# safe-autonomous-systems/fluidgym

Measured on AMD Instinct MI355X. Metric: env-steps/sec (batched) + pressure-Poisson HBM GB/s vs roofline, 1/2/4/8 GPUs, higher is better.
Workload: dtype f32; 1 GPU; ChannelJet2D-v0 (2D channel stand-in for 'cylinder Re=100 256x128'), 64 envs/GPU, 25 PISO steps/env step, random jets, stirred by a body force N(0,2.0) redrawn every env step; global_batch=64, parallelism=env-sharded x1, 1 bcast + 1 all_gather per step (RCCL), lanes_per_gpu=2, workload_modified=True, capped_solves=0, floor_released_solves=0, advection_solver_form=two-brick, velocity_solver=on-chip Jacobi sweeps (policy advection_jacobi; 11972 solves settled by

## Files before the change

### fluidgym_amd/_lib.py

```python
from __future__ import annotations

import ctypes
import os
from ctypes import POINTER, Structure, c_char_p, c_float, c_int, c_int32, c_int64, c_void_p

_HERE = os.path.dirname(os.path.abspath(__file__))
LIB_PATH = os.environ.get("FLUIDGYM_AMD_LIB") or os.path.join(_HERE, "libfluidgym_hip.so")
LIB_F64_PATH = os.environ.get("FLUIDGYM_AMD_LIB_F64") or os.path.join(_HERE, "libfluidgym_hip_f64.so")

FG_MAX_SCALARS = 4
FG_FIELD_SUMMARY_WORK_BYTES = 128
FG_OK = 0
FG_ERR_NOT_CONVERGED = -5
FG_ERR_NOT_FINITE = -6
FG_ERR_FLUX_BALANCE = -7
FG_PERIODIC, FG_FIXED = 0, 1
FG_DIRICHLET, FG_NEUMANN = 0, 1
FG_VELOCITY, FG_PRESSURE, FG_SCALAR, FG_VELOCITY_SOURCE, FG_VISCOSITY_FIELD = 0, 1, 2, 3, 4
FG_BOUND_VELOCITY, FG_BOUND_SCALAR = 8, 16
FG_SOLVER_CG, FG_SOLVER_JACOBI, FG_SOLVER_RBGS, FG_SOLVER_MGCG, FG_SOLVER_FDCG = 0, 1, 2, 3, 4
(FG_BUF_A, FG_BUF_C_OFF, FG_BUF_ADV_RHS, FG_BUF_VEL_RESULT, FG_BUF_H, FG_BUF_DIV, FG_BUF_P_RESULT,
 FG_BUF_SCALAR_RESULT) = range(8)
FG_ERR_UNSUPPORTED = -4
FG_ERR_INVALID_ARG = -1
# ... 77 lines not shown


class FgMbSimOptions(Structure):
    _fields_ = [
        ("step", FgMbStepOptions),
        ("time_step", c_float),
        ("cfl", c_float),
        ("adaptive", c_int32),
        ("substeps", c_int32),
        ("flux_balance_tol", c_float),
        ("outflow_slot0", c_int32),
        ("outflow_count", c_int32),
        ("outflow_velm", c_float * 3),
        ("outflow_tol", c_float),
        ("max_substeps", c_int32),
        ("outflow_slot0_b", c_int32),
        ("outflow_count_b", c_int32),
    ]


(FG_MB_BUF_A, FG_MB_BUF_C_OFF, FG_MB_BUF_RHS, FG_MB_BUF_H, FG_MB_BUF_DIV, FG_MB_BUF_P_DIAG, FG_MB_BUF_P_OFF,
 FG_MB_BUF_VELOCITY_RESULT) = range(8)
FG_MB_BUF_KRYLOV0 = 8


class FgSimOptions(Structure):
    _fields_ = [
        ("step", FgStepOptions),
        ("time_step", c_float),
        ("cfl", c_float),
        ("adaptive", c_int32),
        ("substeps", c_int32),
        ("flux_balance_tol", c_float),
        ("outflow_mask", c_int32),
        ("outflow_velm", c_float * 3),
        ("outflow_tol", c_float),
        ("max_substeps", c_int32),
    ]


SIGNATURES = {
    "fg_abi_version": (c_int, []),
    "fg_last_error": (c_char_p, []),
    "fg_create": (c_int, [POINTER(FgConfig), POINTER(c_float), POINTER(c_float), POINTER(c_float), POINTER(c_void_p)]),
    "fg_destroy": (c_int, [c_void_p]),
    "fg_bind": (c_int, [c_void_p, c_int, c_void_p]),
    "fg_set_viscosity": (c_int, [c_void_p, c_float]),
    "fg_set_scalar_viscosity": (c_int, [c_void_p, c_int, c_float]),
    "fg_set_viscosity_batch": (c_int, [c_void_p, c_void_p]),
    "fg_set_scalar_viscosity_batch": (c_int, [c_void_p, c_int, c_void_p]),
    "fg_set_fd_preconditioner": (c_int, [c_void_p] + [POINTER(c_float)] * 7),
    "fg_max_velocity": (c_int, [c_void_p, c_void_p, c_void_p]),
    "fg_set_fd_fast_transform": (c_int, [c_void_p, c_int, c_float]),
    "fg_set_return_best": (c_int, [c_void_p, c_int]),
    "fg_set_cg_reset_steps": (c_int, [c_void_p, c_int]),
    "fg_set_advection_start": (c_int, [c_void_p, c_int]),
    "fg_set_wall_stress_forcing": (c_int, [c_void_p, c_int, c_float, c_float]),
    "fg_boundary_flux_balance": (c_int, [c_void_p, c_void_p, c_void_p]),
    "fg_step_diagnostics": (c_int, [c_void_p, POINTER(c_float), c_void_p]),
    "fg_update_advective_boundary": (c_int, [c_void_p, c_int, POINTER(c_float), c_void_p, c_void_p]),
    "fg_balance_boundary_fluxes": (c_int, [c_void_p, c_int, c_float, c_void_p, c_void_p]),
    "fg_setup_advection": (c_int, [c_void_p, c_void_p, c_int, c_int, c_void_p]),
    "fg_solve_advection": (c_int, [c_void_p, c_int, c_int, c_float, c_int, POINTER(FgSolveInfo), c_void_p]),
    "fg_copy_scalar_result_to_blocks": (c_int, [c_void_p, c_int, c_void_p]),
    "fg_setup_pressure_matrix": (c_int, [c_void_p, c_void_p]),
    "fg_setup_pressure_rhs": (c_int, [c_void_p, c_void_p, c_void_p]),
    "fg_solve_pressure": (c_int, [c_void_p, c_int, c_float, c_int, c_int, POINTER(FgSolveInfo), c_void_p]),
    "fg_correct_velocity": (c_int, [c_void_p, c_void_p]),
    "fg_copy_velocity_result_to_blocks": (c_int, [c_void_p, c_void_p]),
    "fg_copy_velocity_result_from_blocks": (c_int, [c_void_p, c_void_p]),
    "fg_piso_step": (c_int, [c_void_p, c_void_p, POINTER(FgStepOptions), POINTER(c_int32), c_void_p]),
    "fg_single_step": (c_int, [c_void_p, POINTER(FgSimOptions), POINTER(c_int32), POINTER(c_float), c_void_p]),
    "fg_multi_step": (c_int, [c_void_p, POINTER(FgSimOptions), c_int32, POINTER(c_void_p), POINTER(c_int32), POINTER(c_float), POINTER(c_int32), c_void_p]),
    "fg_make_divergence_free": (c_int, [c_void_p, c_float, c_int, POINTER(FgSolveInfo), c_void_p]),
    "fg_reset_solver_state": (c_int, [c_void_p, c_void_p]),
    "fg_solver_hints": (c_int, [c_void_p, POINTER(c_int32), c_int32]),
    "fg_env_restore_field": (c_int, [c_void_p, c_int, c_void_p, c_int32, POINTER(FgEnvSel), c_int32, c_int32, c_void_p]),
    "fg_env_reset_solver_state": (c_int, [c_void_p, POINTER(FgEnvSel), c_int32, c_void_p]),
    "fg_mb_env_restore_field": (c_int, [c_void_p, c_int, c_void_p, c_int32, POINTER(FgEnvSel), c_int32, c_int32, c_void_p]),
    "fg_mb_env_reset_solver_state": (c_int, [c_void_p, POINTER(FgEnvSel), c_int32, c_void_p]),
    "fg_set_pressure_refinement": (c_int, [c_void_p, c_int32, c_float, c_float]),
    "fg_get_buffer": (c_int, [c_void_p, c_int, POINTER(c_void_p), POINTER(c_int64)]),
    "fg_read_buffer": (c_int, [c_void_p, c_int, c_void_p, c_void_p]),
    "fg_poisson_apply": (c_int, [c_void_p, c_void_p, c_void_p, c_void_p, c_void_p]),
    "fg_poisson_jacobi": (c_int, [c_void_p, c_void_p, c_void_p, c_void_p, c_int, c_float, c_void_p]),
    "fg_poisson_rbgs": (c_int, [c_void_p, c_void_p, c_void_p, c_void_p, c_int, c_float, c_void_p]),
    "fg_poisson_cg": (c_int, [c_void_p, c_void_p, c_void_p, c_void_p, c_float, c_int, c_int, POINTER(FgSolveInfo),
                              c_void_p]),
    "fg_poisson_fdcg": (c_int, [c_void_p, c_void_p, c_void_p, c_void_p, c_float, c_int, c_int, POINTER(FgSolveInfo),
                                c_void_p]),
    "fg_sparse_apply_ell": (c_int, [c_void_p, c_void_p, c_int32, c_int32, c_void_p, c_int64, c_int32, c_void_p, c_void_p]),
    "fg_sparse_apply_csr": (c_int, [c_void_p, c_void_p, c_void_p, c_int32, c_void_p, c_int64, c_int32, c_void_p, c_void_p]),
    "fg_stream_triad": (c_int, [c_void_p, c_void_p, c_void_p, c_float, c_int64, c_int32, POINTER(c_float), c_void_p]),
    "fg_mb_multilevel_status": (c_int, [c_void_p, POINTER(c_int32)]),
    "fg_mb_multilevel_apply": (c_int, [c_void_p, c_void_p, c_void_p, c_void_p]),
    "fg_mb_debug_ilu_apply": (c_int, [c_void_p, c_void_p, c_void_p, c_void_p]),
    "fg_mb_debug_pressure_cg": (c_int, [c_void_p, c_float, c_int32, c_int32, POINTER(c_int32), POINTER(c_int32), POINTER(ctypes.c_double), c_void_p]),
    "fg_mb_wall_forces": (c_int, [c_void_p, c_void_p, c_void_p, c_void_p, c_int32, c_int32, c_float, c_float, c_void_p, c_void_p]),
    "fg_mb_wall_forces_batch": (c_int, [c_void_p, c_void_p, c_void_p, c_void_p, c_int32, c_int32, c_float, c_float, c_void_p, c_void_p, c_void_p]),
    "fg_mb_debug_bicgstab": (c_int, [c_void_p, c_float, c_int32, c_int32, POINTER(c_int64), POINTER(ctypes.c_double), POINTER(c_float), c_void_p]),
    "fg_dacc_host_sum": (c_int, [POINTER(ctypes.c_double), c_int64, ctypes.c_double, POINTER(ctypes.c_double)]),
    "fg_dacc_device_sum": (c_int, [POINTER(ctypes.c_double), c_int64, ctypes.c_double, c_int32, POINTER(ctypes.c_double), c_void_p]),
    "fg_field_summary": (c_int, [c_void_p, c_int32, c_int32, c_int64, c_int32, c_void_p, c_void_p, c_void_p, ctypes.c_double, ctypes.c_double,
                                 c_int32, c_void_p, c_void_p]),
    "fg_plane_moments": (c_int, [POINTER(c_void_p), POINTER(c_int64), c_int32, c_int32, c_int32, c_int32, c_int32, c_int32, c_void_p, c_void_p,
                                 c_void_p, c_void_p, c_void_p]),
    "fg_plane_budgets": (c_int, [POINTER(c_void_p), POINTER(c_int64), c_int32, c_int32, c_int32, c_int32, c_int32, c_void_p, c_void_p, c_void_p,
                                 c_int32, c_int32, c_void_p, c_void_p, c_void_p, c_void_p, c_void_p]),
    "fg_plane_timecorr": (c_int, [POINTER(c_void_p), POINTER(c_int64), c_int32, c_int32, c_int32, c_int32, c_int32, c_int32, c_int32,
                                  POINTER(c_int32), c_void_p, c_void_p, c_void_p, c_void_p]),
    "fg_mb_cell_moments": (c_int, [c_void_p, c_void_p, c_int32, c_int32, c_int64, POINTER(c_int64), c_int32, c_int64, c_void_p, c_void_p,
                                   c_void_p]),
    "fg_mb_cell_moments_widths": (c_int, [c_void_p, c_void_p, c_int64, POINTER(c_int64), c_int32, c_void_p, c_void_p, POINTER(c_int32)]),
    "fg_plane_spectra": (c_int, [POINTER(c_void_p), POINTER(c_int64), c_int32, c_int32, c_int32, c_int32, c_int32, POINTER(c_int32), c_int32,
                                 c_void_p, c_void_p, c_void_p]),
    "fg_coherence_litmus": (c_int, [c_int32, c_int32, c_int32, c_int32, POINTER(c_int64), POINTER(ctypes.c_double), c_void_p]),
    "fg_profile_enable": (c_int, [c_void_p, c_int]),
    "fg_profile_kinds": (c_int, []),
    "fg_profile_kind_name": (ctypes.c_char_p, [c_int]),
    "fg_profile_read": (c_int, [c_void_p, c_int, POINTER(ctypes.c_double), POINTER(c_int64), POINTER(ctypes.c_double),
                                POINTER(ctypes.c_double), POINTER(ctypes.c_double), POINTER(ctypes.c_double),
                                POINTER(c_int64), POINTER(c_int64), POINTER(ctypes.c_double), POINTER(c_int64)]),
    "fg_coords_to_transforms": (c_int, [c_void_p, c_void_p, c_int, c_int, c_int, c_int, c_void_p]),
    "fg_resampler_create": (c_int, [c_int, POINTER(ctypes.c_int32), POINTER(ctypes.c_int32), POINTER(ctypes.c_int32),
                                    POINTER(ctypes.c_float), c_int, c_int, POINTER(c_void_p)]),
    "fg_resampler_destroy": (c_int, [c_void_p]),
    "fg_resample": (c_int, [c_void_p, c_void_p, c_int, c_int, c_void_p, c_int, c_void_p]),
    "fg_envglue_jet_schedule": (c_int, [c_void_p, c_void_p, c_void_p, c_void_p, c_int32, c_int32, c_int32, c_void_p, c_void_p, c_void_p]),
    "fg_envglue_channel_observe": (c_int, [c_void_p, c_void_p, c_void_p, c_int32, c_int32, c_int32, c_int32, c_float, c_float, c_void_p,
                                           c_void_p, c_void_p, c_void_p, c_void_p, c_void_p]),
    "fg_envglue_channel_observe_batch": (c_int, [c_void_p, c_void_p, c_void_p, c_int32, c_int32, c_int32, c_int32, c_void_p, c_float, c_void_p,
                                                 c_void_p, c_void_p, c_void_p, c_void_p, c_void_p]),
    "fg_mb_create": (c_int, [c_int32, c_int32, c_int32, POINTER(c_void_p)]),
    "fg_mb_destroy": (c_int, [c_void_p]),
    "fg_config_dump": (c_int, [c_void_p, ctypes.c_char_p, c_int]),
    "fg_mb_config_dump": (c_int, [c_void_p, ctypes.c_char_p, c_int]),
    "fg_mb_add_block": (c_int, [c_void_p, POINTER(c_float), c_int32, c_int32, c_int32, POINTER(c_int32)]),
    "fg_mb_connect": (c_int, [c_void_p, c_int32, c_int32, c_int32, c_int32, c_int32, c_int32]),
    "fg_mb_make_periodic": (c_int, [c_void_p, c_int32, c_int32]),
    "fg_mb_set_reference_quirks": (c_int, [c_void_p, c_int32, c_int32]),
    "fg_mb_set_nonortho_flags": (c_int, [c_void_p, c_int32]),
    "fg_mb_finalize": (c_int, [c_void_p]),
    "fg_mb_sizes": (c_int, [c_void_p, POINTER(c_int32), POINTER(c_int32)]),
    "fg_mb_block_info": (c_int, [c_void_p, c_int32, POINTER(c_int32), POINTER(c_int32)]),
    "fg_mb_get_host_table": (c_int, [c_void_p, c_int32, c_void_p, POINTER(c_int64)]),
    "fg_mb_get_neighbors": (c_int, [c_void_p, POINTER(c_int32)]),
    "fg_mb_bind": (c_int, [c_void_p, c_void_p, c_void_p, c_void_p, c_void_p]),
    "fg_mb_set_viscosity": (c_int, [c_void_p, c_float]),
    "fg_mb_set_viscosity_batch": (c_int, [c_void_p, c_void_p]),
    "fg_mb_piso_step": (c_int, [c_void_p, c_void_p, POINTER(FgMbStepOptions), POINTER(c_int32), c_void_p]),
    "fg_mb_max_velocity": (c_int, [c_void_p, POINTER(c_float), c_void_p]),
    "fg_mb_set_residual_projection": (c_int, [c_void_p, POINTER(c_float)]),
    "fg_mb_set_stall_limit": (c_int, [c_void_p, c_int32]),
    "fg_mb_set_advection_start": (c_int, [c_void_p, c_int]),
    "fg_mb_set_advection_jacobi": (c_int, [c_void_p, c_int]),
    "fg_mb_advection_jacobi_counts": (c_int, [c_void_p, POINTER(c_int64)]),
    "fg_mb_set_multilevel": (c_int, [c_void_p, c_int32, c_int32, POINTER(c_int32), POINTER(c_int32), POINTER(c_int32), POINTER(c_float),
                                     POINTER(c_float), c_float, c_int32]),
    "fg_mb_env_status": (c_int, [c_void_p, POINTER(c_int32)]),
    "fg_mb_ladder": (c_int, [c_void_p, POINTER(c_int64), c_int32]),
    "fg_mb_debug_cycles": (c_int, [c_void_p, POINTER(ctypes.c_uint64)]),
    "fg_mb_solver_hints": (c_int, [c_void_p, POINTER(c_int32), c_int32]),
    "fg_mb_solver_unconverged": (c_int, [c_void_p, POINTER(c_int64)]),
    "fg_solver_unconverged": (c_int, [c_void_p, POINTER(c_int64)]),
    "fg_mb_solver_counters": (c_int, [c_void_p, POINTER(c_int64), c_int32]),
    "fg_set_advection_preconditioner": (c_int, [c_void_p, c_int]),
# ... 124 lines not shown
```

### fluidgym_amd/csrc/fg_api.hip

```cpp
#include <stdio.h>
#include <string.h>

#include <cmath>
#include <string>
#include <vector>

#include <stdlib.h>

#include "fg_internal.h"

static thread_local std::string g_last_error;
void fg_set_error(const std::string& msg) { g_last_error = msg; }

extern "C" int fg_abi_version(void) { return FG_ABI_VERSION; }
extern "C" const char* fg_last_error(void) { return g_last_error.c_str(); }

static FgBounds make_bounds(const fg_state* s, int channel) {
    FgBounds b;
    for (int f = 0; f < 6; ++f) {
        b.vel[f] = s->bvel[f];
        b.scal[f] = s->bscal[f];
        b.scalar_bc[f] = s->cfg.scalar_bc[f][channel < 0 ? 0 : channel];
    }
    return b;
// ... 20 lines not shown
    FG_REQUIRE(cfg->n_scalars >= 0 && cfg->n_scalars <= FG_MAX_SCALARS, FG_ERR_INVALID_ARG, "bad n_scalars");
    for (int a = 0; a < cfg->dims; ++a)
        FG_REQUIRE(cfg->face_type[2 * a] == cfg->face_type[2 * a + 1], FG_ERR_INVALID_ARG,
                   "a FIXED face needs a FIXED partner (CloseBoundary closes both, domain_structs.cpp:1981-2002)");
    FG_REQUIRE((long long)cfg->nx * cfg->ny * cfg->nz * cfg->batch * 6 < (1LL << 31), FG_ERR_UNSUPPORTED,
               "index space exceeds int32 (reference index_t is int32 as well)");
    FG_HIP_CHECK(hipSetDevice(cfg->device));

    fg_state* s = new fg_state();
    memset(s, 0, sizeof(*s));
    s->cfg = *cfg;
    FgGrid& g = s->grid;
    g.dims = cfg->dims; g.nx = cfg->nx; g.ny = cfg->ny; g.nz = cfg->nz;
    g.n = cfg->nx * cfg->ny * cfg->nz; g.B = cfg->batch;
    for (int f = 0; f < 6; ++f) g.fixed[f] = (f < 2 * cfg->dims) ? (cfg->face_type[f] == FG_FIXED) : 0;
    s->vec = (!FG_F64 && cfg->nx % 4 == 0) ? 4 : 1;
    s->viscosity = 0.f;

    const fg_real* hsrc[3] = {hx, hy, hz};
    const int hn[3] = {cfg->nx, cfg->ny, cfg->nz};
    for (int a = 0; a < 3; ++a) {
        std::vector<fg_real> h(hn[a], 1.f), rh(hn[a], 1.f);
        if (a < cfg->dims)
            for (int i = 0; i < hn[a]; ++i) {
                if (!(hsrc[a][i] > 0.f)) { delete s; fg_set_error("cell widths must be positive"); return FG_ERR_INVALID_ARG; }
                h[i] = hsrc[a][i]; rh[i] = 1.f / hsrc[a][i];
            }
        FG_HIP_CHECK(hipMalloc(&s->d_h[a], sizeof(fg_real) * hn[a]));
        FG_HIP_CHECK(hipMalloc(&s->d_rh[a], sizeof(fg_real) * hn[a]));
        FG_HIP_CHECK(hipMemcpy(s->d_h[a], h.data(), sizeof(fg_real) * hn[a], hipMemcpyHostToDevice));
        FG_HIP_CHECK(hipMemcpy(s->d_rh[a], rh.data(), sizeof(fg_real) * hn[a], hipMemcpyHostToDevice));
        g.h[a] = s->d_h[a]; g.rh[a] = s->d_rh[a];
    }
    const size_t BN = (size_t)g.B * g.n, d = g.dims;
    auto alloc = [&](fg_real** p, size_t count) -> hipError_t {
        hipError_t e = hipMalloc(p, sizeof(fg_real) * count);
        if (e == hipSuccess) e = hipMemset(*p, 0, sizeof(fg_real) * count);
        return e;
    };
    FG_HIP_CHECK(alloc(&s->A, BN));
    FG_HIP_CHECK(alloc(&s->rA, BN));
    FG_HIP_CHECK(alloc(&s->Coff, BN * 2 * d));
    FG_HIP_CHECK(alloc(&s->adv_rhs, BN * d));
    FG_HIP_CHECK(alloc(&s->vel_result, BN * d));
    FG_HIP_CHECK(alloc(&s->hvec, BN * d));
    FG_HIP_CHECK(alloc(&s->div, BN));
    FG_HIP_CHECK(alloc(&s->p_result, BN));
    FG_HIP_CHECK(alloc(&s->scal_result, BN));
    for (int i = 0; i < 8; ++i) FG_HIP_CHECK(alloc(&s->w[i], BN * d));
    const size_t nsys = (size_t)g.B * d;
    FG_HIP_CHECK(hipMalloc(&s->acc, sizeof(FgDacc) * nsys * FG_ACC_DOUBLES));
    FG_HIP_CHECK(hipMemset(s->acc, 0, sizeof(FgDacc) * nsys * FG_ACC_DOUBLES));
    FG_HIP_CHECK(hipMalloc(&s->flags, sizeof(int32_t) * nsys));
    FG_HIP_CHECK(hipMalloc(&s->info_dev, sizeof(fg_solve_info) * nsys));
    FG_HIP_CHECK(hipHostMalloc(&s->info_pinned, sizeof(fg_solve_info) * nsys));
    FG_HIP_CHECK(hipHostMalloc(&s->flags_pinned, sizeof(int32_t) * nsys));
    FG_HIP_CHECK(alloc(&s->scratch_B, (size_t)g.B * (4 + 2 * d)));
    FG_HIP_CHECK(hipMalloc(&s->d_bvel_ptrs, sizeof(fg_real*) * 6));
    FG_HIP_CHECK(hipMemset(s->d_bvel_ptrs, 0, sizeof(fg_real*) * 6));
    FG_HIP_CHECK(hipHostMalloc(&s->diag_pinned, sizeof(fg_real) * 2 * g.B));
    FG_HIP_CHECK(hipHostMalloc(&s->dt_pinned, sizeof(fg_real) * g.B));
    FG_HIP_CHECK(alloc(&s->dt_dev, g.B));
    FG_HIP_CHECK(hipMalloc(&s->env_sel_dev, sizeof(fg_env_sel) * g.B));
    s->t_rem_dev = nullptr;
#if !FG_F64
    FG_HIP_CHECK(hipMalloc(&s->t_rem_dev, sizeof(double) * g.B));
    FG_HIP_CHECK(hipMemset(s->t_rem_dev, 0, sizeof(double) * g.B));
#endif
    if (int rc = fg_poll_create(&s->poll, (int)(nsys > 2 * (size_t)g.B ? nsys : 2 * (size_t)g.B))) return rc;
    for (int k = 0; k < 4; ++k) { s->pred_bicg[k] = 2; s->pred_cg[k] = 1; }
    s->wall_forcing_axis = -1;
    s->ref64_inner = 1e-4f;
    s->cg_wgs_per_slot = 256;
    { const char* ev = getenv("FG_BICG3"); s->bicg3_force = ev ? atoi(ev) : -1; }
    { const char* ev = getenv("FG_BICG3_BXL"); s->bicg3_bxl = ev ? atoi(ev) : 0; }
    { const char* ev = getenv("FG_BICG_SUB"); s->bicg_sub = ev ? atoi(ev) : -1; }
    { const char* ev = getenv("FG_REDUCE_WGS"); s->reduce_wgs = ev ? atoi(ev) : 0; }
    { const char* ev = getenv("FG_BICG3_MIX"); s->bicg3_mix = ev ? atoi(ev) : 3; }
    { const char* ev = getenv("FG_BICG_FUSED"); s->bicg_fused = ev ? atoi(ev) : 1; }
    s->tridiag_cb = 64;
    s->helm_cb_pref = 32;
    { const char* ev = getenv("FG_HELM_ROWFORM"); s->helm_rowform_off = (ev && atoi(ev) == 0) ? 1 : 0; }
    { const char* ev = getenv("FG_FD_FACFUSE"); s->fd_facfuse = ev ? atoi(ev) : 1; }
    { const char* ev = getenv("FG_DEV_DT"); s->dev_dt = ev ? atoi(ev) : 1; }
    { const char* ev = getenv("FG_ADV_LINESWEEP"); s->adv_linesweep = ev ? atoi(ev) : 0; }
    { const char* ev = getenv("FG_FD_ROWMEAN"); s->fd_rowmean = ev ? atoi(ev) : 1; }
    s->fd_row_epoch = -1; s->rA_epoch = 0; s->fd_row_part_epoch = -1;
    { const char* ev = getenv("FG_CG_FUSED"); s->cg_fused = ev ? atoi(ev) : 1; }
    { const char* ev = getenv("FG_BICG_PFUSED"); s->bicg_pfused = ev ? atoi(ev) : 1; }
    { const char* ev = getenv("FG_ADV_JACOBI"); s->adv_jacobi = ev ? atoi(ev) : 0; s->adv_jacobi_env = ev ? 1 : 0; }
    for (int k = 0; k < 4; ++k) s->jac_hist[k] = FgJacHist{0, 0, 0};
    s->jac_solves = s->jac_fallbacks = 0;
    FG_HIP_CHECK(hipHostMalloc(&s->jac_prev, sizeof(float) * 4 * nsys));
    s->jac_rA_epoch = -1;
    FG_HIP_CHECK(hipMalloc(&s->fcg_alpha, sizeof(double) * 2 * (size_t)g.B));
    FG_HIP_CHECK(hipMemset(s->fcg_alpha, 0, sizeof(double) * 2 * (size_t)g.B));
    FG_HIP_CHECK(hipMalloc(&s->fcg_xsum, sizeof(FgDacc) * 2 * (size_t)g.B));
    FG_HIP_CHECK(hipMemset(s->fcg_xsum, 0, sizeof(FgDacc) * 2 * (size_t)g.B));
    FG_HIP_CHECK(hipMalloc(&s->fcg_lazy, sizeof(int32_t) * (size_t)g.B));
    FG_HIP_CHECK(hipMemset(s->fcg_lazy, 0, sizeof(int32_t) * (size_t)g.B));
    { const char* e = getenv("FG_FCG_FIRST"); s->fcg_first = (e && atoi(e) == 0) ? 0 : 1; }
    { const char* e = getenv("FG_JAC_SPEC"); s->jac_spec = (e && atoi(e) == 0) ? 0 : 1; }
    { const char* e = getenv("FG_FCG_SPEC"); s->fcg_spec = (e && atoi(e) == 0) ? 0 : 1; }
    { const char* e = getenv("FG_JAC_PREFACTOR"); s->jac_prefactor = (e && atoi(e) == 0) ? 0 : 1; }
    { const char* e = getenv("FG_JAC_WARM"); s->jac_warm = e ? (atoi(e) != 0 ? 1 : 0) : -1; }
    s->cg_return_best = 1;
    s->cg_reset_steps = 100;
    s->adv_from_result = 1;
    FG_HIP_CHECK(hipMalloc(&s->cg_acc, sizeof(FgDacc) * (size_t)g.B * 8 * 64));
    FG_HIP_CHECK(hipMemset(s->cg_acc, 0, sizeof(FgDacc) * (size_t)g.B * 8 * 64));
    FG_HIP_CHECK(hipMalloc(&s->cg_best.best_crit, sizeof(fg_real) * g.B));
    FG_HIP_CHECK(hipMalloc(&s->cg_best.saved_crit, sizeof(fg_real) * g.B));
    FG_HIP_CHECK(hipMalloc(&s->cg_best.save_at, sizeof(int32_t) * g.B));
    FG_HIP_CHECK(alloc(&s->cg_best.best_x, BN));
    *out = s;
    return FG_OK;
}

extern "C" int fg_destroy(fg_handle s) {
    if (!s) return FG_OK;
    for (int a = 0; a < 3; ++a) { (void)hipFree(s->d_h[a]); (void)hipFree(s->d_rh[a]); }
    fg_real* owned[] = {s->A, s->rA, s->Coff, s->adv_rhs, s->vel_result, s->hvec, s->div, s->p_result, s->scal_result,
                      s->scratch_B};
    for (fg_real* p : owned) (void)hipFree(p);
    for (int i = 0; i < 8; ++i) (void)hipFree(s->w[i]);
    (void)hipFree(s->acc); (void)hipFree(s->flags); (void)hipFree(s->info_dev);
    (void)hipHostFree(s->info_pinned); (void)hipHostFree(s->flags_pinned);
    fg_prof_destroy(s);
    fg_poll_destroy(&s->poll);
    (void)hipFree(s->d_bvel_ptrs); (void)hipHostFree(s->diag_pinned); (void)hipHostFree(s->dt_pinned); (void)hipFree(s->dt_dev); (void)hipFree(s->t_rem_dev); (void)hipFree(s->env_sel_dev);
    float* fd[] = {s->fd_Qx, s->fd_QxT, s->fd_Qz, s->fd_QzT, s->fd_lower, s->fd_inv, s->fd_cp};
    for (float* p : fd) if (p) (void)hipFree(p);
    if (s->fd_dct_tw) { (void)hipFree(s->fd_dct_tw); (void)hipFree(s->fd_dct_rot); }
    (void)hipFree(s->cg_acc); (void)hipFree(s->fcg_alpha); (void)hipFree(s->fcg_xsum); (void)hipFree(s->fcg_lazy);
    if (s->jac_prev) (void)hipHostFree(s->jac_prev);
    (void)hipFree(s->fd_row_part); (void)hipFree(s->fd_lam_x); (void)hipFree(s->fd_row_inv); (void)hipFree(s->fd_row_cp); (void)hipFree(s->fd_row_lower);
    (void)hipFree(s->line_inv); (void)hipFree(s->line_cp); (void)hipFree(s->ilu_d);
    (void)hipFree(s->r64_buf); (void)hipFree(s->r64_acc); (void)hipFree(s->ref64_x); (void)hipFree(s->force_uniform);
    (void)hipFree(s->fd_lam); (void)hipFree(s->helm_diag); (void)hipFree(s->helm_lower); (void)hipFree(s->helm_upper); (void)hipFree(s->helm_tmp); (void)hipFree(s->helm_lower_row); (void)hipFree(s->helm_lower_row2); (void)hipFree(s->line_inv2); (void)hipFree(s->line_cp2);
    (void)hipFree(s->cg_best.best_crit); (void)hipFree(s->cg_best.saved_crit); (void)hipFree(s->cg_best.save_at); (void)hipFree(s->cg_best.best_x);
    delete s;
    return FG_OK;
}

static int sync_bvel_ptrs(fg_state* s);
extern "C" int fg_bind(fg_handle s, int field, fg_real* ptr) {
    FG_REQUIRE(s, FG_ERR_INVALID_ARG, "null handle");
    if (field == FG_VELOCITY) s->velocity = ptr;
    else if (field == FG_PRESSURE) s->pressure = ptr;
    else if (field == FG_SCALAR) s->scalar = ptr;
    else if (field == FG_VELOCITY_SOURCE) s->velocity_source = ptr;
    else if (field == FG_VISCOSITY_FIELD) s->visc_field = ptr;
    else if (field >= FG_BOUND_VELOCITY && field < FG_BOUND_VELOCITY + 6) {
        s->bvel[field - FG_BOUND_VELOCITY] = ptr;
        return sync_bvel_ptrs(s);
    }
    else if (field >= FG_BOUND_SCALAR && field < FG_BOUND_SCALAR + 6) s->bscal[field - FG_BOUND_SCALAR] = ptr;
    else FG_REQUIRE(false, FG_ERR_INVALID_ARG, "fg_bind: unknown field id");
    return FG_OK;
}

extern "C" int fg_set_viscosity(fg_handle s, fg_real v) {
    FG_REQUIRE(s, FG_ERR_INVALID_ARG, "null handle");
    s->viscosity = v;
    return FG_OK;
}
extern "C" int fg_set_scalar_viscosity(fg_handle s, int ch, fg_real v) {
    FG_REQUIRE(s && ch >= 0 && ch < FG_MAX_SCALARS, FG_ERR_INVALID_ARG, "bad channel");
    s->scalar_viscosity[ch] = v;
    s->scalar_viscosity_set = true;
    return FG_OK;
}
extern "C" int fg_set_viscosity_batch(fg_handle s, const fg_real* nu_B) {
    FG_REQUIRE(s, FG_ERR_INVALID_ARG, "null handle");
    s->viscosity_B = nu_B;
    s->helm_pre_mask = 0;
    return FG_OK;
}
extern "C" int fg_set_scalar_viscosity_batch(fg_handle s, int ch, const fg_real* k_B) {
    FG_REQUIRE(s && ch >= 0 && ch < FG_MAX_SCALARS, FG_ERR_INVALID_ARG, "bad channel");
    s->scalar_viscosity_B[ch] = k_B;
    s->helm_pre_mask = 0;
    return FG_OK;
}

extern "C" int fg_set_fd_preconditioner(fg_handle s, const float* Qx, const float* QxT, const float* Qz, const float* QzT,
                                        const float* lower, const float* inv, const float* cp) {
    FG_REQUIRE(s && Qx && QxT && lower && inv && cp, FG_ERR_INVALID_ARG, "null argument");
    FG_REQUIRE(s->grid.fixed[2] && s->grid.fixed[3], FG_ERR_UNSUPPORTED, "FD preconditioner needs FIXED y faces");
    FG_REQUIRE(s->grid.dims == 2 || (Qz && QzT), FG_ERR_INVALID_ARG, "Qz required in 3-D");
#if !FG_F64
    FG_REQUIRE(s->grid.ny <= 640, FG_ERR_UNSUPPORTED, "FD preconditioner: at most 640 cells along y (LDS of the tridiagonal solve)");
#endif
    const size_t nx = s->grid.nx, ny = s->grid.ny, nz = s->grid.nz;
    auto up = [&](float** dst, const float* src, size_t count) -> hipError_t {
        if (*dst) (void)hipFree(*dst);
        hipError_t e = hipMalloc(dst, sizeof(float) * count);
        if (e == hipSuccess) e = hipMemcpy(*dst, src, sizeof(float) * count, hipMemcpyHostToDevice);
        return e;
    };
    FG_HIP_CHECK(up(&s->fd_Qx, Qx, nx * nx));
    FG_HIP_CHECK(up(&s->fd_QxT, QxT, nx * nx));
    if (s->grid.dims == 3) {
        FG_HIP_CHECK(up(&s->fd_Qz, Qz, nz * nz));
        FG_HIP_CHECK(up(&s->fd_QzT, QzT, nz * nz));
    }
    FG_HIP_CHECK(up(&s->fd_lower, lower, ny));
    FG_HIP_CHECK(up(&s->fd_inv, inv, nx * ny * nz));
    FG_HIP_CHECK(up(&s->fd_cp, cp, nx * ny * nz));
    s->fd_dct_x = 0;
    return FG_OK;
}

extern "C" int fg_set_return_best(fg_handle s, int on) {
    FG_REQUIRE(s, FG_ERR_INVALID_ARG, "null handle");
    s->cg_return_best = on ? 1 : 0;
    return FG_OK;
// ... 221 lines not shown
    return setup_advection(s, dt_B, for_scalar, channel, stream, -1, 0);
}
static int setup_advection(fg_handle s, const fg_real* dt_B, int for_scalar, int channel, void* stream, int buoy_axis, fg_real buoy_factor) {
    FG_REQUIRE(s && dt_B, FG_ERR_INVALID_ARG, "null argument");
    if (int rc = check_bound(s, for_scalar != 0)) return rc;
    FG_REQUIRE(!for_scalar || (channel >= 0 && channel < s->cfg.n_scalars), FG_ERR_INVALID_ARG, "bad scalar channel");
    s->cur_dt = dt_B;
    FgAdvArgs a;
    memset(&a, 0, sizeof(a));
    a.vel = s->velocity;
    a.dt = dt_B;
    a.for_scalar = for_scalar;
    a.channel = channel;
    a.n_scalars = s->cfg.n_scalars;
    a.A = s->A; a.Coff = s->Coff; a.rhs = s->adv_rhs;
    if (for_scalar) {
        a.scal = s->scalar + (size_t)channel * s->grid.n;
        a.scal_env_stride = (long)s->cfg.n_scalars * s->grid.n;
        a.nu = fg_nu(s, 1, channel);
    } else {
        a.source = s->velocity_source;
        if (s->wall_forcing_axis >= 0)
            if (int rc = fg_launch_wall_forcing(s, (hipStream_t)stream)) return rc;
        a.force = s->wall_forcing_axis >= 0 ? s->force_uniform : nullptr;
        a.visc = s->visc_field;
        a.nu = fg_nu(s);
        a.rA = s->rA;
        s->adv_last_dt = dt_B;
        s->rA_epoch++;
        s->jac_rA_epoch = s->rA_epoch;
#if !FG_F64
        if (fg_fd_rowmean_ok(s) && s->vec == 4 && (s->grid.nx & 63) == 0) {
            if (!s->fd_row_part) FG_HIP_CHECK(hipMalloc(&s->fd_row_part, sizeof(float) * (size_t)s->grid.B * s->grid.ny * (s->grid.nx / 64)));
            a.row_part = s->fd_row_part;
            s->fd_row_part_epoch = s->rA_epoch;
        }
#endif
        if (buoy_axis >= 0) {
            a.buoy_T = s->scalar; a.buoy_stride = (long)s->cfg.n_scalars * s->grid.n; a.buoy_axis = buoy_axis; a.buoy_factor = buoy_factor;
            a.source_w = s->velocity_source;
        }
    }
    return fg_launch_adv_build(s, make_bounds(s, channel), a, (hipStream_t)stream);
}

static int advection_solve(fg_state* s, FgBicgArgs a, fg_solve_info* info, hipStream_t st, int for_scalar = 0, int channel = 0, bool* spec_ran = nullptr);

extern "C" int fg_solve_advection(fg_handle s, int for_scalar, int channel, fg_real tol, int max_iterations,
                                  fg_solve_info* info_host, void* stream) {
    FG_REQUIRE(s, FG_ERR_INVALID_ARG, "null handle");
    FgBicgArgs a;
    a.diag = s->A; a.off = s->Coff; a.rhs = s->adv_rhs;
    a.dt = s->cur_dt;
    a.tol = tol; a.max_iterations = max_iterations;
    if (for_scalar) { a.x = s->scal_result; a.nc = 1; a.use_x0 = 0; a.kind = 0; }
    else { a.x = s->vel_result; a.nc = s->grid.dims; a.use_x0 = s->adv_from_result; }
    return advection_solve(s, a, info_host, (hipStream_t)stream, for_scalar, channel);
}

extern "C" int fg_copy_scalar_result_to_blocks(fg_handle s, int channel, void* stream) {
    FG_REQUIRE(s && s->scalar, FG_ERR_NOT_BOUND, "scalar not bound");
    const int n = s->grid.n;
    if (s->cfg.n_scalars == 1) return fg_launch_copy_active(s, s->cur_dt, s->scal_result, s->scalar, 1, (hipStream_t)stream);
    FG_HIP_CHECK(hipMemcpy2DAsync(s->scalar + (size_t)channel * n, sizeof(fg_real) * n * s->cfg.n_scalars, s->scal_result,
                                  sizeof(fg_real) * n, sizeof(fg_real) * n, s->grid.B, hipMemcpyDeviceToDevice,
                                  (hipStream_t)stream));
    return FG_OK;
}

extern "C" int fg_setup_pressure_matrix(fg_handle s, void* stream) {
    FG_REQUIRE(s, FG_ERR_INVALID_ARG, "null handle");
    s->rA_epoch++;
    return fg_launch_pressure_setup(s, s->cur_dt, (hipStream_t)stream);
}

extern "C" int fg_setup_pressure_rhs(fg_handle s, const fg_real* dt_B, void* stream) {
    FG_REQUIRE(s && dt_B, FG_ERR_INVALID_ARG, "null argument");
    if (int rc = check_bound(s, false)) return rc;
    hipStream_t st = (hipStream_t)stream;
    if (int rc = fg_launch_h(s, dt_B, s->vel_result, st)) return rc;
    return fg_launch_div(s, make_bounds(s, 0), dt_B, s->hvec, s->div, st);
}

struct SpecH { fg_state* s; const fg_real* dt; const fg_step_options* opt; hipStream_t st; };
static int spec_h(void* p) {
    const SpecH* c = static_cast<const SpecH*>(p);
    fg_state* s = c->s;
    if (int rc = fg_launch_h(s, c->dt, s->vel_result, c->st)) return rc;
    return fg_launch_div(s, make_bounds(s, 0), c->dt, s->hvec, s->div, c->st, !c->opt->pressure_warm_start,
                         c->opt->pressure_method == FG_SOLVER_FDCG && s->fd_Qx != nullptr);
}

static int launch_corrector(fg_state* s, const fg_real* dt, const FgCgOutcome& o, bool last, hipStream_t st) {
    const bool mean_folded = last && o.mean_ready;
    FG_REQUIRE(!o.lazy_z || !last || mean_folded, FG_ERR_UNSUPPORTED, "fg_piso_step: an unmaterialised pressure without its folded mean");
    if (last && !mean_folded)
        if (int rc = fg_launch_mean_sub(s, dt, s->p_result, s->pressure, st)) return rc;
    const FgMeanRef mean = {s->fcg_xsum, s->info_dev, s->pressure, o.marks_valid ? s->fcg_lazy : nullptr, s->fcg_alpha};
    const FgLazyRef lazy = {s->fcg_lazy, s->fcg_alpha, last ? s->p_result : nullptr};
    const fg_real* p = o.lazy_z ? o.lazy_z : ((last && !mean_folded) ? s->pressure : s->p_result);
    return fg_launch_correct(s, dt, s->rA, s->hvec, p, s->vel_result, st, last ? s->velocity : nullptr, mean_folded ? &mean : nullptr, o.lazy_z ? &lazy : nullptr);
}

struct SpecCorrect { fg_state* s; const fg_real* dt; bool last; hipStream_t st; };
static int spec_correct(void* p, const FgCgOutcome& o) {
    const SpecCorrect* c = static_cast<const SpecCorrect*>(p);
    return launch_corrector(c->s, c->dt, o, c->last, c->st);
}

static int solve_pressure(fg_state* s, const fg_real* dt, int method, fg_real tol, int max_iterations, int use_previous,
                          fg_solve_info* info_host, hipStream_t st, bool finalize = true, int kind = 2, FgCgOutcome* out = nullptr,
                          FgCgSpec spec = FgCgSpec{}) {
    int rc = FG_OK;
    FgCgOutcome own;
    if (!out) out = &own;
    if (method == FG_SOLVER_CG || method == FG_SOLVER_FDCG) {
        FgCgArgs a;
        a.rA = s->rA; a.b = s->div; a.x = s->p_result;
        a.r = s->w[0]; a.p = s->w[1]; a.Ap = s->w[2];
        a.dt = dt; a.tol = tol; a.max_iterations = max_iterations; a.use_x0 = use_previous;
        a.reset_steps = s->cg_reset_steps;
        a.precond = (method == FG_SOLVER_FDCG);
        a.kind = kind;
        a.check_every = a.precond ? 2 : 16;
        a.lazy_ok = finalize ? 0 : 1;
        a.spec = spec;
#if !FG_F64
        if (s->ref64_outer > 0) a.lazy_ok = 0;
#endif
        rc = fg_cg_solve(s, a, info_host, st, out);
#if !FG_F64
        if (s->ref64_outer > 0 && (rc == FG_OK || rc == FG_ERR_NOT_CONVERGED)) rc = fg_refine64_pressure(s, a, info_host, st, out);
        if (s->double_fallback && (rc == FG_ERR_NOT_FINITE || (s->ladder_force & 2))) {
            std::vector<fg_solve_info> tmp;
            fg_solve_info* info = info_host;
            if (!info) { tmp.assign(s->info_pinned, s->info_pinned + s->grid.B); info = tmp.data(); }
            s->rung_count[2] += 1;
            rc = fg_rung64_cg(s, a, info, (s->ladder_force & 2) != 0, st, out);
        }
#endif
    } else {
        fg_set_error("fg_solve_pressure: only FG_SOLVER_CG drives the PISO step (Jacobi/RBGS are smoothers)");
        return FG_ERR_UNSUPPORTED;
    }
    if (rc != FG_OK && rc != FG_ERR_NOT_CONVERGED) return rc;
    if (finalize)
        if (int rc2 = fg_launch_mean_sub(s, dt, s->p_result, s->pressure, st)) return rc2;
    return rc;
}

extern "C" int fg_solve_pressure(fg_handle s, int method, fg_real tol, int max_iterations, int use_previous,
                                 fg_solve_info* info_host, void* stream) {
    FG_REQUIRE(s, FG_ERR_INVALID_ARG, "null handle");
    if (int rc = check_bound(s, false)) return rc;
    return solve_pressure(s, s->cur_dt, method, tol, max_iterations, use_previous, info_host, (hipStream_t)stream);
}

extern "C" int fg_set_pressure_refinement(fg_handle s, int32_t max_corrections, fg_real target_tol, fg_real inner_relative_tol) {
    FG_REQUIRE(s, FG_ERR_INVALID_ARG, "null handle");
    FG_REQUIRE(!FG_F64 || max_corrections <= 0, FG_ERR_UNSUPPORTED, "fg_set_pressure_refinement: the fp64 build solves in fp64 already");
    FG_REQUIRE(max_corrections <= 0 || (target_tol > 0 && inner_relative_tol > 0 && inner_relative_tol < 1), FG_ERR_INVALID_ARG,
               "fg_set_pressure_refinement: tolerances must be positive, the relative one below 1");
    s->ref64_outer = max_corrections > 0 ? max_corrections : 0;
    s->ref64_tol = (float)target_tol; s->ref64_inner = (float)inner_relative_tol;
    return FG_OK;
}

extern "C" int fg_correct_velocity(fg_handle s, void* stream) {
    FG_REQUIRE(s, FG_ERR_INVALID_ARG, "null handle");
    if (int rc = check_bound(s, false)) return rc;
    return fg_launch_correct(s, s->cur_dt, s->rA, s->hvec, s->pressure, s->vel_result, (hipStream_t)stream);
}

// ... 29 lines not shown
    if (failed && s->double_fallback && rc != FG_ERR_HIP) {
        s->rung_count[0] += 1;
        rc = fg_rung64_bicgstab(s, a, info, (s->ladder_force & 1) != 0, st);
        if (rc != FG_OK && rc != FG_ERR_NOT_CONVERGED && rc != FG_ERR_NOT_FINITE) return rc;
        failed = (rc != FG_OK) || (s->ladder_force & 4);
    }
#endif
    if (failed && (s->adv_precond == 2 || s->adv_precond == 5)) {
        s->line_retries += 1;
        s->rung_count[1] += 1;
        a.precond = s->adv_precond == 5 ? 3 : 1; a.use_x0 = 0;
        rc = fg_bicgstab_solve(s, a, info, st);
    }
    (void)nsys;
    return rc;
}

extern "C" int fg_piso_step(fg_handle s, const fg_real* dt_B, const fg_step_options* opt, int32_t* stats_host,
                            void* stream) {
    FG_REQUIRE(s && dt_B && opt, FG_ERR_INVALID_ARG, "null argument");
    const bool scalar = opt->advect_scalar && s->cfg.n_scalars > 0;
    if (int rc = check_bound(s, scalar)) return rc;
    FG_REQUIRE(opt->buoyancy_axis < s->grid.dims, FG_ERR_INVALID_ARG, "bad buoyancy axis");
    FG_REQUIRE(opt->buoyancy_axis < 0 || (s->velocity_source && s->scalar), FG_ERR_NOT_BOUND,
               "buoyancy needs velocity source and scalar bound");
    hipStream_t st = (hipStream_t)stream;
    const int B = s->grid.B, d = s->grid.dims;
    std::vector<fg_solve_info> info((size_t)B * d);
    int32_t stats[4] = {-1, -1, -1, -1};
    struct DropHelmRecord { fg_state* s; ~DropHelmRecord() { s->helm_pre_mask = 0; } } drop_helm_record{s};
    int status = FG_OK;
    auto soft = [&](int rc) {
        if (rc == FG_ERR_NOT_CONVERGED) { status = rc; return FG_OK; }
        return rc;
    };
#if !FG_F64
    const bool sweeps_first = s->adv_linesweep && s->grid.dims == 2 && s->jac_hist[0].skip == 0 && s->jac_hist[1].skip == 0;
    if (scalar && s->cfg.n_scalars == 1 && s->adv_precond == 3 && s->fd_lam && !s->visc_field && !sweeps_first) {
        const FgNu nu2[2] = {fg_nu(s, 1, 0), fg_nu(s)};
        const int wlo[2] = {s->cfg.scalar_bc[2][0] == FG_DIRICHLET, 1}, whi[2] = {s->cfg.scalar_bc[3][0] == FG_DIRICHLET, 1};
        if (int rc = fg_helm_factor_pair(s, dt_B, nu2, wlo, whi, st)) return rc;
    }
#endif
    if (scalar) {
        FgRange range_scalar("scalar_advection");
        for (int ch = 0; ch < s->cfg.n_scalars; ++ch) {
            if (int rc = fg_setup_advection(s, dt_B, 1, ch, stream)) return rc;
            FgBicgArgs a;
            a.diag = s->A; a.off = s->Coff; a.rhs = s->adv_rhs; a.x = s->scal_result; a.nc = 1;
            a.dt = dt_B; a.tol = opt->advection_tol; a.max_iterations = opt->max_iterations; a.use_x0 = 0; a.kind = 0;
            if (int rc = soft(advection_solve(s, a, info.data(), st, 1, ch))) return rc;
            const int m = max_iters(info.data(), B);
            stats[0] = m > stats[0] ? m : stats[0];
            s->ctr.add(0, info.data(), B);
            const int n = s->grid.n;
            if (s->cfg.n_scalars == 1) {
                if (int rc = fg_launch_copy_active(s, dt_B, s->scal_result, s->scalar, 1, st)) return rc;
            } else {
                (void)n;
                fg_set_error("multi-channel scalar copy with inactive envs not implemented");
                return FG_ERR_UNSUPPORTED;
            }
        }
    }
    fg_range_push("velocity_assembly_and_solve");
    struct PopOnce { bool armed = true; void fire() { if (armed) { fg_range_pop(); armed = false; } } ~PopOnce() { fire(); } } range_velocity;
    if (int rc = setup_advection(s, dt_B, 0, 0, stream, opt->buoyancy_axis, opt->buoyancy_factor)) return rc;
    bool h_div_ran = false;
    {
        FgBicgArgs a;
        a.diag = s->A; a.off = s->Coff; a.rhs = s->adv_rhs; a.x = s->vel_result; a.nc = d;
        a.dt = dt_B; a.tol = opt->advection_tol; a.max_iterations = opt->max_iterations; a.use_x0 = s->adv_from_result;
        SpecH spec_h_ctx = {s, dt_B, opt, st};
        if (opt->corrector_steps > 0) a.spec = FgSpecHook{spec_h, &spec_h_ctx};
        if (int rc = soft(advection_solve(s, a, info.data(), st, 0, 0, &h_div_ran))) return rc;
        stats[1] = max_iters(info.data(), B * d);
        s->ctr.add(1, info.data(), B * d);
    }
    range_velocity.fire();
    for (int c = 0; c < opt->corrector_steps; ++c) {
        FgRange range_corr(c == 0 ? "pressure_corrector_0" : "pressure_corrector_1+");
        const bool last = (c + 1 == opt->corrector_steps);
        if (!(c == 0 && h_div_ran)) {
            if (int rc = fg_launch_h(s, dt_B, s->vel_result, st)) return rc;
            if (int rc = fg_launch_div(s, make_bounds(s, 0), dt_B, s->hvec, s->div, st, !opt->pressure_warm_start,
                                       opt->pressure_method == FG_SOLVER_FDCG && s->fd_Qx != nullptr))
                return rc;
        }
        SpecCorrect spec_ctx = {s, dt_B, last, st};
        FgCgOutcome outcome;
        if (int rc = soft(solve_pressure(s, dt_B, opt->pressure_method, opt->pressure_tol, opt->max_iterations, opt->pressure_warm_start ? 1 : 0,
                                         info.data(), st, false, c == 0 ? 0 : 1, &outcome, FgCgSpec{spec_correct, &spec_ctx})))
            return rc;
        if (c < 2) { stats[2 + c] = max_iters(info.data(), B); s->ctr.add(2 + c, info.data(), B); }
        if (!outcome.spec_done)
            if (int rc = launch_corrector(s, dt_B, outcome, last, st)) return rc;
    }
    if (opt->corrector_steps <= 0)
        if (int rc = fg_launch_copy_active(s, dt_B, s->vel_result, s->velocity, d, st)) return rc;
    if (stats_host) memcpy(stats_host, stats, sizeof(stats));
    s->ctr.piso_steps += 1;
    return status;
}

extern "C" int fg_config_dump(fg_handle s, char* buf, int n) {
    FG_REQUIRE(s && buf && n > 0, FG_ERR_INVALID_ARG, "fg_config_dump: bad argument");
    char tmp[3072];
    const int len = snprintf(tmp, sizeof(tmp),
        "{\"build\": \"%s\", \"FG_CG_FUSED\": %d, \"FG_BICG_PFUSED\": %d, \"FG_BICG_FUSED\": %d, \"FG_BICG_SUB\": %d, \"FG_BICG3\": %d, "
        "\"FG_BICG3_BXL\": %d, \"FG_BICG3_MIX\": %d, \"FG_REDUCE_WGS\": %d, \"FG_CG_WGS_PER_SLOT\": %d, \"FG_TRIDIAG_CB\": %d, \"FG_HELM_CB\": %d, "
        "\"FG_HELM_ROWFORM\": %d, \"FG_FD_ROWMEAN\": %d, \"FG_POLL_SPIN\": %d, \"FG_PROF_PERIOD\": %d, \"fast_transform_x\": %d, \"fd_preconditioner\": %d, "
        "\"helmholtz\": %d, \"advection_preconditioner\": %d, \"advection_from_result\": %d, \"return_best\": %d, \"cg_reset_steps\": %d, "
        "\"double_fallback\": %d, \"wall_forcing_axis\": %d, \"FG_ADV_JACOBI\": %d, \"FG_FCG_FIRST\": %d, \"FG_JAC_WARM\": %d, \"first_iterate_polls\": %ld, \"unstored_pressure_solves\": %ld, \"FG_JAC_SPEC\": %d, \"FG_FCG_SPEC\": %d, \"jacobi_speculation_misses\": %ld, \"jacobi_floor_released\": %ld, \"pressure_refinement_corrections\": %ld}",
        FG_F64 ? "f64" : "f32", s->cg_fused, s->bicg_pfused, s->bicg_fused, s->bicg_sub, s->bicg3_force, s->bicg3_bxl, s->bicg3_mix, s->reduce_wgs,
        s->cg_wgs_per_slot, s->tridiag_cb, s->helm_cb_pref, s->helm_rowform_off ? 0 : 1, s->fd_rowmean, s->poll.spin, s->prof.period, s->fd_dct_x, s->fd_Qx ? 1 : 0,
        s->fd_lam ? 1 : 0, s->adv_precond, s->adv_from_result, s->cg_return_best, s->cg_reset_steps, s->double_fallback, s->wall_forcing_axis, s->adv_jacobi, s->fcg_first, s->jac_warm,
        s->fcg_first_polls, s->fcg_unstored, s->jac_spec, s->fcg_spec, s->jac_spec_missed, s->jac_floor_released, s->ref64_corrections);
    if (len >= n) return len + 1;
    memcpy(buf, tmp, (size_t)len + 1);
    return FG_OK;
}

extern "C" int fg_solver_unconverged(fg_handle s, int64_t* out4) {
    FG_REQUIRE(s != nullptr && out4 != nullptr, FG_ERR_INVALID_ARG, "fg_solver_unconverged: bad argument");
    for (int k = 0; k < 4; ++k) out4[k] = s->ctr.unconv[k];
    return FG_OK;
}

extern "C" int fg_solver_counters(fg_handle s, int64_t* out13, int32_t reset) {
    FG_REQUIRE(s != nullptr, FG_ERR_INVALID_ARG, "fg_solver_counters: null handle");
    if (out13) s->ctr.write(out13);
    if (reset) s->ctr.reset();
    return FG_OK;
}

extern "C" int fg_single_step(fg_handle s, const fg_sim_options* o, int32_t* out, fg_real* flux_host, void* stream);
extern "C" int fg_multi_step(fg_handle s, const fg_sim_options* o, int32_t n, const fg_real* const* bvel_schedule, int32_t* out_6n,
                             fg_real* flux_host, int32_t* steps_done, void* stream) {
    FG_REQUIRE(s && o && out_6n && n >= 0, FG_ERR_INVALID_ARG, "fg_multi_step: bad argument");
    if (steps_done) *steps_done = 0;
    for (int k = 0; k < n; ++k) {
        if (bvel_schedule)
            for (int f = 0; f < 2 * s->grid.dims; ++f)
                if (const fg_real* p = bvel_schedule[(size_t)k * 6 + f])
                    if (int rc = fg_bind(s, FG_BOUND_VELOCITY + f, const_cast<fg_real*>(p))) return rc;
        if (int rc = fg_single_step(s, o, out_6n + 6 * (size_t)k, flux_host, stream)) return rc;
        if (steps_done) *steps_done = k + 1;
        if (out_6n[6 * (size_t)k + 5] == 0 && !s->cg_return_best) break;
    }
    return FG_OK;
}

static inline bool is_close_zero(double a) { return std::fabs(a) <= 1e-8; }

extern "C" int fg_single_step(fg_handle s, const fg_sim_options* o, int32_t* out, fg_real* flux_host, void* stream) {
    fg_htrace("single_step_in");
    FgRange range_sim("fg_single_step");
    FG_REQUIRE(s && o && out, FG_ERR_INVALID_ARG, "null argument");
    if (int rc = check_bound(s, o->step.advect_scalar && s->cfg.n_scalars > 0)) return rc;
    hipStream_t st = (hipStream_t)stream;
    const int B = s->grid.B;
    const FgBounds bnd = make_bounds(s, 0);
    std::vector<double> t_rem(B, (double)o->time_step);
    int32_t stats[4] = {-1, -1, -1, -1};
    int substeps = 0, all_ok = 1;
    bool first = true;
    int fixed_left = o->adaptive ? 0 : (o->substeps > 0 ? o->substeps : 1);
    for (;;) {
        bool any = false;
        if (o->adaptive) {
            for (int b = 0; b < B; ++b) any = any || (t_rem[b] > 0 && !is_close_zero(t_rem[b]));
        } else {
            any = fixed_left > 0;
        }
        if (!any) break;
        auto advance = [&](int b, fg_real max_vel) -> fg_real {
            fg_real ts = 0.f;
            if (!o->adaptive) {
                ts = o->time_step;
            } else if (t_rem[b] > 0 && !is_close_zero(t_rem[b])) {
                const double mv = (double)max_vel;
                const double max_ts = is_close_zero(mv) ? t_rem[b] : (double)o->cfl / mv;
                double tsd;
                if (max_ts >= t_rem[b]) tsd = t_rem[b];
                else tsd = t_rem[b] / (double)(long long)std::ceil(t_rem[b] / max_ts);
                t_rem[b] -= tsd;
                ts = (fg_real)tsd;
            }
            return ts;
        };
        auto flux_guard = [&]() -> int {
            fg_real worst = 0.f;
            for (int b = 0; b < B; ++b) {
                if (flux_host) flux_host[b] = s->diag_pinned[b];
                const fg_real a = std::fabs(s->diag_pinned[b]);
                worst = (a > worst || a != a) ? a : worst;
            }
            if (!(worst <= o->flux_balance_tol)) {
                fg_set_error("Domain boundary fluxes not balanced, cannot proceed with simulation step.");
                return FG_ERR_FLUX_BALANCE;
// ... 53 lines not shown
                s->diag_pinned[B + b] = fg_poll_word_float(&s->poll, 12 * B + b);
                if (first) s->diag_pinned[b] = fg_poll_word_float(&s->poll, 13 * B + b);
            }
            if (first) if (int rc2 = flux_guard()) return rc2;
            for (int b = 0; b < B; ++b) s->dt_pinned[b] = advance(b, s->diag_pinned[B + b]);
        }
        ++substeps;
        first = false;
        if (!o->adaptive) --fixed_left;
        if (substeps >= (o->max_substeps > 0 ? o->max_substeps : 100000)) break;
    }
    fg_htrace("single_step_out");
    for (int i = 0; i < 4; ++i) out[i] = stats[i];
    out[4] = substeps;
    out[5] = all_ok;
    return FG_OK;
}

extern "C" int fg_make_divergence_free(fg_handle s, fg_real tol, int max_iterations, fg_solve_info* info_host,
                                       void* stream) {
    FG_REQUIRE(s, FG_ERR_INVALID_ARG, "null handle");
    if (int rc = check_bound(s, false)) return rc;
    s->cur_dt = nullptr;
    hipStream_t st = (hipStream_t)stream;
    const size_t BN = (size_t)s->grid.B * s->grid.n;
    std::vector<fg_real> ones(BN, 1.f);
    FG_HIP_CHECK(hipMemcpyAsync(s->rA, ones.data(), sizeof(fg_real) * BN, hipMemcpyHostToDevice, st));
    s->rA_epoch++;
    FG_HIP_CHECK(hipStreamSynchronize(st));
    if (int rc = fg_launch_copy_active(s, nullptr, s->velocity, s->hvec, s->grid.dims, st)) return rc;
    if (int rc = fg_launch_div(s, make_bounds(s, 0), nullptr, s->hvec, s->div, st)) return rc;
    int rc = solve_pressure(s, nullptr, FG_SOLVER_CG, tol, max_iterations, 0, info_host, st);
    if (rc != FG_OK && rc != FG_ERR_NOT_CONVERGED) return rc;
    if (int rc2 = fg_launch_correct(s, nullptr, s->rA, s->hvec, s->pressure, s->vel_result, st)) return rc2;
    if (int rc2 = fg_launch_copy_active(s, nullptr, s->vel_result, s->velocity, s->grid.dims, st)) return rc2;
    return rc;
}

extern "C" int fg_reset_solver_state(fg_handle s, void* stream) {
    FG_REQUIRE(s && s->velocity, FG_ERR_NOT_BOUND, "velocity not bound");
    for (int k = 0; k < 4; ++k) s->jac_hist[k] = FgJacHist{0, 0, 0};
    FG_HIP_CHECK(hipMemsetAsync(s->p_result, 0, sizeof(fg_real) * (size_t)s->grid.B * s->grid.n, (hipStream_t)stream));
    return fg_launch_copy_active(s, nullptr, s->velocity, s->vel_result, s->grid.dims, (hipStream_t)stream);
}

extern "C" int fg_solver_hints(fg_handle s, int32_t* hints12, int32_t set) {
    FG_REQUIRE(s != nullptr && hints12 != nullptr, FG_ERR_INVALID_ARG, "fg_solver_hints: bad argument");
    for (int k = 0; k < 4; ++k) {
        FgJacHist& H = s->jac_hist[k];
        if (set) { H.sweeps = hints12[3 * k]; H.skip = hints12[3 * k + 1]; H.fails = hints12[3 * k + 2]; }
        else { hints12[3 * k] = H.sweeps; hints12[3 * k + 1] = H.skip; hints12[3 * k + 2] = H.fails; }
    }
    return FG_OK;
}

extern "C" int fg_get_buffer(fg_handle s, int which, fg_real** out_ptr, int64_t* out_count) {
    FG_REQUIRE(s && out_ptr && out_count, FG_ERR_INVALID_ARG, "null argument");
    const int64_t BN = (int64_t)s->grid.B * s->grid.n, d = s->grid.dims;
    switch (which) {
        case FG_BUF_A: *out_ptr = s->A; *out_count = BN; break;
        case FG_BUF_C_OFF: *out_ptr = s->Coff; *out_count = BN * 2 * d; break;
        case FG_BUF_ADV_RHS: *out_ptr = s->adv_rhs; *out_count = BN * d; break;
        case FG_BUF_VEL_RESULT: *out_ptr = s->vel_result; *out_count = BN * d; break;
        case FG_BUF_H: *out_ptr = s->hvec; *out_count = BN * d; break;
        case FG_BUF_DIV: *out_ptr = s->div; *out_count = BN; break;
        case FG_BUF_P_RESULT: *out_ptr = s->p_result; *out_count = BN; break;
        case FG_BUF_SCALAR_RESULT: *out_ptr = s->scal_result; *out_count = BN; break;
        default:
            if (which >= 100 && which < 108) { *out_ptr = s->w[which - 100]; *out_count = BN * d; break; }
            FG_REQUIRE(false, FG_ERR_INVALID_ARG, "unknown buffer id");
    }
    return FG_OK;
}

extern "C" int fg_read_buffer(fg_handle s, int which, fg_real* dst, void* stream) {
    fg_real* src = nullptr;
    int64_t count = 0;
    if (int rc = fg_get_buffer(s, which, &src, &count)) return rc;
    FG_REQUIRE(dst, FG_ERR_INVALID_ARG, "null destination");
    FG_HIP_CHECK(hipMemcpyAsync(dst, src, sizeof(fg_real) * count, hipMemcpyDeviceToDevice, (hipStream_t)stream));
    return FG_OK;
}

extern "C" int fg_poisson_apply(fg_handle s, const fg_real* rA, const fg_real* x, fg_real* y, void* stream) {
    FG_REQUIRE(s && rA && x && y, FG_ERR_INVALID_ARG, "null argument");
    return fg_poisson_apply_launch(s, rA, x, y, (hipStream_t)stream);
}

extern "C" int fg_poisson_jacobi(fg_handle s, const fg_real* rA, const fg_real* b, fg_real* x, int n_sweeps, fg_real omega,
                                 void* stream) {
    FG_REQUIRE(s && rA && b && x && n_sweeps >= 0, FG_ERR_INVALID_ARG, "bad argument");
    hipStream_t st = (hipStream_t)stream;
    fg_real* buf[2] = {x, s->w[5]};
    for (int i = 0; i < n_sweeps; ++i)
        if (int rc = fg_poisson_jacobi_launch(s, rA, b, buf[i & 1], buf[(i + 1) & 1], omega, st)) return rc;
    if (n_sweeps & 1)
        FG_HIP_CHECK(hipMemcpyAsync(x, s->w[5], sizeof(fg_real) * (size_t)s->grid.B * s->grid.n, hipMemcpyDeviceToDevice, st));
    return FG_OK;
}

extern "C" int fg_poisson_rbgs(fg_handle s, const fg_real* rA, const fg_real* b, fg_real* x, int n_sweeps, fg_real omega,
                               void* stream) {
    FG_REQUIRE(s && rA && b && x && n_sweeps >= 0, FG_ERR_INVALID_ARG, "bad argument");
    hipStream_t st = (hipStream_t)stream;
    for (int i = 0; i < n_sweeps; ++i) {
        if (int rc = fg_poisson_rbgs_launch(s, rA, b, x, omega, 0, st)) return rc;
        if (int rc = fg_poisson_rbgs_launch(s, rA, b, x, omega, 1, st)) return rc;
    }
    return FG_OK;
}

extern "C" int fg_poisson_cg(fg_handle s, const fg_real* rA, const fg_real* b, fg_real* x, fg_real tol, int max_iterations,
                             int use_x0, fg_solve_info* info_host, void* stream) {
    FG_REQUIRE(s && rA && b && x, FG_ERR_INVALID_ARG, "null argument");
    FgCgArgs a;
    a.rA = rA; a.b = b; a.x = x;
    a.r = s->w[0]; a.p = s->w[1]; a.Ap = s->w[2];
    a.dt = nullptr; a.tol = tol; a.max_iterations = max_iterations; a.use_x0 = use_x0;
    a.reset_steps = 100;
    a.precond = 0;
    a.check_every = (tol > 0.f) ? 16 : (1 << 30);
    return fg_cg_solve(s, a, info_host, (hipStream_t)stream);
}

extern "C" int fg_poisson_fdcg(fg_handle s, const fg_real* rA, const fg_real* b, fg_real* x, fg_real tol, int max_iterations,
                               int use_x0, fg_solve_info* info_host, void* stream) {
    FG_REQUIRE(s && rA && b && x, FG_ERR_INVALID_ARG, "null argument");
    FgCgArgs a;
    a.rA = rA; a.b = b; a.x = x;
    a.r = s->w[0]; a.p = s->w[1]; a.Ap = s->w[2];
    a.dt = nullptr; a.tol = tol; a.max_iterations = max_iterations; a.use_x0 = use_x0;
    a.reset_steps = 0;
    a.precond = 1;
    a.check_every = (tol > 0.f) ? 2 : (1 << 30);
    return fg_cg_solve(s, a, info_host, (hipStream_t)stream);
}

extern "C" int fg_coords_to_transforms(const float* coords, float* transforms, int dims, int nx, int ny, int nz,
                                       void* stream) {
    FG_REQUIRE(coords && transforms && (dims == 2 || dims == 3), FG_ERR_INVALID_ARG, "bad argument");
#if FG_F64
    fg_set_error("fg_coords_to_transforms is an fp32 entry point: use libfluidgym_hip.so");
    return FG_ERR_UNSUPPORTED;
#else
    return fg_metrics_launch(coords, transforms, dims, nx, ny, nz, (hipStream_t)stream);
#endif
}
```

### fluidgym_amd/csrc/fg_cg.h

```cpp
#pragma once
#include "fg_internal.h"

#define FG_CG_SLOTS 64
#define FG_CG_NAMES 8

#ifdef __HIPCC__
__device__ __forceinline__ FgDacc* fg_acc_ptr(FgDacc* acc, int b, int name) {
    return acc + ((size_t)b * FG_CG_NAMES + name) * FG_CG_SLOTS;
}
__device__ __forceinline__ double fg_acc_total(const FgDacc* a, int ns) {
    if (ns == 1) return acc_ld(a + (0));
    const int lane = threadIdx.x & 63;
    double v = (lane < ns) ? acc_ld(a + (lane)) : 0.0;
#pragma unroll
    for (int o = 32; o > 0; o >>= 1) v += __shfl_xor(v, o, 64);
    return v;
}
__device__ __forceinline__ void fg_acc_zero(FgDacc* a, int ns) {
    const int lane = threadIdx.x & 63;
    if (lane < ns) acc_st(a + (lane), 0.0);
}
__device__ __forceinline__ void fg_acc_add(FgDacc* a, int ns, unsigned tile, double v) {
    acc_add(a + (tile & (unsigned)(ns - 1)), v);
}
#endif

struct FgCgBegin { FgDacc* acc; int32_t* flags; fg_solve_info* info; FgDacc* mean_sums; FgBest best; int track_best, ns;
                   FgDacc* xsum; };
int fg_cg_slots(const fg_state* s);
#ifdef __HIPCC__
__device__ __forceinline__ void fg_cg_begin_env(const FgCgBegin& q, const fg_real* __restrict__ dt, int b) {
    for (int k = threadIdx.x; k < FG_CG_NAMES * q.ns; k += blockDim.x)
        acc_st(fg_acc_ptr(q.acc, b, k / q.ns) + k % q.ns, 0.0);
    if (threadIdx.x != 0) return;
    acc_st(q.mean_sums + b, 0.0);
    if (q.xsum) { acc_st(q.xsum + 2 * b, 0.0); acc_st(q.xsum + 2 * b + 1, 0.0); }
    q.best.best_crit[b] = q.track_best ? INFINITY : 0.f;
    q.best.saved_crit[b] = INFINITY;
    q.best.save_at[b] = -1;
    const bool active = (dt == nullptr) || (dt[b] > 0.f);
    flag_st(q.flags + (b), active ? 0 : 3);
    q.info[b].final_residual = 0.f;
    q.info[b].used_iterations = -1;
    q.info[b].converged = active ? 0 : 1;
    q.info[b].is_finite = 1;
}
#endif

struct FgCgStart { FgDacc* acc; fg_real* r; fg_real* x; int ns; };

struct FgCgJudge {
    FgDacc* acc;
    int32_t* flags; fg_solve_info* info;
    fg_real tol; int it, n, ns;
};
#ifdef __HIPCC__
__device__ __forceinline__ bool fg_cg_judge(const FgCgJudge& j, int b, bool leader) {
    const double rr = fg_acc_total(fg_acc_ptr(j.acc, b, (j.it + 1) % 3), j.ns);
    const fg_real crit = (fg_real)sqrt(rr / (double)j.n);
    if (crit >= j.tol) return false;
    if (leader) {
        const bool finite = isfinite(crit);
        j.info[b].final_residual = crit;
        j.info[b].used_iterations = j.it;
        j.info[b].converged = finite ? 1 : 0;
        j.info[b].is_finite = finite ? 1 : 0;
        flag_st(j.flags + (b), finite ? 1 : 2);
    }
    return true;
}
#endif

struct FgCgLead { FgCgJudge judge; FgBest best; };
#ifdef __HIPCC__
__device__ __forceinline__ bool fg_cg_lead(const FgCgLead& q, int b, bool lead_block) {
    const FgCgJudge& j = q.judge;
    const double rr = fg_acc_total(fg_acc_ptr(j.acc, b, (j.it + 1) % 3), j.ns);
    const fg_real crit = (fg_real)sqrt(rr / (double)j.n);
    const bool done = !(crit >= j.tol);
    if (lead_block && threadIdx.x < 64) {
        if (!done) fg_acc_zero(fg_acc_ptr(j.acc, b, (j.it + 2) % 3), j.ns);
        if (threadIdx.x == 0) {
            j.info[b].final_residual = crit;
            j.info[b].used_iterations = j.it;
            if (done) {
                const bool finite = isfinite(crit);
                j.info[b].converged = finite ? 1 : 0;
                j.info[b].is_finite = finite ? 1 : 0;
                flag_st(j.flags + (b), finite ? 1 : 2);
            } else {
                fg_best_decide(q.best, b, crit, j.it + 1);
            }
        }
    }
    return done;
}
#endif
```

### fluidgym_amd/csrc/fg_fftcg.h

```cpp
#pragma once
#include "fg_internal.h"
#include "fg_cg.h"

constexpr int FCG_DELTA = 3, FCG_GAMMA = 5;

struct FcgVectors {
    fg_real* z; fg_real* w;
    fg_real* p; fg_real* s;
    fg_real* x; fg_real* r; fg_real* t1;
};

struct FcgUpdArgs {
    const float* z; const float* w; float* p; float* s; float* x; float* r; float* t1;
    const float2* tw; const float2* rot; float fs0, fs;
    const int32_t* flags; FgDacc* acc; double* alpha; FgDacc* xsum; FgBest best;
    int ns, rows, it, first; long env_stride;
    const float* r0; int x_zero;
    const int32_t* lazy;
};
struct FcgInvArgs {
    const float* u; const float* r; const float* rA; float* z; float* w;
    const float2* tw; const float2* rot; float is0, is;
    const int32_t* flags; FgDacc* acc; int ns, rows, it; long env_stride;
    const float* hy; const float* rhy; const float* hx; const float* rhx; int fixed_x;
    FgDacc* xsum; int extras;
};

struct FcgDivArgs {
    const float* h; float* div; float* r; float* x; float* t1;
    const float* bvel[4];
    const float2* tw; const float2* rot; float fs0, fs;
    const float* dt; FgDacc* acc; int ns, rows; long n;
    const float* hx; const float* hy; int fixed_x;
};

#if !FG_F64
int fg_fcg_div_fwd(fg_state* s, const FgBounds& bnd, const fg_real* dt, const fg_real* hvec, fg_real* div, int ns, hipStream_t st);
bool fg_fcg_ok(const fg_state* s);
int fg_fcg_update_fwd(fg_state* s, const FcgVectors& v, int it, int first, int ns, hipStream_t st, bool marks_valid, const fg_real* r0 = nullptr);
int fg_fcg_inv_apply(fg_state* s, const FcgVectors& v, const fg_real* rA, int it, int ns, hipStream_t st, int extras = 0);
int fg_fcg_check0(fg_state* s, fg_real tol, int ns, hipStream_t st, FgPollOut poll, bool* marks_valid);
#endif
```

### fluidgym_amd/csrc/fg_fftcg.hip

```cpp
#include "fg_internal.h"
#include "fg_cg.h"
#include "fg_fftrow.h"
#include "fg_fftcg.h"

#if !FG_F64
namespace {

using fgfft::Map;

template <int N, bool PERIODIC>
__global__ __launch_bounds__(256) void k_fcg_update_fwd(FcgUpdArgs a) {
    constexpr int EPL = N / 64;
    __shared__ __attribute__((aligned(16))) float2 buf[2][4][N];
    __shared__ __attribute__((aligned(16))) float2 twl[N];
    __shared__ float red[8];
    const int b = blockIdx.y;
    const int lane = threadIdx.x & 63, wave = threadIdx.x >> 6;
    if (a.flags[b] != 0) {
        if (a.lazy && a.lazy[b] == 1) {
            const float alpha = (float)a.alpha[b * 2];
            const int row0 = 2 * (blockIdx.x * 4 + wave);
#pragma unroll
            for (int half = 0; half < 2; ++half) {
                const int row = row0 + half;
                if (row >= a.rows) continue;
                const size_t o = (size_t)b * a.env_stride + (size_t)row * N;
                float zv[EPL], xv[EPL];
                fgfft::load_row<N>(a.z + o, lane, zv);
                if (a.x_zero) {
#pragma unroll
                    for (int e = 0; e < EPL; ++e) xv[e] = 0.f;
                } else {
                    fgfft::load_row<N>(a.x + o, lane, xv);
                }
#pragma unroll
                for (int e = 0; e < EPL; ++e) xv[e] += alpha * zv[e];
                fgfft::store_row<N>(a.x + o, lane, xv);
            }
        } else if (a.x_zero && (a.flags[b] == 1 || a.flags[b] == 2)) {
            float z0[EPL];
#pragma unroll
            for (int e = 0; e < EPL; ++e) z0[e] = 0.f;
            const int r0 = 2 * (blockIdx.x * 4 + wave);
            if (r0 < a.rows) fgfft::store_row<N>(a.x + (size_t)b * a.env_stride + (size_t)r0 * N, lane, z0);
            if (r0 + 1 < a.rows) fgfft::store_row<N>(a.x + (size_t)b * a.env_stride + (size_t)(r0 + 1) * N, lane, z0);
        }
        return;
    }
    for (int k = threadIdx.x; k < N; k += 256) twl[k] = a.tw[k];
    const int it = a.it;
    const double g_new = fg_acc_total(fg_acc_ptr(a.acc, b, FCG_GAMMA + it % 3), a.ns);
    const double d_new = fg_acc_total(fg_acc_ptr(a.acc, b, FCG_DELTA + (it & 1)), a.ns);
    double beta = 0.0, denom = d_new;
    if (!a.first) {
        const double g_old = fg_acc_total(fg_acc_ptr(a.acc, b, FCG_GAMMA + (it + 2) % 3), a.ns);
        const double al_old = a.alpha[b * 2 + ((it + 1) & 1)];
        beta = g_new / g_old;
        denom = d_new - beta * g_new / al_old;
    }
    const double alpha_d = g_new / denom;
    const float alpha = (float)alpha_d, betaf = (float)beta;
    const bool save = a.best.save_at[b] == it;
    if (blockIdx.x == 0 && threadIdx.x < 64) {
        fg_acc_zero(fg_acc_ptr(a.acc, b, FCG_GAMMA + (it + 1) % 3), a.ns);
        fg_acc_zero(fg_acc_ptr(a.acc, b, FCG_DELTA + ((it + 1) & 1)), a.ns);
        if (threadIdx.x == 0) {
            a.alpha[b * 2 + (it & 1)] = alpha_d;
            acc_st(a.xsum + (b * 2 + ((it + 1) & 1)), 0.0);
        }
    }
    const int row0 = 2 * (blockIdx.x * 4 + wave), row1 = row0 + 1;
    const bool live0 = row0 < a.rows, live1 = row1 < a.rows;
    const size_t o0 = (size_t)b * a.env_stride + (size_t)(live0 ? row0 : 0) * N;
    const size_t o1 = (size_t)b * a.env_stride + (size_t)(live1 ? row1 : 0) * N;
    float pa[EPL], pb[EPL], sa[EPL], sb[EPL], xa[EPL], xb[EPL], ra[EPL], rb[EPL];
    {
        float za[EPL], zb[EPL], wa[EPL], wb[EPL];
        fgfft::load_row<N>(a.z + o0, lane, za); fgfft::load_row<N>(a.z + o1, lane, zb);
        fgfft::load_row<N>(a.w + o0, lane, wa); fgfft::load_row<N>(a.w + o1, lane, wb);
        if (!a.first) {
            fgfft::load_row<N>(a.p + o0, lane, pa); fgfft::load_row<N>(a.p + o1, lane, pb);
            fgfft::load_row<N>(a.s + o0, lane, sa); fgfft::load_row<N>(a.s + o1, lane, sb);
        }
        if (a.x_zero) {
#pragma unroll
            for (int e = 0; e < EPL; ++e) { xa[e] = 0.f; xb[e] = 0.f; }
// ... 189 lines not shown
        const double g = fg_acc_total(fg_acc_ptr(acc, b, FCG_GAMMA), ns), d = fg_acc_total(fg_acc_ptr(acc, b, FCG_DELTA), ns);
        const double dd = fg_acc_total(fg_acc_ptr(acc, b, 2), ns);
        const double dw = fg_acc_total(fg_acc_ptr(acc, b, FCG_GAMMA + 2), ns), ww = fg_acc_total(fg_acc_ptr(acc, b, FCG_DELTA + 1), ns);
        const double alpha_d = g / d;
        const double e1 = 1.0 - (double)(float)alpha_d;
        double rr1 = dd + 2.0 * e1 * dw + e1 * e1 * ww;
        if (rr1 < 0.0) rr1 = 0.0;
        const float crit = (float)sqrt(rr1 / (double)n);
        if (lane == 0) {
            info[b].final_residual = crit;
            info[b].used_iterations = 0;
            if (!(crit >= tol)) {
                const bool finite = isfinite(crit);
                flag_st(flags + (b), finite ? 1 : 2);
                info[b].converged = finite ? 1 : 0;
                info[b].is_finite = finite ? 1 : 0;
                if (finite) { alpha[b * 2] = alpha_d; lz = 1; }
            }
        }
    }
    if (valid && lane == 0) lazy[b] = lz;
    if (!mirror) return;
    if (poll.gran) {
        uint32_t w[2] = {0u, 0u};
        const bool writer = valid && lane == 0;
        if (writer) { const fg_solve_info v = info[b]; w[0] = __float_as_uint(v.final_residual); w[1] = fg_info_word(v); }
        fg_poll_publish_records<2>(poll, b0, min(CHECK_WAVES, B - b0), wave, w, writer, stage);
    } else if (valid && lane == 0) { mirror[b] = info[b]; fg_poll_publish(poll, b); }
}

template <int N, bool PERIODIC>
__global__ __launch_bounds__(256) void k_fcg_div_fwd(FcgDivArgs a) {
    constexpr int EPL = N / 64;
    using M = Map<N>;
    constexpr int VW = M::VW;
    __shared__ __attribute__((aligned(16))) float2 buf[2][4][N];
    __shared__ __attribute__((aligned(16))) float2 twl[N];
    __shared__ float red[4];
    const int b = blockIdx.y;
    if (a.dt && !(a.dt[b] > 0.f)) return;
    const int lane = threadIdx.x & 63, wave = threadIdx.x >> 6;
    for (int k = threadIdx.x; k < N; k += 256) twl[k] = a.tw[k];
    const int row0 = 2 * (blockIdx.x * 4 + wave);
    const size_t hb0 = ((size_t)b * 2 + 0) * a.n, hb1 = ((size_t)b * 2 + 1) * a.n;
    float* sx = reinterpret_cast<float*>(buf[1][wave]);
    float da[EPL], db[EPL];
    float part[1] = {0.f};
#pragma unroll
    for (int half = 0; half < 2; ++half) {
        const int j = row0 + half;
        const bool live = j < a.rows;
        const int jc = live ? j : 0;
        float h0[EPL];
        fgfft::load_row<N>(a.h + hb0 + (size_t)jc * N, lane, h0);
#pragma unroll
        for (int q = 0; q < M::NG; ++q) fgfft::stv<VW>(sx + half * N + q * 64 * VW + lane * VW, &h0[q * VW]);
    }
    fgfft::wave_sync();
#pragma unroll
    for (int half = 0; half < 2; ++half) {
        const int j = row0 + half;
        const bool live = j < a.rows;
        const int jc = live ? j : 0;
        const float hy = a.hy[jc];
        const bool at_lo = jc == 0, at_hi = jc == a.rows - 1;
        const float* sr = sx + half * N;
        float* out = half ? db : da;
#pragma unroll
        for (int q = 0; q < M::NG; ++q) {
            const int i0 = q * 64 * VW + lane * VW;
            float hc[VW], v1[VW], vu[VW], vd[VW], hx[VW], bl[VW], bh[VW];
            fgfft::ldv<VW>(sr + i0, hc);
            fgfft::ldv<VW>(a.h + hb1 + (size_t)jc * N + i0, v1);
            fgfft::ldv<VW>(a.h + hb1 + (size_t)(at_lo ? jc : jc - 1) * N + i0, vu);
            fgfft::ldv<VW>(a.h + hb1 + (size_t)(at_hi ? jc : jc + 1) * N + i0, vd);
            fgfft::ldv<VW>(a.hx + i0, hx);
            if (at_lo) fgfft::ldv<VW>(a.bvel[2] + ((size_t)b * 2 + 1) * N + i0, bl);
            if (at_hi) fgfft::ldv<VW>(a.bvel[3] + ((size_t)b * 2 + 1) * N + i0, bh);
            const float hl = sr[(i0 == 0) ? N - 1 : i0 - 1], hr = sr[(i0 + VW == N) ? 0 : i0 + VW];
            const bool xlo = (i0 == 0) && a.fixed_x, xhi = (i0 + VW == N) && a.fixed_x;
#pragma unroll
            for (int e = 0; e < VW; ++e) {
                const float h_l = (e == 0) ? hl : hc[e > 0 ? e - 1 : 0], h_r = (e == VW - 1) ? hr : hc[e < VW - 1 ? e + 1 : VW - 1];
                float acc = 0.f;
                {
                    const float area = hy;
                    const float F_hi = (e == VW - 1 && xhi) ? a.bvel[1][((size_t)b * 2 + 0) * a.rows + jc] * area : 0.5f * (hc[e] + h_r) * area;
                    const float F_lo = (e == 0 && xlo) ? a.bvel[0][((size_t)b * 2 + 0) * a.rows + jc] * area : 0.5f * (hc[e] + h_l) * area;
                    acc += F_hi - F_lo;
                }
                {
                    const float area = hx[e];
                    const float F_hi = at_hi ? bh[e] * area : 0.5f * (v1[e] + vd[e]) * area;
                    const float F_lo = at_lo ? bl[e] * area : 0.5f * (v1[e] + vu[e]) * area;
                    acc += F_hi - F_lo;
                }
                out[q * VW + e] = live ? acc : 0.f;
            }
        }
        if (live) {
#pragma unroll
            for (int e = 0; e < EPL; ++e) part[0] += out[e] * out[e];
            const size_t o = (size_t)b * a.n + (size_t)j * N;
            fgfft::store_row<N>(a.div + o, lane, half ? db : da);
        }
    }
    __syncthreads();
    float oa[EPL], ob[EPL];
    fgfft::forward_rows<N, PERIODIC>(da, db, oa, ob, buf[0][wave], buf[1][wave], twl, a.rot, fgfft::Scales{a.fs0, a.fs}, lane);
    if (row0 < a.rows) fgfft::store_row<N>(a.t1 + (size_t)b * a.n + (size_t)row0 * N, lane, oa);
    if (row0 + 1 < a.rows) fgfft::store_row<N>(a.t1 + (size_t)b * a.n + (size_t)(row0 + 1) * N, lane, ob);
    fg_block_sum<1>(part, red);
    if (threadIdx.x == 0) fg_acc_add(fg_acc_ptr(a.acc, b, 0), a.ns, blockIdx.x, (double)part[0]);
}

template <bool PERIODIC>
int launch_upd(const fg_state* s, int slot, int n, const FcgUpdArgs& a, dim3 grid, hipStream_t st) {
    switch (n) {
        case 64: FG_LAUNCH_P(s, slot, (k_fcg_update_fwd<64, PERIODIC>), grid, dim3(256), 0, st, a); break;
        case 128: FG_LAUNCH_P(s, slot, (k_fcg_update_fwd<128, PERIODIC>), grid, dim3(256), 0, st, a); break;
        case 256: FG_LAUNCH_P(s, slot, (k_fcg_update_fwd<256, PERIODIC>), grid, dim3(256), 0, st, a); break;
        case 512: FG_LAUNCH_P(s, slot, (k_fcg_update_fwd<512, PERIODIC>), grid, dim3(256), 0, st, a); break;
        default: fg_set_error("fused CG: unsupported row length"); return FG_ERR_UNSUPPORTED;
    }
    return FG_OK;
}
template <bool PERIODIC>
int launch_inv(const fg_state* s, int slot, int n, const FcgInvArgs& a, dim3 grid, hipStream_t st) {
    switch (n) {
        case 64: FG_LAUNCH_P(s, slot, (k_fcg_inv_apply<64, PERIODIC>), grid, dim3(320), 0, st, a); break;
        case 128: FG_LAUNCH_P(s, slot, (k_fcg_inv_apply<128, PERIODIC>), grid, dim3(320), 0, st, a); break;
        case 256: FG_LAUNCH_P(s, slot, (k_fcg_inv_apply<256, PERIODIC>), grid, dim3(320), 0, st, a); break;
        case 512: FG_LAUNCH_P(s, slot, (k_fcg_inv_apply<512, PERIODIC>), grid, dim3(320), 0, st, a); break;
        default: fg_set_error("fused CG: unsupported row length"); return FG_ERR_UNSUPPORTED;
    }
    return FG_OK;
}

template <bool PERIODIC>
int launch_div(const fg_state* s, int n, const FcgDivArgs& a, dim3 grid, hipStream_t st) {
    const int slot = fg_prof_slot(s, FG_PK_DIV, nullptr, s->grid.B, 28.0 * (double)s->grid.n, (8.0 + 5.0 * log2((double)n)) * (double)s->grid.n, st);
    switch (n) {
        case 64: FG_LAUNCH_P(s, slot, (k_fcg_div_fwd<64, PERIODIC>), grid, dim3(256), 0, st, a); break;
        case 128: FG_LAUNCH_P(s, slot, (k_fcg_div_fwd<128, PERIODIC>), grid, dim3(256), 0, st, a); break;
        case 256: FG_LAUNCH_P(s, slot, (k_fcg_div_fwd<256, PERIODIC>), grid, dim3(256), 0, st, a); break;
        case 512: FG_LAUNCH_P(s, slot, (k_fcg_div_fwd<512, PERIODIC>), grid, dim3(256), 0, st, a); break;
        default: fg_set_error("fused CG: unsupported row length"); return FG_ERR_UNSUPPORTED;
    }
    return FG_OK;
}

}

bool fg_fcg_ok(const fg_state* s) {
    const FgGrid& G = s->grid;
    return s->cg_fused && s->fd_dct_x != 0 && G.dims == 2 && fg_fd_dct_supported(G.nx) && G.fixed[2] && G.fixed[3] && G.ny >= 3 &&
           s->fcg_alpha != nullptr;
}

int fg_fcg_update_fwd(fg_state* s, const FcgVectors& v, int it, int first, int ns, hipStream_t st, bool marks_valid, const fg_real* r0) {
    const FgGrid& G = s->grid;
    FcgUpdArgs a = {};
    a.r0 = r0; a.x_zero = r0 ? 1 : 0;
    a.lazy = (it == 0 && marks_valid) ? s->fcg_lazy : nullptr;
    a.z = v.z; a.w = v.w; a.p = v.p; a.s = v.s; a.x = v.x; a.r = v.r; a.t1 = v.t1;
    a.tw = s->fd_dct_tw; a.rot = s->fd_dct_rot; a.fs0 = s->fd_dct_fwd[0]; a.fs = s->fd_dct_fwd[1];
    a.flags = s->flags; a.acc = s->cg_acc; a.alpha = s->fcg_alpha; a.xsum = s->fcg_xsum; a.best = s->cg_best;
    a.ns = ns; a.rows = G.ny; a.it = it; a.first = first; a.env_stride = G.n;
    const dim3 grid((G.ny + 7) / 8, G.B);
    const int slot = fg_prof_slot(s, FG_PK_FCG_UPD, s->flags, G.B, (first ? (r0 ? 24.0 : 28.0) : 44.0) * G.n, (10.0 + 5.0 * log2((double)G.nx)) * G.n, st);
    if (int rc = (s->fd_dct_x == 2 ? launch_upd<true>(s, slot, G.nx, a, grid, st) : launch_upd<false>(s, slot, G.nx, a, grid, st))) return rc;
    FG_HIP_CHECK(hipGetLastError());
    return FG_OK;
}

int fg_fcg_inv_apply(fg_state* s, const FcgVectors& v, const fg_real* rA, int it, int ns, hipStream_t st, int extras) {
    const FgGrid& G = s->grid;
    FcgInvArgs a = {};
    a.u = v.t1; a.r = v.r; a.rA = rA; a.z = v.z; a.w = v.w;
    a.tw = s->fd_dct_tw; a.rot = s->fd_dct_rot; a.is0 = s->fd_dct_inv[0]; a.is = s->fd_dct_inv[1];
    a.flags = s->flags; a.acc = s->cg_acc; a.ns = ns; a.rows = G.ny; a.it = it; a.env_stride = G.n;
    a.xsum = s->fcg_xsum; a.extras = (extras && it == 0) ? 1 : 0;
    a.hy = G.h[1]; a.rhy = G.rh[1]; a.hx = G.h[0]; a.rhx = G.rh[0]; a.fixed_x = G.fixed[0];
    const dim3 grid((G.ny + 7) / 8, G.B);
    const int slot = fg_prof_slot(s, FG_PK_FCG_INV, s->flags, G.B, 20.0 * G.n, (14.0 + 5.0 * log2((double)G.nx)) * G.n, st);
    if (int rc = (s->fd_dct_x == 2 ? launch_inv<true>(s, slot, G.nx, a, grid, st) : launch_inv<false>(s, slot, G.nx, a, grid, st))) return rc;
    FG_HIP_CHECK(hipGetLastError());
    return FG_OK;
}
int fg_fcg_check0(fg_state* s, fg_real tol, int ns, hipStream_t st, FgPollOut poll, bool* marks_valid) {
    const FgGrid& G = s->grid;
    hipLaunchKernelGGL(k_fcg_check0, dim3((G.B + CHECK_WAVES - 1) / CHECK_WAVES), dim3(64 * CHECK_WAVES), 0, st, s->cg_acc, s->flags, s->info_dev, s->info_pinned, s->fcg_alpha, s->fcg_lazy,
                       tol, G.n, G.B, ns, poll);
    FG_HIP_CHECK(hipGetLastError());
    *marks_valid = true;
    return FG_OK;
}
int fg_fcg_div_fwd(fg_state* s, const FgBounds& bnd, const fg_real* dt, const fg_real* hvec, fg_real* div, int ns, hipStream_t st) {
    const FgGrid& G = s->grid;
    FcgDivArgs a = {};
    a.h = hvec; a.div = div; a.r = s->w[0]; a.x = s->p_result; a.t1 = s->w[3];
    for (int f = 0; f < 4; ++f) a.bvel[f] = bnd.vel[f];
    a.tw = s->fd_dct_tw; a.rot = s->fd_dct_rot; a.fs0 = s->fd_dct_fwd[0]; a.fs = s->fd_dct_fwd[1];
    a.dt = dt; a.acc = s->cg_acc; a.ns = ns; a.rows = G.ny; a.n = G.n;
    a.hx = G.h[0]; a.hy = G.h[1]; a.fixed_x = G.fixed[0];
    const dim3 grid((G.ny + 7) / 8, G.B);
    if (int rc = (s->fd_dct_x == 2 ? launch_div<true>(s, G.nx, a, grid, st) : launch_div<false>(s, G.nx, a, grid, st))) return rc;
    FG_HIP_CHECK(hipGetLastError());
    return FG_OK;
}
#endif
```

### fluidgym_amd/csrc/fg_internal.h

```cpp
#pragma once
#include <hip/hip_runtime.h>
#include <hip/hip_ext.h>
#include <math.h>
#include <stdint.h>
#include <cstring>
#include <string>
#include <type_traits>

#include "../../include/fluidgym_hip.h"

#ifdef FG_REAL_DOUBLE
struct alignas(16) fg_real4 { double x, y, z, w; };
__host__ __device__ __forceinline__ fg_real4 make_fg_real4(double x, double y, double z, double w) { fg_real4 r; r.x = x; r.y = y; r.z = z; r.w = w; return r; }
#define FG_F64 1
#define FG_FMAX fmax
#define FG_FABS fabs
#define FG_SQRT sqrt
#else
typedef float4 fg_real4;
#define make_fg_real4 make_float4
#define FG_F64 0
#define FG_FMAX fmaxf
#define FG_FABS fabsf
#define FG_SQRT sqrtf
// ... 550 lines not shown
    bool cg_for(const fg_real* dt) const { return cg_ns > 0 && cg_dt == dt; }
    void set_cg_start(int form) { cg_start = form; }
    bool take_bicg(int nc, const fg_real* dt) { const bool ready = bicg_nc == nc && bicg_dt == dt; clear(); return ready; }
    int take_cg(int ns, int best, const fg_real* dt) {
        const int got = (cg_ns == ns && cg_best == best && cg_dt == dt) ? cg_start : -1; clear(); return got;
    }
};

struct FgNu {
    fg_real v = 0; const fg_real* per_env = nullptr;
#ifdef __HIPCC__
    __device__ __forceinline__ fg_real at(int b) const { return per_env ? per_env[b] : v; }
#endif
    bool same(const FgNu& o) const { return v == o.v && per_env == o.per_env; }
};

struct fg_state {
    fg_config cfg;
    FgGrid grid;
    int vec;
    fg_real viscosity;
    fg_real scalar_viscosity[FG_MAX_SCALARS];
    bool scalar_viscosity_set;
    const fg_real* viscosity_B;
    const fg_real* scalar_viscosity_B[FG_MAX_SCALARS];
    fg_real* d_h[3];
    fg_real* d_rh[3];
    fg_real* velocity;
    fg_real* pressure;
    fg_real* scalar;
    fg_real* velocity_source;
    fg_real* visc_field;
    fg_real* bvel[6];
    fg_real* bscal[6];
    fg_real* A;
    fg_real* rA;
    fg_real* Coff;
    fg_real* adv_rhs;
    fg_real* vel_result;
    fg_real* hvec;
    fg_real* div;
    fg_real* p_result;
    fg_real* scal_result;
    fg_real* w[8];
    FgDacc* acc;
    int32_t* flags;
    fg_solve_info* info_dev;
    fg_solve_info* info_pinned;
    int32_t* flags_pinned;
    fg_real* scratch_B;
    FgProf prof;
    FgDacc* cg_acc;
    FgBest cg_best;
    int cg_return_best;
    int cg_reset_steps;
    int adv_from_result;
    int adv_precond; long long line_retries;
    int cg_wgs_per_slot;
    int wall_forcing_axis; fg_real wall_forcing_coef[2]; fg_real* force_uniform;
    int reduce_wgs;
    int bicg_sub;
    int bicg3_force, bicg3_bxl, bicg3_mix;
    int bicg_fused;
    int cg_fused, bicg_pfused; double* fcg_alpha; FgDacc* fcg_xsum;
    int32_t* fcg_lazy; int fcg_first;
    int fcg_spec;
    int jac_spec; long jac_spec_missed;
    long jac_floor_released = 0;
    int jac_prefactor;
    int jac_warm;
    long fcg_unstored, fcg_first_polls;
    fg_real* line_inv; fg_real* line_cp;
    fg_real* ilu_d;
    int double_fallback; int ladder_force; long long rung_count[4];
    double* r64_buf; FgDacc* r64_acc;
    int ref64_outer; float ref64_tol, ref64_inner; double* ref64_x; long ref64_corrections;
    float* fd_Qx; float* fd_QxT; float* fd_Qz; float* fd_QzT; float* fd_lower; float* fd_inv; float* fd_cp;
    float* fd_lam; float* helm_diag; float* helm_lower; float* helm_upper; float* helm_tmp;
    float* helm_lower_row; float helm_rs; int helm_cb, helm_rowform_off, helm_cb_pref;
    float* line_inv2; float* line_cp2; float* helm_lower_row2; int helm_pre_mask; const fg_real* helm_pre_dt; FgNu helm_pre_nu[2]; int helm_pre_walls[2][2]; int helm_set;
    int tridiag_cb;
    int fd_dct_x; float2* fd_dct_tw; float2* fd_dct_rot; float fd_dct_fwd[2]; float fd_dct_inv[2];
    float* fd_lam_x; float* fd_row_inv; float* fd_row_cp; float* fd_row_lower; int fd_rowmean; long fd_row_epoch; mutable long rA_epoch;
    int fd_facfuse;
    float* fd_row_part; long fd_row_part_epoch;
    int32_t* forms_rec;
    const fg_real* adv_last_dt;
    fg_real** d_bvel_ptrs;
    fg_real* diag_pinned;
    fg_real* dt_pinned;
    fg_real* dt_dev;
    double* t_rem_dev;
    int dev_dt;
    int pred_bicg[4], pred_cg[4];
    int adv_jacobi, adv_jacobi_env; FgJacHist jac_hist[4]; float* jac_prev;
    int adv_linesweep;
    long long jac_solves, jac_fallbacks;
    long jac_rA_epoch;
    FgCounters ctr;
    const fg_real* cur_dt;
    FgPoll poll;
    mutable int maxvel_clean;
    FgPrepared prepared;
    fg_env_sel* env_sel_dev;
    size_t n_cells() const { return (size_t)grid.n; }
};
inline FgNu fg_nu(const fg_state* s, int for_scalar = 0, int channel = 0) {
    FgNu n;
    if (for_scalar && s->scalar_viscosity_B[channel]) { n.v = s->scalar_viscosity[channel]; n.per_env = s->scalar_viscosity_B[channel]; }
    else if (for_scalar && s->scalar_viscosity_set) n.v = s->scalar_viscosity[channel];
    else { n.v = s->viscosity; n.per_env = s->viscosity_B; }
    return n;
}

void fg_set_error(const std::string& msg);
#define FG_REQUIRE(cond, code, msg)  \
    do {                             \
        if (!(cond)) {               \
            fg_set_error(msg);       \
            return code;             \
        }                            \
    } while (0)
#define FG_HIP_CHECK(expr)                                                                        \
    do {                                                                                          \
        hipError_t _e = (expr);                                                                   \
        if (_e != hipSuccess) {                                                                   \
            fg_set_error(std::string(#expr) + ": " + hipGetErrorString(_e));                      \
            return FG_ERR_HIP;                                                                    \
        }                                                                                         \
    } while (0)

#if FG_F64
#define FG_DISPATCH(s, ...)                                                       \
    do {                                                                          \
        if ((s)->grid.dims == 2) { constexpr int DIMS = 2, VEC = 1; __VA_ARGS__; } \
        else { constexpr int DIMS = 3, VEC = 1; __VA_ARGS__; }                    \
    } while (0)
#else
#define FG_DISPATCH(s, ...)                                                       \
    do {                                                                          \
        if ((s)->grid.dims == 2) {                                                \
            if ((s)->vec == 4) { constexpr int DIMS = 2, VEC = 4; __VA_ARGS__; }  \
            else { constexpr int DIMS = 2, VEC = 1; __VA_ARGS__; }                \
        } else {                                                                  \
            if ((s)->vec == 4) { constexpr int DIMS = 3, VEC = 4; __VA_ARGS__; }  \
            else { constexpr int DIMS = 3, VEC = 1; __VA_ARGS__; }                \
        }                                                                         \
    } while (0)
#endif

struct FgBicgBegin { FgDacc* acc; fg_real* sc; int32_t* flags; fg_solve_info* info; int nc; };
#ifdef __HIPCC__
__device__ __forceinline__ void fg_bicg_begin_sys(const FgBicgBegin& q, const fg_real* __restrict__ dt, int sys) {
    for (int k = 0; k < FG_ACC_DOUBLES; ++k) acc_st(q.acc + ((size_t)sys * FG_ACC_DOUBLES + k), 0.0);
    sc_st(q.sc + (sys * 2), 1.f); sc_st(q.sc + (sys * 2 + 1), 1.f);
    const bool active = (dt == nullptr) || (dt[sys / q.nc] > 0.f);
    flag_st(q.flags + (sys), active ? 0 : 3);
    q.info[sys].final_residual = 0.f;
    q.info[sys].used_iterations = -1;
    q.info[sys].converged = active ? 0 : 1;
    q.info[sys].is_finite = 1;
}
#endif
struct FgAdvArgs {
    const fg_real* vel;
    const fg_real* scal;
    long scal_env_stride;
    const fg_real* source;
    const fg_real* force;
    const fg_real* dt;
    FgNu nu;
    const fg_real* visc;
    int for_scalar;
    int channel, n_scalars;
    fg_real* A; fg_real* Coff; fg_real* rhs;
    fg_real* rA;
    FgBicgBegin begin;
    const fg_real* buoy_T; long buoy_stride; int buoy_axis; fg_real buoy_factor; fg_real* source_w;
    fg_real* row_part;
};
int fg_launch_adv_build(fg_state* s, const FgBounds& bnd, const FgAdvArgs& a, hipStream_t st);
int fg_launch_wall_forcing(const fg_state* s, hipStream_t st);
int fg_launch_sgs(const fg_state* s, const FgBounds& bnd, fg_real coefficient, fg_real* out, hipStream_t st);
int fg_launch_pressure_setup(const fg_state* s, const fg_real* dt, hipStream_t st);
int fg_launch_h(fg_state* s, const fg_real* dt, const fg_real* vel_result, hipStream_t st);
int fg_launch_div(fg_state* s, const FgBounds& bnd, const fg_real* dt, const fg_real* hvec, fg_real* div, hipStream_t st,
                  bool cg_from_zero = false,
                  bool fused_fwd = false);
struct FgMeanRef { const FgDacc* sums; const fg_solve_info* info; fg_real* p_copy; const int32_t* lazy; const double* alpha; };
struct FgLazyRef { const int32_t* lazy; const double* alpha; fg_real* p_res; };
int fg_launch_correct(const fg_state* s, const fg_real* dt, const fg_real* rA, const fg_real* hvec, const fg_real* p,
                      fg_real* vel_out, hipStream_t st, fg_real* vel_copy = nullptr, const FgMeanRef* mean = nullptr, const FgLazyRef* lazy = nullptr);
struct FgDtRule { double* t_rem; fg_real* dt_out; float cfl; double time_step; int reset; };
int fg_launch_max_velocity(const fg_state* s, const FgBounds& bnd, fg_real* out_B, hipStream_t st, fg_real* mirror_B = nullptr,
                           FgPollOut poll = FgPollOut{nullptr, 0}, fg_real* flux_B = nullptr, fg_real* flux_mirror = nullptr,
                           FgDtRule rule = FgDtRule{nullptr, nullptr, 0.f, 0.0, 0});
int fg_launch_flux_balance(const fg_state* s, const FgBounds& bnd, fg_real* out_B, hipStream_t st, FgPollOut poll = FgPollOut{nullptr, 0});
int fg_launch_copy_active(const fg_state* s, const fg_real* dt, const fg_real* src, fg_real* dst, int comps, hipStream_t st);
int fg_launch_buoyancy(const fg_state* s, const fg_real* dt, const fg_real* T, long t_env_stride, fg_real* source, int axis,
                       fg_real factor, hipStream_t st);
int fg_launch_outflow(const fg_state* s, int face, fg_real velm_axis, const fg_real* dt, hipStream_t st);
int fg_launch_balance(const fg_state* s, const FgBounds& bnd, int free_mask, fg_real atol, const fg_real* dt, hipStream_t st,
                      int outflow_mask = 0, const fg_real* outflow_velm = nullptr,
                      const fg_real* dt_host_values = nullptr);
bool fg_outflow_folds(const fg_state* s, int outflow_mask);
int fg_launch_mean_sub(const fg_state* s, const fg_real* active_dt, fg_real* p, fg_real* p_copy, hipStream_t st);

int fg_poisson_apply_launch(const fg_state* s, const fg_real* rA, const fg_real* x, fg_real* y, hipStream_t st);
int fg_poisson_jacobi_launch(const fg_state* s, const fg_real* rA, const fg_real* b, const fg_real* x, fg_real* xnew,
                             fg_real omega, hipStream_t st);
int fg_poisson_rbgs_launch(const fg_state* s, const fg_real* rA, const fg_real* b, fg_real* x, fg_real omega, int color,
                           hipStream_t st);
struct FgCgOutcome {
    const fg_real* lazy_z = nullptr;
    bool mean_ready = false;
    bool marks_valid = false;
    bool spec_done = false;
};
struct FgCgSpec { int (*fn)(void* ctx, const FgCgOutcome& o) = nullptr; void* ctx = nullptr; };
struct FgCgArgs {
    const fg_real* rA; const fg_real* b; fg_real* x;
    fg_real* r; fg_real* p; fg_real* Ap;
    const fg_real* dt;
    fg_real tol; int max_iterations; int use_x0; int reset_steps;
    int check_every;
    int precond;
    int kind = 2;
    int lazy_ok = 0;
    FgCgSpec spec;
};
int fg_cg_solve(fg_state* s, const FgCgArgs& a, fg_solve_info* info_host, hipStream_t st, FgCgOutcome* out = nullptr);

struct FgSpecHook { int (*fn)(void* ctx) = nullptr; void* ctx = nullptr; };
struct FgBicgArgs {
    const fg_real* diag; const fg_real* off;
    const fg_real* rhs; fg_real* x;
    int nc;
    const fg_real* dt;
    fg_real tol; int max_iterations; int use_x0;
    int precond = 0;
    FgNu nu; int wall_lo = 1, wall_hi = 1;
    int kind = 1;
    FgSpecHook spec;
};
int fg_bicgstab_solve(fg_state* s, const FgBicgArgs& a, fg_solve_info* info_host, hipStream_t st, bool* spec_ran = nullptr);
#if !FG_F64
enum FgSweepOutcome {
    FG_SWEEP_NOT_TRIED,
    FG_SWEEP_SOLVED,
    FG_SWEEP_SOLVED_SPEC,
    FG_SWEEP_GAVE_UP,
    FG_SWEEP_SPEC_MISSED,
};
bool fg_jacobi_ok(const fg_state* s, const FgBicgArgs& a);
bool fg_linesweep_ok(const fg_state* s, const FgBicgArgs& a);
int fg_linesweep_solve(fg_state* s, const FgBicgArgs& a, fg_solve_info* info_host, hipStream_t st, FgSweepOutcome* outcome);
int fg_jacobi_solve(fg_state* s, const FgBicgArgs& a, fg_solve_info* info_host, hipStream_t st, FgSweepOutcome* outcome);
#endif
int fg_rung64_bicgstab(fg_state* s, const FgBicgArgs& a, fg_solve_info* info_host, bool all_systems, hipStream_t st);
int fg_rung64_cg(fg_state* s, const FgCgArgs& a, fg_solve_info* info_host, bool all_envs, hipStream_t st, FgCgOutcome* out);

bool fg_zmarch_ok(const fg_state* s, int* zc_out);
int fg_zmarch_apply(const fg_state* s, const fg_real* rA, const fg_real* x, fg_real* y, int zc, hipStream_t st);
int fg_zmarch_relax(const fg_state* s, const fg_real* rA, const fg_real* b, const fg_real* x, fg_real* xnew, fg_real omega,
                    int color, int zc, hipStream_t st);
int fg_zmarch_cg_ap(const fg_state* s, const fg_real* rA, const fg_real* z, const fg_real* p_in, fg_real* p_out, fg_real* Ap,
                    FgDacc* acc, int32_t* flags, fg_solve_info* info, int prof_slot, fg_real tol, int it, int first,
                    int ns, int num_base, int zc, hipStream_t st);
// ... 42 lines not shown
```

### fluidgym_amd/csrc/fg_piso.hip

```cpp
#include "fg_internal.h"
#include "fg_cg.h"
#include "fg_fftcg.h"

namespace {

template <int VEC>
__device__ __forceinline__ fg_real fg_elem_mask(int e, fg_real lo_mask_or_hi, bool is_edge_elem) {
    return is_edge_elem ? lo_mask_or_hi : 1.f;
}

template <int DIMS, int VEC>
__device__ __forceinline__ int fg_slab_index(const FgGrid& g, const FgCtx<DIMS, VEC>& c, int a) {
    if (a == 0) return c.k * g.ny + c.j;
    if (a == 1) return c.k * g.nx + c.i0;
    return c.j * g.nx + c.i0;
}
__device__ __forceinline__ int fg_slab_size(const FgGrid& g, int a) {
    return (a == 0) ? g.ny * g.nz : (a == 1) ? g.nx * g.nz : g.nx * g.ny;
}

template <int DIMS, int VEC, bool SCALAR, bool VISC = false>
__global__ __launch_bounds__(FG_BLOCK) void k_adv_build(FgGrid g, FgBounds bnd, FgAdvArgs a, int tiles_x,
                                                         int tiles_y, int tiles) {
    const FgCtx<DIMS, VEC> c = fg_make_ctx<DIMS, VEC>(g, tiles_x, tiles_y, tiles);
    if (a.begin.acc) {
        if (fg_xcd_remap(blockIdx.x, gridDim.x) % (unsigned)tiles == 0 && (int)threadIdx.x < a.begin.nc)
            fg_bicg_begin_sys(a.begin, a.dt, c.b * a.begin.nc + threadIdx.x);
    }
    const fg_real dt = a.dt[c.b];
    if (!(dt > 0.f) || !c.valid) return;
    const size_t N = g.n;
    const fg_real* __restrict__ vel = a.vel + (size_t)c.b * DIMS * N;
    const FgMetric<DIMS, VEC> m = fg_metrics<DIMS, VEC>(g, c);
    const fg_real nu = a.nu.at(c.b);
    const fg_real rdt = 1.f / dt;

    fg_real J[VEC], diag[VEC], off[2 * DIMS][VEC];
    fg_real bsum[SCALAR ? 1 : DIMS][VEC];
#pragma unroll
    for (int e = 0; e < VEC; ++e) {
        J[e] = m.hx[e] * m.hy * m.hz;
        diag[e] = J[e] * rdt;
#pragma unroll
        for (int q = 0; q < (SCALAR ? 1 : DIMS); ++q) bsum[q][e] = 0.f;
    }
    FgVec<VEC> u[DIMS];

#pragma unroll
    for (int ax = 0; ax < DIMS; ++ax) {
        FgVec<VEC> lo, hi;
        fg_gather_axis<DIMS, VEC>(vel + ax * N, c, ax, u[ax], lo, hi);
        FgVec<VEC> nu_c, nu_lo, nu_hi;
        if constexpr (VISC) fg_gather_axis<DIMS, VEC>(a.visc + (size_t)c.b * N, c, ax, nu_c, nu_lo, nu_hi);
        const int f_lo = 2 * ax, f_hi = 2 * ax + 1;
        const int slab = fg_slab_index<DIMS, VEC>(g, c, ax);
        const int slab_n = fg_slab_size(g, ax);
#pragma unroll
        for (int e = 0; e < VEC; ++e) {
            fg_real area, rh_p, rh_lo, rh_hi, mask_lo, mask_hi;
            if (ax == 0) {
                area = m.hy * m.hz;
                rh_p = m.rhx[e];
                rh_lo = (e == 0) ? m.rhx_m : m.rhx[e > 0 ? e - 1 : 0];
                rh_hi = (e == VEC - 1) ? m.rhx_p : m.rhx[e < VEC - 1 ? e + 1 : VEC - 1];
                mask_lo = (e == 0) ? c.mxm : 1.f;
                mask_hi = (e == VEC - 1) ? c.mxp : 1.f;
            } else if (ax == 1) {
                area = m.hx[e] * m.hz;
                rh_p = m.rhy; rh_lo = m.rhy_m; rh_hi = m.rhy_p;
                mask_lo = c.mym; mask_hi = c.myp;
            } else {
                area = m.hx[e] * m.hy;
                rh_p = m.rhz; rh_lo = m.rhz_m; rh_hi = m.rhz_p;
                mask_lo = c.mzm; mask_hi = c.mzp;
            }
            const fg_real Uc = u[ax].v[e] * area;
            const fg_real al_p = area * rh_p;
            const fg_real nu_p = VISC ? nu_c.v[e] : nu;
            if (mask_lo != 0.f) {
                const fg_real ff = -0.25f * (Uc + lo.v[e] * area);
                fg_real visc;
                if constexpr (VISC) visc = 0.5f * (nu_p * al_p + nu_lo.v[e] * (area * rh_lo));
                else visc = 0.5f * nu * (al_p + area * rh_lo);
                diag[e] += ff + visc;
                off[f_lo][e] = ff - visc;
// ... 61 lines not shown
#define FG_DPP16(x, ctrl) __int_as_float(__builtin_amdgcn_update_dpp(__float_as_int(x), __float_as_int(x), ctrl, 0xf, 0xf, false))
                v += FG_DPP16(v, 0xb1);
                v += FG_DPP16(v, 0x4e);
                v += FG_DPP16(v, 0x124);
                v += FG_DPP16(v, 0x128);
#undef FG_DPP16
                if ((threadIdx.x & 15) == 0) a.row_part[((size_t)c.b * g.ny + c.j) * tiles_x + c.i0 / 64] = v;
            }
        }
#endif
    }
#pragma unroll
    for (int f = 0; f < 2 * DIMS; ++f) {
#pragma unroll
        for (int e = 0; e < VEC; ++e) out.v[e] = off[f][e] * rJ[e];
        fg_store<VEC>(a.Coff + ((size_t)c.b * 2 * DIMS + f) * N + c.idx, out);
    }
    if constexpr (SCALAR) {
        const FgVec<VEC> T = fg_load<VEC>(a.scal + (size_t)c.b * a.scal_env_stride + c.idx);
#pragma unroll
        for (int e = 0; e < VEC; ++e) out.v[e] = (J[e] * T.v[e] * rdt + bsum[0][e]) * rJ[e];
        fg_store<VEC>(a.rhs + (size_t)c.b * N + c.idx, out);
    } else {
#pragma unroll
        for (int q = 0; q < DIMS; ++q) {
            FgVec<VEC> S;
            const bool have_s = a.source != nullptr || a.buoy_T != nullptr;
            if (a.buoy_T) {
                if (q == a.buoy_axis) {
                    S = fg_load<VEC>(a.buoy_T + (size_t)c.b * a.buoy_stride + c.idx);
#pragma unroll
                    for (int e = 0; e < VEC; ++e) S.v[e] = a.buoy_factor * S.v[e];
                } else {
#pragma unroll
                    for (int e = 0; e < VEC; ++e) S.v[e] = 0.f;
                }
                fg_store<VEC>(a.source_w + ((size_t)c.b * DIMS + q) * N + c.idx, S);
            } else if (a.source) S = fg_load<VEC>(a.source + ((size_t)c.b * DIMS + q) * N + c.idx);
            const fg_real F = a.force ? a.force[c.b * DIMS + q] : 0.f;
#pragma unroll
            for (int e = 0; e < VEC; ++e)
                out.v[e] = (J[e] * u[q].v[e] * rdt + bsum[q][e]) * rJ[e] + ((have_s ? S.v[e] : 0.f) + F);
            fg_store<VEC>(a.rhs + ((size_t)c.b * DIMS + q) * N + c.idx, out);
        }
    }
}

__global__ __launch_bounds__(FG_BLOCK) void k_reciprocal(const fg_real* __restrict__ A, fg_real* __restrict__ rA,
                                                          const fg_real* __restrict__ dt, int n, int n4) {
    const int b = blockIdx.y;
    if (dt && !(dt[b] > 0.f)) return;
    const fg_real4* src = reinterpret_cast<const fg_real4*>(A + (size_t)b * n);
    fg_real4* dst = reinterpret_cast<fg_real4*>(rA + (size_t)b * n);
    for (int i = blockIdx.x * blockDim.x + threadIdx.x; i < n4; i += gridDim.x * blockDim.x) {
        const fg_real4 v = src[i];
        dst[i] = make_fg_real4(1.f / v.x, 1.f / v.y, 1.f / v.z, 1.f / v.w);
    }
    if (blockIdx.x == 0) {
        for (int i = n4 * 4 + threadIdx.x; i < n; i += blockDim.x) rA[(size_t)b * n + i] = 1.f / A[(size_t)b * n + i];
    }
}

template <int DIMS, int VEC>
__global__ __launch_bounds__(FG_BLOCK) void k_h(FgGrid g, const fg_real* __restrict__ dt,
                                                 const fg_real* __restrict__ rA_, const fg_real* __restrict__ Coff,
                                                 const fg_real* __restrict__ rhs, const fg_real* __restrict__ velr,
                                                 fg_real* __restrict__ hvec, FgCgBegin begin, int tiles_x, int tiles_y, int tiles) {
    const FgCtx<DIMS, VEC> c = fg_make_ctx<DIMS, VEC>(g, tiles_x, tiles_y, tiles);
    if (begin.acc && fg_xcd_remap(blockIdx.x, gridDim.x) % (unsigned)tiles == 0) fg_cg_begin_env(begin, dt, c.b);
    if (!(dt[c.b] > 0.f) || !c.valid) return;
    const size_t N = g.n;
    const FgVec<VEC> rA = fg_load<VEC>(rA_ + (size_t)c.b * N + c.idx);
    FgVec<VEC> off[2 * DIMS];
#pragma unroll
    for (int f = 0; f < 2 * DIMS; ++f) off[f] = fg_load<VEC>(Coff + ((size_t)c.b * 2 * DIMS + f) * N + c.idx);
#pragma unroll
    for (int q = 0; q < DIMS; ++q) {
        const size_t base = ((size_t)c.b * DIMS + q) * N;
        const FgNbr<DIMS, VEC> u = fg_gather<DIMS, VEC>(velr + base, c);
        const FgVec<VEC> r = fg_load<VEC>(rhs + base + c.idx);
        FgVec<VEC> out;
#pragma unroll
        for (int e = 0; e < VEC; ++e) {
            fg_real H = off[0].v[e] * u.xm.v[e] + off[1].v[e] * u.xp.v[e] + off[2].v[e] * u.ym.v[e] +
                      off[3].v[e] * u.yp.v[e];
            if constexpr (DIMS == 3) H += off[4].v[e] * u.zm.v[e] + off[5].v[e] * u.zp.v[e];
            out.v[e] = rA.v[e] * (r.v[e] - H);
        }
        fg_store<VEC>(hvec + base + c.idx, out);
    }
}

template <int DIMS, int VEC>
__global__ __launch_bounds__(FG_BLOCK) void k_div(FgGrid g, FgBounds bnd, const fg_real* __restrict__ dt,
                                                   const fg_real* __restrict__ hvec, fg_real* __restrict__ div, FgCgStart start,
                                                   int tiles_x, int tiles_y, int tiles) {
    const FgCtx<DIMS, VEC> c = fg_make_ctx<DIMS, VEC>(g, tiles_x, tiles_y, tiles);
    if (dt && !(dt[c.b] > 0.f)) return;
    if (!c.valid && !start.acc) return;
    const size_t N = g.n;
    const FgMetric<DIMS, VEC> m = fg_metrics<DIMS, VEC>(g, c);
    fg_real acc[VEC];
#pragma unroll
    for (int e = 0; e < VEC; ++e) acc[e] = 0.f;
#pragma unroll
    for (int ax = 0; ax < DIMS; ++ax) {
        FgVec<VEC> ctr, lo, hi;
        fg_gather_axis<DIMS, VEC>(hvec + ((size_t)c.b * DIMS + ax) * N, c, ax, ctr, lo, hi);
        const int slab = fg_slab_index<DIMS, VEC>(g, c, ax);
        const int slab_n = fg_slab_size(g, ax);
#pragma unroll
        for (int e = 0; e < VEC; ++e) {
            fg_real area, mask_lo, mask_hi;
            if (ax == 0) { area = m.hy * m.hz; mask_lo = (e == 0) ? c.mxm : 1.f; mask_hi = (e == VEC - 1) ? c.mxp : 1.f; }
            else if (ax == 1) { area = m.hx[e] * m.hz; mask_lo = c.mym; mask_hi = c.myp; }
            else { area = m.hx[e] * m.hy; mask_lo = c.mzm; mask_hi = c.mzp; }
            const int bi = slab + ((ax == 0) ? 0 : e);
            fg_real F_hi, F_lo;
            if (mask_hi != 0.f) F_hi = 0.5f * (ctr.v[e] + hi.v[e]) * area;
            else F_hi = bnd.vel[2 * ax + 1][((size_t)c.b * DIMS + ax) * slab_n + bi] * area;
            if (mask_lo != 0.f) F_lo = 0.5f * (ctr.v[e] + lo.v[e]) * area;
            else F_lo = bnd.vel[2 * ax][((size_t)c.b * DIMS + ax) * slab_n + bi] * area;
            acc[e] += F_hi - F_lo;
        }
    }
    FgVec<VEC> out;
#pragma unroll
    for (int e = 0; e < VEC; ++e) out.v[e] = acc[e];
    if (c.valid) fg_store<VEC>(div + (size_t)c.b * N + c.idx, out);
    if (start.acc) {
        __shared__ fg_real lds[4];
        fg_real part[1] = {0.f};
        if (c.valid) {
            FgVec<VEC> z;
#pragma unroll
            for (int e = 0; e < VEC; ++e) { z.v[e] = 0.f; part[0] += out.v[e] * out.v[e]; }
            fg_store<VEC>(start.x + (size_t)c.b * N + c.idx, z);
            fg_store<VEC>(start.r + (size_t)c.b * N + c.idx, out);
        }
        fg_block_sum<1>(part, lds);
        if (threadIdx.x == 0) {
            const unsigned tile = fg_xcd_remap(blockIdx.x, gridDim.x) % tiles;
            fg_acc_add(fg_acc_ptr(start.acc, c.b, 0), start.ns, tile, (double)part[0]);
        }
    }
}

template <int DIMS, int VEC>
__global__ __launch_bounds__(FG_BLOCK) void k_correct(FgGrid g, const fg_real* __restrict__ dt,
                                                       const fg_real* __restrict__ rA_, const fg_real* __restrict__ hvec,
                                                       const fg_real* __restrict__ p, fg_real* __restrict__ vel_out,
                                                       fg_real* __restrict__ vel_copy, FgMeanRef mean, FgLazyRef lazy, int tiles_x, int tiles_y, int tiles) {
    const FgCtx<DIMS, VEC> c = fg_make_ctx<DIMS, VEC>(g, tiles_x, tiles_y, tiles);
    if ((dt && !(dt[c.b] > 0.f)) || !c.valid) return;
    const size_t N = g.n;
    const FgMetric<DIMS, VEC> m = fg_metrics<DIMS, VEC>(g, c);
    const FgVec<VEC> rA = fg_load<VEC>(rA_ + (size_t)c.b * N + c.idx);
    FgNbr<DIMS, VEC> P = fg_gather<DIMS, VEC>(p + (size_t)c.b * N, c);
    if (lazy.lazy) {
        const bool on = lazy.lazy[c.b] == 1;
        const fg_real sc = on ? (fg_real)lazy.alpha[2 * c.b] : (fg_real)0;
        auto scale = [&](FgVec<VEC>& v) {
#pragma unroll
            for (int e = 0; e < VEC; ++e) v.v[e] = on ? sc * v.v[e] : (fg_real)0;
        };
        scale(P.c); scale(P.xm); scale(P.xp); scale(P.ym); scale(P.yp);
        if constexpr (DIMS == 3) { scale(P.zm); scale(P.zp); }
        if (lazy.p_res) fg_store<VEC>(lazy.p_res + (size_t)c.b * N + c.idx, P.c);
    }
    if (mean.sums) {
// ... 523 lines not shown
                for (int q = 0; q < DIMS; ++q) diff[q] += (up ? 1.f : -1.f) * u[(size_t)q * g.n + n];
            }
        }
#pragma unroll
        for (int q = 0; q < DIMS; ++q) grad[q][a] = diff[q] / dist * g.rh[a][pos[a]];
    }
    fg_real d = 0.f;
#pragma unroll
    for (int i = 0; i < DIMS; ++i)
#pragma unroll
        for (int j = i; j < DIMS; ++j) {
            fg_real sij = 0.5f * (grad[i][j] + grad[j][i]);
            sij *= sij;
            d += (i != j) ? 2.f * sij : sij;
        }
    out[(size_t)b * g.n + c] = coefficient * delta * FG_SQRT(2.f * d);
}

__global__ __launch_bounds__(1024) void k_wall_forcing(FgGrid g, const fg_real* __restrict__ vel, int axis, fg_real coef_lo, fg_real coef_hi,
                                                        fg_real* __restrict__ force, int dims) {
    const int b = blockIdx.x;
    const size_t N = g.n;
    const fg_real* __restrict__ u = vel + ((size_t)b * dims + axis) * N;
    double lo = 0.0, hi = 0.0;
    const int rows = g.nz;
    for (int idx = threadIdx.x; idx < rows * g.nx; idx += blockDim.x) {
        const int k = idx / g.nx, i = idx - k * g.nx;
        lo += (double)u[((size_t)k * g.ny + 0) * g.nx + i];
        hi += (double)u[((size_t)k * g.ny + (g.ny - 1)) * g.nx + i];
    }
    __shared__ double lds[2][16];
#pragma unroll
    for (int o = 32; o > 0; o >>= 1) { lo += __shfl_down(lo, o, 64); hi += __shfl_down(hi, o, 64); }
    if ((threadIdx.x & 63) == 0) { lds[0][threadIdx.x >> 6] = lo; lds[1][threadIdx.x >> 6] = hi; }
    __syncthreads();
    if (threadIdx.x == 0) {
        double sl = 0.0, sh = 0.0;
        for (int w = 0; w < (int)(blockDim.x >> 6); ++w) { sl += lds[0][w]; sh += lds[1][w]; }
        const double n = (double)rows * g.nx;
        const fg_real tau_lo = coef_lo * (fg_real)(sl / n), tau_hi = coef_hi * (fg_real)(sh / n);
        for (int q = 0; q < dims; ++q) force[b * dims + q] = (q == axis) ? (fg_real)0.5 * (tau_lo + tau_hi) : (fg_real)0;
    }
}

int fg_launch_wall_forcing(const fg_state* s, hipStream_t st) {
    hipLaunchKernelGGL(k_wall_forcing, dim3(s->grid.B), dim3(1024), 0, st, s->grid, (const fg_real*)s->velocity, s->wall_forcing_axis,
                       s->wall_forcing_coef[0], s->wall_forcing_coef[1], s->force_uniform, s->grid.dims);
    FG_HIP_CHECK(hipGetLastError());
    return FG_OK;
}

int fg_launch_sgs(const fg_state* s, const FgBounds& bnd, fg_real coefficient, fg_real* out, hipStream_t st) {
    const dim3 grid((s->grid.n + FG_BLOCK - 1) / FG_BLOCK, s->grid.B);
    if (s->grid.dims == 2) hipLaunchKernelGGL(k_sgs_smagorinsky<2>, grid, dim3(FG_BLOCK), 0, st, s->grid, bnd, (const fg_real*)s->velocity, coefficient, out);
    else hipLaunchKernelGGL(k_sgs_smagorinsky<3>, grid, dim3(FG_BLOCK), 0, st, s->grid, bnd, (const fg_real*)s->velocity, coefficient, out);
    FG_HIP_CHECK(hipGetLastError());
    return FG_OK;
}

int fg_launch_pressure_setup(const fg_state* s, const fg_real* dt, hipStream_t st) {
    const int n = s->grid.n;
    hipLaunchKernelGGL(k_reciprocal, stride_grid(s, n), dim3(FG_BLOCK), 0, st, s->A, s->rA, dt, n, (n % 4 == 0) ? n / 4 : 0);
    FG_HIP_CHECK(hipGetLastError());
    return FG_OK;
}

int fg_launch_h(fg_state* s, const fg_real* dt, const fg_real* vel_result, hipStream_t st) {
    fg_htrace("h_launch_in");
    FgCgBegin begin;
    begin.acc = s->cg_acc; begin.flags = s->flags; begin.info = s->info_dev; begin.mean_sums = s->acc; begin.best = s->cg_best;
    begin.track_best = s->cg_return_best; begin.ns = fg_cg_slots(s); begin.xsum = s->fcg_xsum;
    s->prepared.set_cg(begin.ns, begin.track_best, dt);
    const int slot_h = fg_prof_slot(s, FG_PK_H, nullptr, s->grid.B, (s->grid.dims == 3 ? 68.0 : 52.0) * (double)s->grid.n, 6.0 * s->grid.dims * s->grid.dims * (double)s->grid.n, st);
    FG_DISPATCH(s, {
        const FgLaunch L = fg_launch_geometry<DIMS, VEC>(s->grid);
        FG_LAUNCH_P(s, slot_h, (k_h<DIMS, VEC>), L.grid, dim3(FG_BLOCK), 0, st, s->grid, dt, s->rA, s->Coff, s->adv_rhs,
                    vel_result, s->hvec, begin, L.tiles_x, L.tiles_y, L.tiles);
    });
    FG_HIP_CHECK(hipGetLastError());
    fg_htrace("h_launch_out");
    return FG_OK;
}

int fg_launch_div(fg_state* s, const FgBounds& bnd, const fg_real* dt, const fg_real* hvec, fg_real* div,
                  hipStream_t st, bool cg_from_zero, bool fused_fwd) {
    FgCgStart start = {nullptr, nullptr, nullptr, 1};
    s->prepared.set_cg_start(0);
    if (cg_from_zero && dt != nullptr && s->prepared.cg_for(dt) && div == s->div) {
#if !FG_F64
        if (fused_fwd && fg_fcg_ok(s)) {
            s->prepared.set_cg_start(2);
            return fg_fcg_div_fwd(s, bnd, dt, hvec, div, s->prepared.cg_ns, st);
        }
#endif
        start.acc = s->cg_acc; start.r = s->w[0]; start.x = s->p_result; start.ns = s->prepared.cg_ns;
        s->prepared.set_cg_start(1);
    }
    const int slot_d = fg_prof_slot(s, FG_PK_DIV, nullptr, s->grid.B, 28.0 * (double)s->grid.n, 4.0 * s->grid.dims * (double)s->grid.n, st);
    FG_DISPATCH(s, {
        const FgLaunch L = fg_launch_geometry<DIMS, VEC>(s->grid);
        FG_LAUNCH_P(s, slot_d, (k_div<DIMS, VEC>), L.grid, dim3(FG_BLOCK), 0, st, s->grid, bnd, dt, hvec, div, start, L.tiles_x,
                    L.tiles_y, L.tiles);
    });
    FG_HIP_CHECK(hipGetLastError());
    return FG_OK;
}

int fg_launch_correct(const fg_state* s, const fg_real* dt, const fg_real* rA, const fg_real* hvec, const fg_real* p,
                      fg_real* vel_out, hipStream_t st, fg_real* vel_copy, const FgMeanRef* mean, const FgLazyRef* lazy) {
    fg_htrace("correct_in");
    const FgMeanRef mr = mean ? *mean : FgMeanRef{nullptr, nullptr, nullptr, nullptr, nullptr};
    const FgLazyRef lz = lazy ? *lazy : FgLazyRef{nullptr, nullptr, nullptr};
    const double cb = (s->grid.dims == 3 ? 36.0 : 28.0) + (vel_copy ? 4.0 * s->grid.dims : 0.0) + ((mean && mean->sums) || (lazy && lazy->p_res) ? 4.0 : 0.0);
    const int slot_c = fg_prof_slot(s, FG_PK_CORRECT, nullptr, s->grid.B, cb * (double)s->grid.n, 5.0 * s->grid.dims * (double)s->grid.n, st);
    FG_DISPATCH(s, {
        const FgLaunch L = fg_launch_geometry<DIMS, VEC>(s->grid);
        FG_LAUNCH_P(s, slot_c, (k_correct<DIMS, VEC>), L.grid, dim3(FG_BLOCK), 0, st, s->grid, dt, rA, hvec, p, vel_out, vel_copy, mr, lz,
                    L.tiles_x, L.tiles_y, L.tiles);
    });
    FG_HIP_CHECK(hipGetLastError());
    fg_htrace("correct_out");
    return FG_OK;
}

int fg_launch_max_velocity(const fg_state* s, const FgBounds& bnd, fg_real* out_B, hipStream_t st, fg_real* mirror_B, FgPollOut poll,
                           fg_real* flux_B, fg_real* flux_mirror, FgDtRule rule) {
    FG_REQUIRE(!rule.t_rem || (poll.gran && mirror_B && !FG_F64), FG_ERR_INVALID_ARG, "the device-side sub-step rule needs the result-word form");
    FG_REQUIRE(!flux_B || (mirror_B && flux_mirror), FG_ERR_INVALID_ARG, "the flux balance rides in the mirrored form only");
    int32_t* done_B = reinterpret_cast<int32_t*>(out_B + s->grid.B);
    FG_REQUIRE(!mirror_B || out_B == s->scratch_B + s->grid.B, FG_ERR_INVALID_ARG, "mirror needs the scratch row as out_B");
    if (!mirror_B || !s->maxvel_clean)
        FG_HIP_CHECK(hipMemsetAsync(out_B, 0, mirror_B ? sizeof(fg_real) * s->grid.B + sizeof(int32_t) * (s->grid.B + 1) : sizeof(fg_real) * s->grid.B, st));
    s->maxvel_clean = mirror_B ? 1 : 0;
    if ((s->grid.nx & 3) == 0) {
        const int rows = s->grid.ny * s->grid.nz;
        int rpb = 4;
        while ((long)((rows + 2 * rpb - 1) / (2 * rpb)) * s->grid.B >= 2048) rpb *= 2;
        while ((rows + rpb - 1) / rpb > (int)fg_reduce_wgs(s)) rpb *= 2;
        dim3 grid((rows + rpb - 1) / rpb, s->grid.B);
        const int slot_m = fg_prof_slot(s, FG_PK_MAXVEL, nullptr, s->grid.B, 4.0 * s->grid.dims * (double)s->grid.n, 2.0 * s->grid.dims * (double)s->grid.n, st);
        if (s->grid.dims == 2)
            FG_LAUNCH_P(s, slot_m, k_max_velocity_rows<2>, grid, dim3(FG_BLOCK), 0, st, s->grid, bnd, s->velocity, out_B, done_B,
                        mirror_B, rpb, poll, flux_B, flux_mirror, rule);
        else
            FG_LAUNCH_P(s, slot_m, k_max_velocity_rows<3>, grid, dim3(FG_BLOCK), 0, st, s->grid, bnd, s->velocity, out_B, done_B,
                        mirror_B, rpb, poll, flux_B, flux_mirror, rule);
        FG_HIP_CHECK(hipGetLastError());
        return FG_OK;
    }
    dim3 grid = stride_grid(s, (long)s->grid.n * 4);
    if (s->grid.dims == 2)
        hipLaunchKernelGGL(k_max_velocity<2>, grid, dim3(FG_BLOCK), 0, st, s->grid, bnd, s->velocity, out_B, done_B, mirror_B, poll, flux_B, flux_mirror, rule);
    else
        hipLaunchKernelGGL(k_max_velocity<3>, grid, dim3(FG_BLOCK), 0, st, s->grid, bnd, s->velocity, out_B, done_B, mirror_B, poll, flux_B, flux_mirror, rule);
    FG_HIP_CHECK(hipGetLastError());
    return FG_OK;
}

int fg_launch_flux_balance(const fg_state* s, const FgBounds& bnd, fg_real* out_B, hipStream_t st, FgPollOut poll) {
    if (s->grid.dims == 2)
        hipLaunchKernelGGL(k_flux_balance<2>, dim3(s->grid.B), dim3(FG_BLOCK), 0, st, s->grid, bnd, out_B, poll);
    else
        hipLaunchKernelGGL(k_flux_balance<3>, dim3(s->grid.B), dim3(FG_BLOCK), 0, st, s->grid, bnd, out_B, poll);
    FG_HIP_CHECK(hipGetLastError());
    return FG_OK;
}
// ... 74 lines not shown
```

### fluidgym_amd/native.py

```python
from __future__ import annotations

import ctypes
import os
from typing import Dict, List, Optional, Sequence

import numpy as np
import torch

from . import _lib as L


def _ptr(t: Optional[torch.Tensor]):
    return None if t is None else ctypes.c_void_p(t.data_ptr())


def _stream(device) -> ctypes.c_void_p:
    return ctypes.c_void_p(torch.cuda.current_stream(device).cuda_stream)


class LinsolveError(RuntimeError):
    """A linear solve failed (reference: ``PISOtorch_diff.LinsolveError``, PISOtorch_diff.py:262)."""


class NativeSolver:
# ... 105 lines not shown
        for f in range(2 * self.dims):
            if self.fixed[f]:
                self.set_boundary_velocity(f, z(self.B, self.dims, *self.slab(f)))
                if self.n_scalars:
                    self.set_boundary_scalar(f, z(self.B, self.n_scalars, *self.slab(f)))

    def set_velocity(self, t):
        self.velocity = t
        self.bind(L.FG_VELOCITY, t)

    def set_pressure(self, t):
        self.pressure = t
        self.bind(L.FG_PRESSURE, t)

    def set_scalar(self, t):
        self.scalar = t
        self.bind(L.FG_SCALAR, t)

    def set_velocity_source(self, t):
        self.velocity_source = t
        self.bind(L.FG_VELOCITY_SOURCE, t)

    def set_viscosity_field(self, t: Optional[torch.Tensor]):
        self.viscosity_field = t
        self.bind(L.FG_VISCOSITY_FIELD, t)

    def sgs_smagorinsky(self, coefficient: float, out: Optional[torch.Tensor] = None) -> torch.Tensor:
        if out is None:
            out = torch.empty((self.B,) + tuple(self.spatial), dtype=self.dtype, device=self.device)
        L.check(self.lib.fg_sgs_smagorinsky(self.handle, float(coefficient), _ptr(out), _stream(self.device)), lib=self.lib)
        return out

    def set_boundary_velocity(self, face, t):
        self.bvel[face] = t
        self.bind(L.FG_BOUND_VELOCITY + face, t)

    def set_boundary_scalar(self, face, t):
        self.bscal[face] = t
        self.bind(L.FG_BOUND_SCALAR + face, t)

    def _per_env(self, v, what: str) -> Optional[torch.Tensor]:
        if isinstance(v, (int, float)):
            return None
        t = (v.detach() if isinstance(v, torch.Tensor) else torch.as_tensor(np.asarray(v, dtype=np.float64))).reshape(-1)
        if t.numel() == 1:
            return None
        if t.numel() != self.B:
            raise ValueError(f"{what}: expected one value or one per env ({self.B}), got {t.numel()}")
        return t.to(device=self.device, dtype=self.dtype).contiguous()

    def set_viscosity(self, nu):
        per_env = self._per_env(nu, "set_viscosity")
        if per_env is None:
            self.viscosity = float(torch.as_tensor(nu).reshape(-1)[0]) if not isinstance(nu, (int, float)) else float(nu)
            L.check(self.lib.fg_set_viscosity(self.handle, self.viscosity), lib=self.lib)
        else:
            self.viscosity = None
        self.viscosity_B = per_env
        L.check(self.lib.fg_set_viscosity_batch(self.handle, _ptr(per_env)), lib=self.lib)

    def set_scalar_viscosity(self, ch: int, k):
        per_env = self._per_env(k, "set_scalar_viscosity")
        if per_env is None:
            kf = float(torch.as_tensor(k).reshape(-1)[0]) if not isinstance(k, (int, float)) else float(k)
            self.scalar_viscosities[int(ch)] = kf
            L.check(self.lib.fg_set_scalar_viscosity(self.handle, ch, kf), lib=self.lib)
        self.scalar_viscosities_B[int(ch)] = per_env
        L.check(self.lib.fg_set_scalar_viscosity_batch(self.handle, ch, _ptr(per_env)), lib=self.lib)

    def dt_tensor(self, dt) -> torch.Tensor:
        if isinstance(dt, torch.Tensor) and dt.is_cuda:
            return dt
        self._dt_host.copy_(torch.as_tensor(np.broadcast_to(np.asarray(dt, dtype=self._np_real), (self.B,)).copy()))
        self._dt.copy_(self._dt_host, non_blocking=True)
        return self._dt

    def buffer(self, which: int, shape) -> torch.Tensor:
        p, n = ctypes.c_void_p(), ctypes.c_int64()
        L.check(self.lib.fg_get_buffer(self.handle, which, ctypes.byref(p), ctypes.byref(n)), lib=self.lib)
        out = torch.empty(int(n.value), dtype=self.dtype, device=self.device)
        L.check(self.lib.fg_read_buffer(self.handle, which, _ptr(out), _stream(self.device)), lib=self.lib)
        return out.view(*shape)

    def _infos(self, n):
        return (L.FgSolveInfo * n)()

    def max_velocity(self) -> torch.Tensor:
        L.check(self.lib.fg_max_velocity(self.handle, _ptr(self._out_B), _stream(self.device)), lib=self.lib)
        return self._out_B.clone()

    def boundary_flux_balance(self) -> torch.Tensor:
        L.check(self.lib.fg_boundary_flux_balance(self.handle, _ptr(self._out_B), _stream(self.device)), lib=self.lib)
        return self._out_B.clone()

    def step_diagnostics(self):
        buf = np.empty(2 * self.B, dtype=self._np_real)
        L.check(self.lib.fg_step_diagnostics(self.handle, buf.ctypes.data_as(ctypes.POINTER(self._c_real)),
                                             _stream(self.device)))
        return buf[: self.B], buf[self.B:]

    def update_advective_boundary(self, face: int, velm, dt):
        v = np.ascontiguousarray(velm, dtype=self._np_real).reshape(-1)
        L.check(self.lib.fg_update_advective_boundary(self.handle, face, v.ctypes.data_as(ctypes.POINTER(self._c_real)),
                                                      _ptr(self.dt_tensor(dt)), _stream(self.device)))

    def balance_boundary_fluxes(self, free_faces, atol: float, dt):
        mask = 0
        for f in free_faces:
            mask |= 1 << int(f)
        L.check(self.lib.fg_balance_boundary_fluxes(self.handle, mask, float(atol), _ptr(self.dt_tensor(dt)),
                                                    _stream(self.device)))

    def setup_advection(self, dt, for_scalar=False, channel=0):
        L.check(self.lib.fg_setup_advection(self.handle, _ptr(self.dt_tensor(dt)), int(for_scalar), channel,
                                            _stream(self.device)))

    def solve_advection(self, for_scalar=False, channel=0, tol=1e-5, max_iterations=5000) -> List[L.FgSolveInfo]:
        n = self.B * (1 if for_scalar else self.dims)
        info = self._infos(n)
        rc = self.lib.fg_solve_advection(self.handle, int(for_scalar), channel, tol, max_iterations, info,
                                         _stream(self.device))
        L.check(rc, allow=(L.FG_ERR_NOT_CONVERGED, L.FG_ERR_NOT_FINITE))
        return list(info)

    def copy_scalar_result_to_blocks(self, channel=0):
        L.check(self.lib.fg_copy_scalar_result_to_blocks(self.handle, channel, _stream(self.device)), lib=self.lib)

    def setup_pressure_matrix(self):
        L.check(self.lib.fg_setup_pressure_matrix(self.handle, _stream(self.device)), lib=self.lib)

    def setup_pressure_rhs(self, dt):
        L.check(self.lib.fg_setup_pressure_rhs(self.handle, _ptr(self.dt_tensor(dt)), _stream(self.device)), lib=self.lib)

    def solve_pressure(self, tol=1e-5, max_iterations=5000, method=None, use_previous=False):
        method = self.default_method if method is None else method
        info = self._infos(self.B)
        rc = self.lib.fg_solve_pressure(self.handle, method, tol, max_iterations, int(use_previous), info,
                                        _stream(self.device))
        L.check(rc, allow=(L.FG_ERR_NOT_CONVERGED, L.FG_ERR_NOT_FINITE))
        return list(info)

    def correct_velocity(self):
        L.check(self.lib.fg_correct_velocity(self.handle, _stream(self.device)), lib=self.lib)

    def copy_velocity_result_to_blocks(self):
        L.check(self.lib.fg_copy_velocity_result_to_blocks(self.handle, _stream(self.device)), lib=self.lib)

    def copy_velocity_result_from_blocks(self):
        L.check(self.lib.fg_copy_velocity_result_from_blocks(self.handle, _stream(self.device)), lib=self.lib)

    def piso_step(self, dt, corrector_steps=2, advect_scalar=True, advection_tol=1e-5, pressure_tol=1e-5,
                  max_iterations=5000, buoyancy_axis=-1, buoyancy_factor=0.0, method=None,
                  pressure_warm_start=False):
        method = self.default_method if method is None else method
        opt = self._StepOptions(corrector_steps, int(advect_scalar), method, max_iterations, advection_tol,
                              pressure_tol, buoyancy_axis, buoyancy_factor, int(pressure_warm_start))
        stats = (ctypes.c_int32 * 4)()
        rc = self.lib.fg_piso_step(self.handle, _ptr(self.dt_tensor(dt)), ctypes.byref(opt), stats,
                                   _stream(self.device))
        if rc == L.FG_ERR_NOT_FINITE:
            raise LinsolveError("linear solve produced a non-finite residual")
        L.check(rc, allow=(L.FG_ERR_NOT_CONVERGED,))
        return rc == L.FG_OK, list(stats)

    def _sim_options(self, time_step, cfl, adaptive=True, substeps=1, flux_balance_tol=1e-5, outflow_faces=(),
                     outflow_velm=(0.0, 0.0, 0.0), outflow_tol=1e-5, corrector_steps=2, advect_scalar=True,
                     advection_tol=1e-5, pressure_tol=1e-5, max_iterations=5000, buoyancy_axis=-1, buoyancy_factor=0.0,
                     method=None, pressure_warm_start=False, max_substeps=1000):
        method = self.default_method if method is None else method
        o = self._SimOptions()
        o.step = self._StepOptions(corrector_steps, int(advect_scalar), method, max_iterations, advection_tol, pressure_tol,
                                 buoyancy_axis, buoyancy_factor, int(pressure_warm_start))
        o.time_step, o.cfl, o.adaptive, o.substeps = float(time_step), float(cfl), int(adaptive), int(substeps)
        o.flux_balance_tol = float(flux_balance_tol)
        mask = 0
        for f in outflow_faces:
            mask |= 1 << int(f)
        o.outflow_mask = mask
        for i in range(3):
            o.outflow_velm[i] = float(outflow_velm[i]) if i < len(outflow_velm) else 0.0
        o.outflow_tol = float(outflow_tol)
        o.max_substeps = int(max_substeps)
        return o

    def single_step(self, time_step, cfl, adaptive=True, substeps=1, flux_balance_tol=1e-5, outflow_faces=(),
                    outflow_velm=(0.0, 0.0, 0.0), outflow_tol=1e-5, corrector_steps=2, advect_scalar=True,
                    advection_tol=1e-5, pressure_tol=1e-5, max_iterations=5000, buoyancy_axis=-1, buoyancy_factor=0.0,
                    method=None, pressure_warm_start=False, max_substeps=1000):
        o = self._sim_options(time_step, cfl, adaptive, substeps, flux_balance_tol, outflow_faces, outflow_velm, outflow_tol, corrector_steps,
                              advect_scalar, advection_tol, pressure_tol, max_iterations, buoyancy_axis, buoyancy_factor, method,
                              pressure_warm_start, max_substeps)
        out = (ctypes.c_int32 * 6)()
        flux = (self._c_real * self.B)()
        rc = self.lib.fg_single_step(self.handle, ctypes.byref(o), out, flux, _stream(self.device))
        if rc == L.FG_ERR_FLUX_BALANCE:
            raise RuntimeError(
                "Domain boundary fluxes not balanced, cannot proceed with simulation step. "
                f"Flux balance: {list(flux)}, flux_balance_tol: {flux_balance_tol}")
        if rc == L.FG_ERR_NOT_FINITE:
            raise LinsolveError("linear solve produced a non-finite residual")
        L.check(rc)
        return bool(out[5]), [int(out[i]) for i in range(4)], int(out[4])

    def multi_step(self, n, time_step, cfl, boundary_schedule=None, **kw):
        o = self._sim_options(time_step, cfl, **kw)
        sched = None
        if boundary_schedule:
            sched = (ctypes.c_void_p * (6 * n))()
            for face, t in boundary_schedule.items():
                assert t.shape[0] == n and t[0].is_contiguous() and t.dtype == self.dtype and t.device == self.device
                base, step_bytes = t.data_ptr(), t.stride(0) * t.element_size()
                for k in range(n):
                    sched[6 * k + int(face)] = base + k * step_bytes
        out = (ctypes.c_int32 * (6 * n))()
        flux = (self._c_real * self.B)()
# ... 193 lines not shown
```

### include/fluidgym_hip.h

```cpp
#ifndef FLUIDGYM_HIP_H
#define FLUIDGYM_HIP_H

#include <stdint.h>

#ifdef __cplusplus
extern "C" {
#endif

#define FG_ABI_VERSION 1

#ifdef FG_REAL_DOUBLE
typedef double fg_real;
#else
typedef float fg_real;
#endif
#define FG_MAX_SCALARS 4

#define FG_OK 0
#define FG_ERR_INVALID_ARG (-1)
#define FG_ERR_NOT_BOUND (-2)
#define FG_ERR_HIP (-3)
#define FG_ERR_UNSUPPORTED (-4)
#define FG_ERR_NOT_CONVERGED (-5)
#define FG_ERR_NOT_FINITE (-6)
// ... 98 lines not shown
#define FG_FORM_TRI_F64 6
#define FG_FORM_FAC_GRID 1
#define FG_FORM_FAC_ROWMEAN 2
#define FG_FORM_FAC_MADE 3
#define FG_FORM_HELM_ARRAY 1
#define FG_FORM_HELM_ROW32 2
#define FG_FORM_HELM_ROW64 3
#define FG_FORM_LINE_LDS 1
#define FG_FORM_LINE_STREAM 2
int fg_set_fd_helmholtz(fg_handle h, const float* lam_host);
int fg_advection_retries(fg_handle h, int64_t* out, int32_t reset);
int fg_set_double_fallback(fg_handle h, int on);
int fg_set_advection_jacobi(fg_handle h, int on);
int fg_advection_jacobi_counts(fg_handle h, int64_t* out2);
int fg_ladder(fg_handle h, int64_t* out4, int32_t force_mask);
int fg_advection_solver_form(fg_handle h, int nc, int32_t* out);
int fg_copy_scalar_result_to_blocks(fg_handle h, int channel, void* stream);
int fg_setup_pressure_matrix(fg_handle h, void* stream);
int fg_setup_pressure_rhs(fg_handle h, const fg_real* dt_B, void* stream);
int fg_solve_pressure(fg_handle h, int method, fg_real tol, int max_iterations, int use_previous,
                      fg_solve_info* info_host, void* stream);
int fg_set_pressure_refinement(fg_handle h, int32_t max_corrections, fg_real target_tol, fg_real inner_relative_tol);
int fg_correct_velocity(fg_handle h, void* stream);
int fg_copy_velocity_result_to_blocks(fg_handle h, void* stream);
int fg_copy_velocity_result_from_blocks(fg_handle h, void* stream);

typedef struct fg_step_options {
    int32_t corrector_steps;
    int32_t advect_scalar;
    int32_t pressure_method;
    int32_t max_iterations;
    fg_real advection_tol;
    fg_real pressure_tol;
    int32_t buoyancy_axis;
    fg_real buoyancy_factor;
    int32_t pressure_warm_start;
} fg_step_options;
int fg_piso_step(fg_handle h, const fg_real* dt_B, const fg_step_options* opt, int32_t* stats_host,
                 void* stream);
int fg_solver_counters(fg_handle h, int64_t* out13_host, int32_t reset);
int fg_solver_unconverged(fg_handle h, int64_t* out4_host);
typedef struct fg_sim_options {
    fg_step_options step;
    fg_real time_step;
    fg_real cfl;
    int32_t adaptive;
    int32_t substeps;
    fg_real flux_balance_tol;
    int32_t outflow_mask;
    fg_real outflow_velm[3];
    fg_real outflow_tol;
    int32_t max_substeps;
} fg_sim_options;
int fg_single_step(fg_handle h, const fg_sim_options* opt, int32_t* out_host_6, fg_real* flux_balance_host,
                   void* stream);
int fg_multi_step(fg_handle h, const fg_sim_options* opt, int32_t n, const fg_real* const* bvel_schedule, int32_t* out_host_6n,
                  fg_real* flux_balance_host, int32_t* steps_done, void* stream);
int fg_make_divergence_free(fg_handle h, fg_real tol, int max_iterations, fg_solve_info* info_host,
                            void* stream);

enum fg_buffer {
    FG_BUF_A = 0,
    FG_BUF_C_OFF = 1,
    FG_BUF_ADV_RHS = 2,
    FG_BUF_VEL_RESULT = 3,
    FG_BUF_H = 4,
    FG_BUF_DIV = 5,
    FG_BUF_P_RESULT = 6,
    FG_BUF_SCALAR_RESULT = 7
};
int fg_reset_solver_state(fg_handle h, void* stream);
int fg_solver_hints(fg_handle h, int32_t* hints12, int32_t set);

typedef struct fg_env_sel {
    int32_t env, src;
    int32_t flip_x, flip_z;
    int32_t shift_x, shift_z;
} fg_env_sel;
int fg_env_restore_field(fg_handle h, int which_field, const fg_real* bank, int32_t S, const fg_env_sel* sel, int32_t n_sel,
                         int32_t signed_components, void* stream);
int fg_env_reset_solver_state(fg_handle h, const fg_env_sel* sel, int32_t n_sel, void* stream);
int fg_get_buffer(fg_handle h, int which, fg_real** out_ptr, int64_t* out_count);
int fg_read_buffer(fg_handle h, int which, fg_real* dst, void* stream);

int fg_poisson_apply(fg_handle h, const fg_real* rA, const fg_real* x, fg_real* y, void* stream);
int fg_poisson_jacobi(fg_handle h, const fg_real* rA, const fg_real* b, fg_real* x, int n_sweeps, fg_real omega,
                      void* stream);
int fg_poisson_rbgs(fg_handle h, const fg_real* rA, const fg_real* b, fg_real* x, int n_sweeps, fg_real omega,
                    void* stream);
int fg_poisson_cg(fg_handle h, const fg_real* rA, const fg_real* b, fg_real* x, fg_real tol, int max_iterations,
                  int use_x0, fg_solve_info* info_host, void* stream);
int fg_poisson_fdcg(fg_handle h, const fg_real* rA, const fg_real* b, fg_real* x, fg_real tol, int max_iterations,
                    int use_x0, fg_solve_info* info_host, void* stream);

int fg_stream_triad(float* a, const float* b, const float* c, float scalar, int64_t n, int32_t reps, float* ms_per_launch, void* stream);
int fg_coherence_litmus(int32_t atomic_access, int32_t nsys, int32_t cells, int32_t iterations, int64_t* bad_reads, double* bad_value,
                        void* stream);
int fg_dacc_host_sum(const double* values, int64_t n, double plain, double* out_sum);
int fg_dacc_device_sum(const double* values_host, int64_t n, double plain, int32_t reps, double* out_sums_host, void* stream);
#define FG_FIELD_SUMMARY_WORK_BYTES 128
int fg_field_summary(const fg_real* field, int32_t batch, int32_t channels, int64_t n, int32_t channel, void* workspace,
                     double* moments, int64_t* counts, double lo, double width, int32_t nbins, uint64_t* hist, void* stream);
int fg_plane_moments(const fg_real* const* channels, const int64_t* batch_stride, int32_t K, int32_t batch, int32_t nz, int32_t ny,
                     int32_t nx, int32_t order, double* n, double* mean, double* central, uint64_t* tickets, void* stream);
int fg_plane_timecorr(const fg_real* const* channels, const int64_t* batch_stride, int32_t K, int32_t batch, int32_t nz, int32_t ny,
                      int32_t nx, int32_t lags, int32_t n_slots, const int32_t* slot_lag, fg_real* base, double* base_ss, double* acc,
                      void* stream);
int fg_mb_cell_moments(const fg_real* velocity, const fg_real* pressure, int32_t dims, int32_t batch, int64_t n_cells,
                       const int64_t* block_table, int32_t n_blocks, int64_t samples, double* mean, double* central, void* stream);
int fg_mb_cell_moments_widths(const fg_real* velocity, const fg_real* pressure, int64_t n_cells, const int64_t* block_table,
                              int32_t n_blocks, const double* mean, const double* central, int32_t* widths);
int fg_plane_budgets(const fg_real* const* fields, const int64_t* batch_stride, int32_t n_fields, int32_t batch, int32_t nz, int32_t ny,
                     int32_t nx, const double* x, const double* y, const double* z, int32_t wrap_x, int32_t wrap_z, double* n,
                     double* mean, double* central, uint64_t* tickets, void* stream);
int fg_plane_spectra(const fg_real* const* channels, const int64_t* batch_stride, int32_t K, int32_t batch, int32_t nz, int32_t ny,
                     int32_t nx, const int32_t* planes, int32_t n_planes, double* amp, double* power, void* stream);
int fg_profile_enable(fg_handle h, int on);
int fg_profile_kinds(void);
const char* fg_profile_kind_name(int kind);
int fg_profile_read(fg_handle h, int kind, double* ms_sum, int64_t* samples, double* bytes_sum, double* flops_sum,
                    double* full_ms_sum, double* full_bytes_sum, int64_t* full_samples, int64_t* launches,
                    double* all_ms_sum, int64_t* all_samples);

int fg_sparse_apply_ell(const int32_t* idx, const float* w, int32_t rows, int32_t K, const float* x, int64_t n, int32_t m, float* y,
                        void* stream);
int fg_sparse_apply_csr(const int32_t* indptr, const int32_t* col, const float* val, int32_t rows, const float* x, int64_t n, int32_t m,
                        float* y, void* stream);
typedef struct fg_resampler_state* fg_resampler;
int fg_resampler_create(int dims, const int32_t* n_src, const int32_t* n_out, const int32_t* base_cat,
                        const float* frac_cat, int quirk3d, int device, fg_resampler* out);
int fg_resampler_destroy(fg_resampler r);
int fg_resample(fg_resampler r, const float* src, int batch, int channels, float* dst, int fill_max_steps,
                void* stream);

int fg_envglue_jet_schedule(const float* target, const float* current, const float* decay, const float* shape, int32_t n,
                            int32_t batch, int32_t nx, float* jets, float* last, void* stream);
int fg_envglue_channel_observe(const float* velocity, const float* pressure, const int64_t* sensor, int32_t n_sensors,
                               int32_t batch, int32_t ny, int32_t nx, float shear_scale, float penalty, float* obs_velocity,
                               float* obs_pressure, float* cross, float* shear, float* reward, void* stream);
int fg_envglue_channel_observe_batch(const float* velocity, const float* pressure, const int64_t* sensor, int32_t n_sensors,
                                     int32_t batch, int32_t ny, int32_t nx, const float* shear_scale_B, float penalty,
                                     float* obs_velocity, float* obs_pressure, float* cross, float* shear, float* reward,
                                     void* stream);

typedef struct fg_mb_state* fg_mb_handle;
int fg_mb_create(int32_t dims, int32_t batch, int32_t device, fg_mb_handle* out);
int fg_mb_destroy(fg_mb_handle h);
int fg_mb_add_block(fg_mb_handle h, const fg_real* vertex_coords_host, int32_t nx, int32_t ny, int32_t nz, int32_t* block_id);
int fg_mb_connect(fg_mb_handle h, int32_t block1, int32_t face1, int32_t block2, int32_t face2, int32_t axis1, int32_t axis2);
int fg_mb_make_periodic(fg_mb_handle h, int32_t block, int32_t axis);
int fg_mb_set_reference_quirks(fg_mb_handle h, int32_t connected_diagonal_offset, int32_t first_layer_rule);
int fg_mb_set_nonortho_flags(fg_mb_handle h, int32_t flags);
int fg_mb_finalize(fg_mb_handle h);
int fg_mb_sizes(fg_mb_handle h, int32_t* n_cells, int32_t* n_boundary_faces);
int fg_mb_block_info(fg_mb_handle h, int32_t block, int32_t* cell_offset, int32_t* boundary_slot0 );
int fg_mb_get_neighbors(fg_mb_handle h, int32_t* out_host );
int fg_mb_get_host_table(fg_mb_handle h, int32_t which, void* out, int64_t* count);
int fg_mb_bind(fg_mb_handle h, fg_real* velocity, fg_real* pressure_result, fg_real* boundary_velocity, const fg_real* source);
int fg_mb_set_viscosity(fg_mb_handle h, fg_real nu);
int fg_mb_set_viscosity_batch(fg_mb_handle h, const fg_real* nu_B);
typedef struct fg_mb_step_options {
    int32_t corrector_steps;
    int32_t advect_non_ortho_steps;
    int32_t pressure_non_ortho_steps;
    int32_t max_iterations;
    fg_real advection_tol;
// ... 88 lines not shown
```

### profiles/gen_switch_table.py

```python
import os
import re
import sys

ROOT = os.path.dirname(os.path.dirname(os.path.abspath(__file__)))

NOTES = {
    "FG_CG_FUSED": ("bits", "1 (default): three-launch preconditioned pressure CG on 2-D fast-transform grids (fg_fftcg.hip); 0: the five kernels"),
    "FG_BICG_PFUSED": ("bits", "1 (default): six-launch Helmholtz-preconditioned BiCGStab (fg_fftbicg.hip); 0: eleven launches per iteration"),
    "FG_BICG_FUSED": ("bits", "1 (default): two-kernel BiCGStab iteration in 2-D; 0: five kernels; 2: two kernels in 3-D bricks too"),
    "FG_BICG_SUB": ("no", "envs per sub-batch of the 2-D two-kernel BiCGStab (unset: by working set; 0: never)"),
    "FG_BICG3": ("bits", "z-marching 3-D BiCGStab: 0 never, N always with z-chunk N (tests), unset by the rule"),
    "FG_BICG3_BXL": ("no", "tile lanes along x of the z-marching BiCGStab (16 / 32)"),
    "FG_BICG3_MIX": ("bits", "debugging: bit 0 kernel a, bit 1 kernel b as z-march, bit 2 keep the init kernel"),
    "FG_REDUCE_WGS": ("no", "workgroups per env of the reduction kernels (0 = rule)"),
    "FG_HELM_ROWFORM": ("bits", "0: Helmholtz factors through k_helm_coeffs + the array-form line kernels (IEEE division instead of v_rcp)"),
    "FG_ADV_LINESWEEP": ("bits", "1: the advection-diffusion systems of the Helmholtz-preconditioned family (wall-refined 2-D grids: RBC) go to line sweeps x <- (D + O_y)^-1 (b - O_x x) first (k_line_sweep_y, fg_linepre.hip), BiCGStab takes what they do not settle; 0 (default): the preconditioned BiCGStab always -- measured on the RBC leg: 16-17 sweeps per velocity solve at the bench state's sub-step, 775 against 793 env-steps/s"),
    "FG_FD_FACFUSE": ("no", "1 (default): the first tridiagonal solve after 1/A changed makes the per-env row-mean factors itself (k_tridiag_y_lds<.., FAC>: same arithmetic, same bits); 0: k_fd_rowmean_factor as a launch of its own (A/B runs)"),
    "FG_FD_ROWMEAN": ("bits", "1 (default): the fused pressure CG is preconditioned by the row-mean operator (per-env factors, one factorisation per PISO step); 0: the grid's A = 1 factors"),
    "FG_ADV_JACOBI": ("bits", "velocity systems of uniform 2-D grids: 1 Jacobi sweeps first (fg_jacobi.hip), 0 BiCGStab always; unset = what fg_set_advection_jacobi says (the Simulation turns it on: policy advection_jacobi)"),
    "FLUIDGYM_AMD_ADVECTION_JACOBI": ("policy", "policy advection_jacobi (default 1): the Simulation asks for the Jacobi sweeps of fg_jacobi.hip on the grids that qualify"),
    "FLUIDGYM_AMD_PRESSURE_REFINEMENT": ("bits", "policy pressure_refinement (default 0 = off): up to N mixed-precision corrections behind every single-block pressure solve (fp64 residual, fp32 corrections: fg_set_pressure_refinement) -- an accuracy mode"),
    "FLUIDGYM_AMD_MULTI_STEP": ("no", "0: the sim steps of an env step are issued one by one from Python instead of through fg_multi_step (A/B runs; same bits)"),
    "FG_FCG_FIRST": ("bits", "1 (default): the fused CG judges its first iterate from I'(0)'s dot products (k_fcg_check0) and stores no pressure when every env ends there; 0: the verdict on the updated residual (A/B runs, tests)"),
    "FG_JAC_WARM": ("bits", "start vector of the Jacobi sweeps of a step's velocity systems: 1 the block velocity, 0 the BiCGStab start vector (zero on the non-orthogonal branch); unset: the block velocity on on-chip grids of 2^17 cells and more (where it saves a pass)"),
    "FG_JAC_PREFACTOR": ("no", "0: the row-mean factors of the pressure preconditioner are made in front of the first tridiagonal solve instead of behind the sweeps' check kernel (A/B runs)"),
    "FG_FCG_SPEC": ("no", "0: the corrector waits for the verdict on the first iterate instead of being launched behind the verdict kernel (A/B runs)"),
    "FG_JAC_SPEC": ("no", "0: k_h and the divergence kernel of the first corrector wait for the verdict on the velocity sweeps instead of being launched behind the check kernel (A/B runs)"),
    "FG_JAC_XCD": ("no", "0: the on-chip Jacobi regions in launch order instead of one XCD per run of an env's regions (A/B runs)"),
    "FG_JAC_SHAPE": ("bits", "A/B runs of the Jacobi sweeps: 1 full-row regions only, 2 bands only (unset: the cheaper of the two for the grid)"),
    "FG_JAC_SWEEPS": ("bits", "A/B runs: sweeps per pass of the Jacobi sweeps (unset: 4 / 6 / 8 for full rows, 8 / 12 for bands, by region depth)"),
    "FG_ROCTX": ("no", "1: named roctx ranges around the phases of a step (fg_single_step, scalar / velocity assembly and solve, pressure correctors; mb_velocity_solve, mb_pressure_solve) for rocprofv3 --marker-trace; the library is dlopen'ed, off by default"),
    "FG_HTRACE": ("no", "1: host time stamps around the polls and the launches behind them (fg_poll.hip), per-pair averages printed at exit"),
    "FG_FORCE_ZMARCH": ("bits", "z-march chunk length of the 3-D Poisson kernels (tests on small grids; -1 = brick kernels)"),
    "FG_ZMARCH_SB": ("no", "single-barrier ring of the z-march kernels: bit per mode, 0 never, unset = rule"),
    "FG_POLL_SPIN": ("no", "0: host polls wait with hipStreamSynchronize instead of spinning on pinned sequence words"),
    "FG_POLL_WORDS": ("no", "0: polled verdicts through the host-pinned mirror + a system-scope release (one L2 write-back per verdict kernel) instead of travelling in the 8-byte result words the host spins on (A/B runs: 8 790 against 9 600 env-steps/s on the headline, one lane)"),
    "FG_DEV_DT": ("no", "0: fg_single_step waits for the CFL maxima and computes the adaptive sub-steps on the host before the PISO step, instead of the CFL kernel's last workgroup taking them on the device (FgDtRule: same doubles, same bits) and the host reading the maxima after the step (A/B runs)"),
    "FLUIDGYM_AMD_F64_FD": ("bits", "0: the fp64 library solves the pressure systems with the reference's plain CG instead of the CG preconditioned by the fast-diagonalisation operator in doubles (csrc/fg_f64_fd.hip; A/B runs: iterations per solve)"),
    "FLUIDGYM_AMD_ENV_GLUE": ("bits", "0: ChannelJet2D's action schedule and reward / observation as elementwise torch launches instead of the two native kernels of fg_envglue.hip (A/B runs; the schedule is bit-identical, the means differ by fp32 rounding of the summation order)"),
    "FLUIDGYM_AMD_LANES": ("no", "default of ParallelFluidEnv(lanes=...): sub-batches of a rank's env batch, each its own solver handle, stepped concurrently by that many host threads on their own HIP streams (1 = one batch; bench.py passes --lanes 2).  Same bits per env as the sub-batches stepped alone"),
    "FG_PROF_PERIOD": ("no", "sampling period of the live kernel timing (64)"),
    "FG_FD_NO_FFT": ("bits", "1: the x basis change of the FD preconditioner as dense GEMM instead of the row FFT (tests)"),
    "FG_MB_BICG_VEC4": ("no", "bit per multi-block BiCGStab kernel: four-cell form (31 = all)"),
    "FG_MB_BICG_FUSE": ("bits", "multi-block BiCGStab: 0 five kernels, 1 s/t fused, 2 (default) also p/v"),
    "FG_MB_ML_FUSE": ("bits", "multilevel BiCGStab forms p / s inside the restriction: 0 never, 1 up to 32 systems, 2 always"),
    "FG_MB_ML_TRY_CAP": ("policy", "iteration cap of an attempt of the multilevel trial (200; tests force 2)"),
    "FG_MB_TRACE": ("no", "residual / verification trace of the pressure BiCGStab on stderr"),
    "FG_MB_TRACE_FAIL": ("no", "recurrence words of a system that ends non-finite"),
    "FG_MB_COMPACT": ("no", "0: every multi-block Krylov launch covers all systems of the batch"),
    "FG_MB_OC_RTG_NT": ("bits", "register-resident on-chip CG with a global residual copy on 16-24 k-cell meshes instead of k_mbc_l2"),
    "FG_MB_ONCHIP": ("bits", "0: no whole-solve on-chip CG (chunked CG kernels)"),
    "FG_MB_OC_AGG": ("bits", "0: cell-ordered on-chip CG instead of the aggregate-owned one"),
    "FG_MB_CLUSTER": ("bits", "pressure CG of an env by a cluster of four workgroups (fg_mb_cluster.hip): 0 never (the one-workgroup kernels), 1 (default) meshes beyond 8 k cells, 2 every mesh its tables fit (tests)"),
    "FG_MB_CL_JACOBI": ("bits", "0: the velocity sweeps of the meshes the cluster CG takes stay one launch per sweep (k_mbj_sweep_env) instead of one launch per solve by the clusters (k_mbj_cluster; A/B runs: 2 552 against 3 045 env-steps/s on the cylinder mesh)"),
    "FG_MB_CL_HALF": ("bits", "0: meshes whose rows of the coarse inverse do not fit LDS as fp32 stream them from L2 instead of holding them as fp16 (A/B runs: 19.7 against 16.8 us per iteration on 23 k cells)"),
    "FG_MB_CL_MAXCL": ("no", "cap on the clusters of one launch of the cluster CG (tests: envs beyond it queue inside the kernel; same bits)"),
    "FG_MB_CL_NEAR": ("no", "0: granule stores of the cluster CG always write through (sc1), also when a cluster's workgroups reported one XCD (A/B runs: 10.0 against 8.6 us per iteration)"),
    "FG_MB_OC_VARIANT": ("no", "on-chip CG variant bits (fences / coefficient layout)"),
    "FG_MB_RUNG_ILU": ("bits", "0: column-scaled preconditioned rung instead of ILU(0)"),
    "FLUIDGYM_AMD_LIB": ("no", "path of libfluidgym_hip.so (sanitizer build: tests/run_sanitizer_suite.sh)"),
    "FLUIDGYM_AMD_LIB_F64": ("no", "path of libfluidgym_hip_f64.so"),
    "FLUIDGYM_AMD_ADVECTION_FD_PRECONDITIONER": ("bits", "policy advection_fd_preconditioner: auto (2-D periodic-x grids) / always / never"),
    "FLUIDGYM_AMD_ADVECTION_LINE_PRECONDITIONER": ("bits", "policy advection_line_preconditioner (off)"),
    "FLUIDGYM_AMD_ADVECTION_RUNG_PRECONDITIONER": ("bits", "preconditioner of the BiCG_precondition_fallback rung: line / ilu"),
    "FLUIDGYM_AMD_ADVECTION_WARM_START": ("policy", "1: velocity solve starts from the current velocity in both branches (reference: branch rule)"),
    "FLUIDGYM_AMD_PRESSURE_WARM_START": ("policy", "1: pressure solves start from the previous pressure (reference: zero)"),
    "FLUIDGYM_AMD_PRESSURE_STALL_ACCEPT": ("policy", "accept a stalled pressure solve within a factor of the tolerance (off)"),
    "FLUIDGYM_AMD_PRESSURE_MULTILEVEL": ("bits", "multilevel preconditioner of the multi-block pressure CG"),
    "FLUIDGYM_AMD_PRESSURE_MULTILEVEL_BICGSTAB": ("bits", "multilevel trial of the airfoil's refined BiCGStab"),
    "FLUIDGYM_AMD_PRESSURE_MULTILEVEL_FP64": ("bits", "policy pressure_multilevel_fp64 (default 0): float64 cylinder / airfoil envs on 2-D meshes install the multilevel preconditioner in the fp64 build (kernel-form preconditioned CG, unfused BiCGStab trial) instead of the plain recurrences"),
    "FG_MB_PCG_KERNEL": ("bits", "1 (fp32 build, debugging): the multilevel-preconditioned pressure CG as the kernel-form loop of mb_cg (five launches per iteration: what the fp64 build runs) instead of the on-chip / cluster kernels; 0 (default)"),
    "FLUIDGYM_AMD_PRESSURE_BICGSTAB_LARGE_MESHES": ("bits", "3-D multi-block ids take the refined BiCGStab"),
    "FLUIDGYM_AMD_NATIVE_WALL_FORCING": ("bits", "policy native_wall_forcing: the TCF forcing hook runs inside the library"),
    "FLUIDGYM_COLLECTIVE_TIMEOUT_S": ("no", "timeout of ParallelFluidEnv's process group (600 s)"),
    "FLUIDGYM_FORCE_COLLECTIVES": ("no", "ParallelFluidEnv issues its collectives at world size 1 too (tests)"),
    "FLUIDGYM_MASTER_PORT": ("no", "rendezvous port of the reference-style ParallelFluidEnv(cuda_ids=...) entry"),
    "FLUIDGYM_DATA_PATH": ("no", "local data path (initial domains), as config.update('local_data_path', ...)"),
}
IGNORE = {"RANK", "WORLD_SIZE", "LOCAL_RANK", "MASTER_ADDR", "MASTER_PORT", "HSA_ENABLE_IPC_MODE_LEGACY", "PYTHONPATH", "OMP_NUM_THREADS",
          "OPENBLAS_NUM_THREADS", "MKL_NUM_THREADS", "TMPDIR", "GRAFT_REPO_ROOT"}


def scan():
    found = {}
    for base, _, files in os.walk(os.path.join(ROOT, "fluidgym_amd")):
        if "_san" in base or "_f64" in base or "_var" in base or "__pycache__" in base:
            continue
        for fn in files:
            if not fn.endswith((".hip", ".h", ".py")):
                continue
            path = os.path.join(base, fn)
            rel = os.path.relpath(path, ROOT)
            for no, line in enumerate(open(path, errors="replace"), 1):
                for m in re.finditer(r'getenv\("([A-Z][A-Z0-9_]+)"\)', line):
                    found.setdefault(m.group(1), []).append(f"{rel}:{no}")
                for m in re.finditer(r'environ(?:\.get)?[\[(]\s*"([A-Z][A-Z0-9_]+)"', line):
                    found.setdefault(m.group(1), []).append(f"{rel}:{no}")
    return {k: v for k, v in found.items() if k not in IGNORE}


# ... 40 lines not shown
```

Baseline: 9512 env-steps/s.

## Fuse H operator, divergence, CG start and forward transform into one row kernel

Adds k_fcg_hdiv_fwd, which computes the H vector, the divergence of H, the CG begin-state reset and the first forward transform in one row kernel, replacing separate k_h and k_fcg_div_fwd launches on fused-CG grids. It is on by default through FG_HDIV_FUSED and used whenever the solve starts from zero with the fused forward path. The intent is to remove one launch and the write and re-read of hvec between the two kernels, at the cost of computing halo rows redundantly, a larger LDS footprint, and an extra wave per block. Shared helpers keep the arithmetic bit-identical, and debug write_buffer and pressure_rhs entry points are added for testing.

```diff
diff --git a/fluidgym_amd/_lib.py b/fluidgym_amd/_lib.py
--- a/fluidgym_amd/_lib.py
+++ b/fluidgym_amd/_lib.py
@@ -183,6 +183,8 @@
     "fg_set_pressure_refinement": (c_int, [c_void_p, c_int32, c_float, c_float]),
     "fg_get_buffer": (c_int, [c_void_p, c_int, POINTER(c_void_p), POINTER(c_int64)]),
     "fg_read_buffer": (c_int, [c_void_p, c_int, c_void_p, c_void_p]),
+    "fg_write_buffer": (c_int, [c_void_p, c_int, c_void_p, c_void_p]),
+    "fg_debug_pressure_rhs": (c_int, [c_void_p, c_int, c_int, c_void_p]),
     "fg_poisson_apply": (c_int, [c_void_p, c_void_p, c_void_p, c_void_p, c_void_p]),
     "fg_poisson_jacobi": (c_int, [c_void_p, c_void_p, c_void_p, c_void_p, c_int, c_float, c_void_p]),
     "fg_poisson_rbgs": (c_int, [c_void_p, c_void_p, c_void_p, c_void_p, c_int, c_float, c_void_p]),
diff --git a/fluidgym_amd/csrc/fg_api.hip b/fluidgym_amd/csrc/fg_api.hip
--- a/fluidgym_amd/csrc/fg_api.hip
+++ b/fluidgym_amd/csrc/fg_api.hip
@@ -126,6 +126,7 @@
     s->helm_cb_pref = 32;
     { const char* ev = getenv("FG_HELM_ROWFORM"); s->helm_rowform_off = (ev && atoi(ev) == 0) ? 1 : 0; }
     { const char* ev = getenv("FG_FD_FACFUSE"); s->fd_facfuse = ev ? atoi(ev) : 1; }
+    { const char* ev = getenv("FG_HDIV_FUSED"); s->hdiv_fused = ev ? atoi(ev) : 1; }
     { const char* ev = getenv("FG_DEV_DT"); s->dev_dt = ev ? atoi(ev) : 1; }
     { const char* ev = getenv("FG_ADV_LINESWEEP"); s->adv_linesweep = ev ? atoi(ev) : 0; }
     { const char* ev = getenv("FG_FD_ROWMEAN"); s->fd_rowmean = ev ? atoi(ev) : 1; }
@@ -143,6 +144,13 @@
     FG_HIP_CHECK(hipMemset(s->fcg_xsum, 0, sizeof(FgDacc) * 2 * (size_t)g.B));
     FG_HIP_CHECK(hipMalloc(&s->fcg_lazy, sizeof(int32_t) * (size_t)g.B));
     FG_HIP_CHECK(hipMemset(s->fcg_lazy, 0, sizeof(int32_t) * (size_t)g.B));
+    s->hdiv_launches = 0; s->hdiv_part = nullptr; s->hdiv_ticket = nullptr;
+#if !FG_F64
+    FG_HIP_CHECK(hipMalloc(&s->hdiv_part, sizeof(uint32_t) * 64 * (size_t)g.B));
+    FG_HIP_CHECK(hipMemset(s->hdiv_part, 0, sizeof(uint32_t) * 64 * (size_t)g.B));
+    FG_HIP_CHECK(hipMalloc(&s->hdiv_ticket, sizeof(int32_t) * (size_t)g.B));
+    FG_HIP_CHECK(hipMemset(s->hdiv_ticket, 0, sizeof(int32_t) * (size_t)g.B));
+#endif
     { const char* e = getenv("FG_FCG_FIRST"); s->fcg_first = (e && atoi(e) == 0) ? 0 : 1; }
     { const char* e = getenv("FG_JAC_SPEC"); s->jac_spec = (e && atoi(e) == 0) ? 0 : 1; }
     { const char* e = getenv("FG_FCG_SPEC"); s->fcg_spec = (e && atoi(e) == 0) ? 0 : 1; }
@@ -177,6 +185,7 @@
     for (float* p : fd) if (p) (void)hipFree(p);
     if (s->fd_dct_tw) { (void)hipFree(s->fd_dct_tw); (void)hipFree(s->fd_dct_rot); }
     (void)hipFree(s->cg_acc); (void)hipFree(s->fcg_alpha); (void)hipFree(s->fcg_xsum); (void)hipFree(s->fcg_lazy);
+    (void)hipFree(s->hdiv_part); (void)hipFree(s->hdiv_ticket);
     if (s->jac_prev) (void)hipHostFree(s->jac_prev);
     (void)hipFree(s->fd_row_part); (void)hipFree(s->fd_lam_x); (void)hipFree(s->fd_row_inv); (void)hipFree(s->fd_row_cp); (void)hipFree(s->fd_row_lower);
     (void)hipFree(s->line_inv); (void)hipFree(s->line_cp); (void)hipFree(s->ilu_d);
@@ -564,13 +573,18 @@
     return fg_launch_div(s, make_bounds(s, 0), dt_B, s->hvec, s->div, st);
 }
 
+extern "C" int fg_debug_pressure_rhs(fg_handle s, int method, int pressure_warm_start, void* stream) {
+    FG_REQUIRE(s && s->cur_dt, FG_ERR_INVALID_ARG, "fg_debug_pressure_rhs: needs a velocity fg_setup_advection first");
+    if (int rc = check_bound(s, false)) return rc;
+    return fg_launch_h_div(s, make_bounds(s, 0), s->cur_dt, (hipStream_t)stream, !pressure_warm_start, method == FG_SOLVER_FDCG && s->fd_Qx != nullptr);
+}
+
 struct SpecH { fg_state* s; const fg_real* dt; const fg_step_options* opt; hipStream_t st; };
 static int spec_h(void* p) {
     const SpecH* c = static_cast<const SpecH*>(p);
     fg_state* s = c->s;
-    if (int rc = fg_launch_h(s, c->dt, s->vel_result, c->st)) return rc;
-    return fg_launch_div(s, make_bounds(s, 0), c->dt, s->hvec, s->div, c->st, !c->opt->pressure_warm_start,
-                         c->opt->pressure_method == FG_SOLVER_FDCG && s->fd_Qx != nullptr);
+    return fg_launch_h_div(s, make_bounds(s, 0), c->dt, c->st, !c->opt->pressure_warm_start,
+                           c->opt->pressure_method == FG_SOLVER_FDCG && s->fd_Qx != nullptr);
 }
 
 static int launch_corrector(fg_state* s, const fg_real* dt, const FgCgOutcome& o, bool last, hipStream_t st) {
@@ -766,9 +780,8 @@
         FgRange range_corr(c == 0 ? "pressure_corrector_0" : "pressure_corrector_1+");
         const bool last = (c + 1 == opt->corrector_steps);
         if (!(c == 0 && h_div_ran)) {
-            if (int rc = fg_launch_h(s, dt_B, s->vel_result, st)) return rc;
-            if (int rc = fg_launch_div(s, make_bounds(s, 0), dt_B, s->hvec, s->div, st, !opt->pressure_warm_start,
-                                       opt->pressure_method == FG_SOLVER_FDCG && s->fd_Qx != nullptr))
+            if (int rc = fg_launch_h_div(s, make_bounds(s, 0), dt_B, st, !opt->pressure_warm_start,
+                                         opt->pressure_method == FG_SOLVER_FDCG && s->fd_Qx != nullptr))
                 return rc;
         }
         SpecCorrect spec_ctx = {s, dt_B, last, st};
@@ -795,11 +808,13 @@
         "\"FG_BICG3_BXL\": %d, \"FG_BICG3_MIX\": %d, \"FG_REDUCE_WGS\": %d, \"FG_CG_WGS_PER_SLOT\": %d, \"FG_TRIDIAG_CB\": %d, \"FG_HELM_CB\": %d, "
         "\"FG_HELM_ROWFORM\": %d, \"FG_FD_ROWMEAN\": %d, \"FG_POLL_SPIN\": %d, \"FG_PROF_PERIOD\": %d, \"fast_transform_x\": %d, \"fd_preconditioner\": %d, "
         "\"helmholtz\": %d, \"advection_preconditioner\": %d, \"advection_from_result\": %d, \"return_best\": %d, \"cg_reset_steps\": %d, "
-        "\"double_fallback\": %d, \"wall_forcing_axis\": %d, \"FG_ADV_JACOBI\": %d, \"FG_FCG_FIRST\": %d, \"FG_JAC_WARM\": %d, \"first_iterate_polls\": %ld, \"unstored_pressure_solves\": %ld, \"FG_JAC_SPEC\": %d, \"FG_FCG_SPEC\": %d, \"jacobi_speculation_misses\": %ld, \"jacobi_floor_released\": %ld, \"pressure_refinement_corrections\": %ld}",
+        "\"double_fallback\": %d, \"wall_forcing_axis\": %d, \"FG_ADV_JACOBI\": %d, \"FG_FCG_FIRST\": %d, \"FG_JAC_WARM\": %d, \"first_iterate_polls\": %ld, \"unstored_pressure_solves\": %ld, \"FG_JAC_SPEC\": %d, \"FG_FCG_SPEC\": %d, \"jacobi_speculation_misses\": %ld, \"jacobi_floor_released\": %ld, \"pressure_refinement_corrections\": %ld, "
+        "\"FG_HDIV_FUSED\": %d, \"hdiv_fused_launches\": %ld}",
         FG_F64 ? "f64" : "f32", s->cg_fused, s->bicg_pfused, s->bicg_fused, s->bicg_sub, s->bicg3_force, s->bicg3_bxl, s->bicg3_mix, s->reduce_wgs,
         s->cg_wgs_per_slot, s->tridiag_cb, s->helm_cb_pref, s->helm_rowform_off ? 0 : 1, s->fd_rowmean, s->poll.spin, s->prof.period, s->fd_dct_x, s->fd_Qx ? 1 : 0,
         s->fd_lam ? 1 : 0, s->adv_precond, s->adv_from_result, s->cg_return_best, s->cg_reset_steps, s->double_fallback, s->wall_forcing_axis, s->adv_jacobi, s->fcg_first, s->jac_warm,
-        s->fcg_first_polls, s->fcg_unstored, s->jac_spec, s->fcg_spec, s->jac_spec_missed, s->jac_floor_released, s->ref64_corrections);
+        s->fcg_first_polls, s->fcg_unstored, s->jac_spec, s->fcg_spec, s->jac_spec_missed, s->jac_floor_released, s->ref64_corrections,
+        s->hdiv_fused, s->hdiv_launches);
     if (len >= n) return len + 1;
     memcpy(buf, tmp, (size_t)len + 1);
     return FG_OK;
@@ -1019,6 +1034,15 @@
     return FG_OK;
 }
 
+extern "C" int fg_write_buffer(fg_handle s, int which, const fg_real* src, void* stream) {
+    fg_real* dst = nullptr;
+    int64_t count = 0;
+    if (int rc = fg_get_buffer(s, which, &dst, &count)) return rc;
+    FG_REQUIRE(src, FG_ERR_INVALID_ARG, "null source");
+    FG_HIP_CHECK(hipMemcpyAsync(dst, src, sizeof(fg_real) * count, hipMemcpyDeviceToDevice, (hipStream_t)stream));
+    return FG_OK;
+}
+
 extern "C" int fg_poisson_apply(fg_handle s, const fg_real* rA, const fg_real* x, fg_real* y, void* stream) {
     FG_REQUIRE(s && rA && x && y, FG_ERR_INVALID_ARG, "null argument");
     return fg_poisson_apply_launch(s, rA, x, y, (hipStream_t)stream);
diff --git a/fluidgym_amd/csrc/fg_cg.h b/fluidgym_amd/csrc/fg_cg.h
--- a/fluidgym_amd/csrc/fg_cg.h
+++ b/fluidgym_amd/csrc/fg_cg.h
@@ -29,8 +29,8 @@
                    FgDacc* xsum; };
 int fg_cg_slots(const fg_state* s);
 #ifdef __HIPCC__
-__device__ __forceinline__ void fg_cg_begin_env(const FgCgBegin& q, const fg_real* __restrict__ dt, int b) {
-    for (int k = threadIdx.x; k < FG_CG_NAMES * q.ns; k += blockDim.x)
+__device__ __forceinline__ void fg_cg_begin_env(const FgCgBegin& q, const fg_real* __restrict__ dt, int b, bool keep_rr0 = false) {
+    for (int k = threadIdx.x + (keep_rr0 ? q.ns : 0); k < FG_CG_NAMES * q.ns; k += blockDim.x)
         acc_st(fg_acc_ptr(q.acc, b, k / q.ns) + k % q.ns, 0.0);
     if (threadIdx.x != 0) return;
     acc_st(q.mean_sums + b, 0.0);
diff --git a/fluidgym_amd/csrc/fg_fftcg.h b/fluidgym_amd/csrc/fg_fftcg.h
--- a/fluidgym_amd/csrc/fg_fftcg.h
+++ b/fluidgym_amd/csrc/fg_fftcg.h
@@ -34,7 +34,17 @@
     const float* hx; const float* hy; int fixed_x;
 };
 
+struct FcgHdivArgs {
+    FcgDivArgs d;
+    const float* rA; const float* Coff; const float* rhs; const float* u;
+    float* hvec;
+    FgCgBegin begin;
+    uint32_t* part; int32_t* ticket;
+};
+
 #if !FG_F64
+bool fg_fcg_hdiv_ok(const fg_state* s);
+int fg_fcg_hdiv_fwd(fg_state* s, const FgBounds& bnd, const fg_real* dt, const fg_real* vel_result, fg_real* hvec, fg_real* div, const FgCgBegin& begin, hipStream_t st);
 int fg_fcg_div_fwd(fg_state* s, const FgBounds& bnd, const fg_real* dt, const fg_real* hvec, fg_real* div, int ns, hipStream_t st);
 bool fg_fcg_ok(const fg_state* s);
 int fg_fcg_update_fwd(fg_state* s, const FcgVectors& v, int it, int first, int ns, hipStream_t st, bool marks_valid, const fg_real* r0 = nullptr);
diff --git a/fluidgym_amd/csrc/fg_fftcg.hip b/fluidgym_amd/csrc/fg_fftcg.hip
--- a/fluidgym_amd/csrc/fg_fftcg.hip
+++ b/fluidgym_amd/csrc/fg_fftcg.hip
@@ -2,6 +2,7 @@
 #include "fg_cg.h"
 #include "fg_fftrow.h"
 #include "fg_fftcg.h"
+#include "fg_hdiv.h"
 
 #if !FG_F64
 namespace {
@@ -357,25 +358,13 @@
 #pragma unroll
             for (int e = 0; e < VW; ++e) {
                 const float h_l = (e == 0) ? hl : hc[e > 0 ? e - 1 : 0], h_r = (e == VW - 1) ? hr : hc[e < VW - 1 ? e + 1 : VW - 1];
-                float acc = 0.f;
-                {
-                    const float area = hy;
-                    const float F_hi = (e == VW - 1 && xhi) ? a.bvel[1][((size_t)b * 2 + 0) * a.rows + jc] * area : 0.5f * (hc[e] + h_r) * area;
-                    const float F_lo = (e == 0 && xlo) ? a.bvel[0][((size_t)b * 2 + 0) * a.rows + jc] * area : 0.5f * (hc[e] + h_l) * area;
-                    acc += F_hi - F_lo;
-                }
-                {
-                    const float area = hx[e];
-                    const float F_hi = at_hi ? bh[e] * area : 0.5f * (v1[e] + vd[e]) * area;
-                    const float F_lo = at_lo ? bl[e] * area : 0.5f * (v1[e] + vu[e]) * area;
-                    acc += F_hi - F_lo;
-                }
+                const float acc = fg_div_cell2d(hc[e], h_l, h_r, v1[e], vu[e], vd[e], hy, hx[e], e == 0 && xlo, e == VW - 1 && xhi, at_lo, at_hi,
+                                                a.bvel[0] + ((size_t)b * 2 + 0) * a.rows + jc, a.bvel[1] + ((size_t)b * 2 + 0) * a.rows + jc, bl[e], bh[e]);
                 out[q * VW + e] = live ? acc : 0.f;
             }
         }
         if (live) {
-#pragma unroll
-            for (int e = 0; e < EPL; ++e) part[0] += out[e] * out[e];
+            fg_sumsq_row<EPL>(part[0], half ? db : da);
             const size_t o = (size_t)b * a.n + (size_t)j * N;
             fgfft::store_row<N>(a.div + o, lane, half ? db : da);
         }
@@ -387,6 +376,189 @@
     if (row0 + 1 < a.rows) fgfft::store_row<N>(a.t1 + (size_t)b * a.n + (size_t)(row0 + 1) * N, lane, ob);
     fg_block_sum<1>(part, red);
     if (threadIdx.x == 0) fg_acc_add(fg_acc_ptr(a.acc, b, 0), a.ns, blockIdx.x, (double)part[0]);
+}
+
+template <int N>
+__device__ __forceinline__ void row_neighbours(const float (&c)[N / 64], int lane, float (&left)[Map<N>::NG], float (&right)[Map<N>::NG]) {
+    using M = Map<N>;
+    float from_l[M::NG], from_r[M::NG];
+#pragma unroll
+    for (int q = 0; q < M::NG; ++q) {
+        from_l[q] = __shfl(c[q * M::VW + M::VW - 1], (lane + 63) & 63, 64);
+        from_r[q] = __shfl(c[q * M::VW], (lane + 1) & 63, 64);
+    }
+#pragma unroll
+    for (int q = 0; q < M::NG; ++q) {
+        left[q] = lane > 0 ? from_l[q] : from_l[(q + M::NG - 1) % M::NG];
+        right[q] = lane < 63 ? from_r[q] : from_r[(q + 1) % M::NG];
+    }
+}
+template <int N>
+__device__ __forceinline__ void hdiv_h_row(const FcgHdivArgs& q, int b, int j, int comp, int lane, const float (&rA)[N / 64],
+                                           const float (&off)[4][N / 64], float (&out)[N / 64]) {
+    using M = Map<N>;
+    constexpr int EPL = N / 64, VW = M::VW;
+    const int rows = q.d.rows;
+    const size_t base = ((size_t)b * 2 + comp) * q.d.n;
+    float uc[EPL], um[EPL], up[EPL], r[EPL];
+    fgfft::load_row<N>(q.u + base + (size_t)j * N, lane, uc);
+    fgfft::load_row<N>(q.u + base + (size_t)(j == 0 ? j : j - 1) * N, lane, um);
+    fgfft::load_row<N>(q.u + base + (size_t)(j == rows - 1 ? j : j + 1) * N, lane, up);
+    fgfft::load_row<N>(q.rhs + base + (size_t)j * N, lane, r);
+    float ul[M::NG], ur[M::NG];
+    row_neighbours<N>(uc, lane, ul, ur);
+    if (q.d.fixed_x) {
+        if (lane == 0) ul[0] = uc[0];
+        if (lane == 63) ur[M::NG - 1] = uc[EPL - 1];
+    }
+#pragma unroll
+    for (int g = 0; g < M::NG; ++g) {
+#pragma unroll
+        for (int e = 0; e < VW; ++e) {
+            const int i = g * VW + e;
+            const float u_xm = (e == 0) ? ul[g] : uc[i > 0 ? i - 1 : 0], u_xp = (e == VW - 1) ? ur[g] : uc[i < EPL - 1 ? i + 1 : EPL - 1];
+            const float H = fg_h_faces(off[0][i], off[1][i], off[2][i], off[3][i], u_xm, u_xp, um[i], up[i]);
+            out[i] = fg_h_value(rA[i], r[i], H);
+        }
+    }
+}
+template <int N>
+__device__ __forceinline__ void hdiv_coef_row(const FcgHdivArgs& q, int b, int j, int lane, float (&rA)[N / 64], float (&off)[4][N / 64]) {
+    const size_t n = q.d.n, o = (size_t)j * N;
+    fgfft::load_row<N>(q.rA + (size_t)b * n + o, lane, rA);
+#pragma unroll
+    for (int f = 0; f < 4; ++f) fgfft::load_row<N>(q.Coff + ((size_t)b * 4 + f) * n + o, lane, off[f]);
+}
+
+template <int N, bool PERIODIC>
+__global__ __launch_bounds__(320) void k_fcg_hdiv_fwd(FcgHdivArgs q) {
+    constexpr int EPL = N / 64;
+    using M = Map<N>;
+    constexpr int VW = M::VW;
+    const FcgDivArgs& a = q.d;
+    __shared__ __attribute__((aligned(16))) float2 buf[2][5][N];
+    __shared__ __attribute__((aligned(16))) float2 twl[N];
+    __shared__ float red[4];
+    __shared__ float parts[64];
+    const int b = blockIdx.y;
+    const bool active = a.dt[b] > 0.f;
+    if (blockIdx.x == 0) fg_cg_begin_env(q.begin, a.dt, b, active);
+    if (!active) return;
+    const int lane = threadIdx.x & 63, wave = threadIdx.x >> 6;
+    for (int k = threadIdx.x; k < N; k += 320) twl[k] = a.tw[k];
+    const int j0 = blockIdx.x * 8;
+    const int rowa = wave < 4 ? j0 + 2 * wave : j0 - 1, rowb = wave < 4 ? rowa + 1 : j0 + 8;
+    const bool livea = rowa >= 0 && rowa < a.rows, liveb = rowb < a.rows;
+    float hxa[EPL], hxb[EPL], hya[EPL], hyb[EPL];
+#pragma unroll
+    for (int e = 0; e < EPL; ++e) { hxa[e] = 0.f; hxb[e] = 0.f; hya[e] = 0.f; hyb[e] = 0.f; }
+    {
+        float rA[EPL], off[4][EPL];
+        if (livea) {
+            hdiv_coef_row<N>(q, b, rowa, lane, rA, off);
+            if (wave < 4) hdiv_h_row<N>(q, b, rowa, 0, lane, rA, off, hxa);
+            hdiv_h_row<N>(q, b, rowa, 1, lane, rA, off, hya);
+        }
+        if (liveb) {
+            hdiv_coef_row<N>(q, b, rowb, lane, rA, off);
+            if (wave < 4) hdiv_h_row<N>(q, b, rowb, 0, lane, rA, off, hxb);
+            hdiv_h_row<N>(q, b, rowb, 1, lane, rA, off, hyb);
+        }
+    }
+    float* sy = reinterpret_cast<float*>(buf[1][wave]);
+#pragma unroll
+    for (int g = 0; g < M::NG; ++g) {
+        fgfft::stv<VW>(sy + g * 64 * VW + lane * VW, &hya[g * VW]);
+        fgfft::stv<VW>(sy + N + g * 64 * VW + lane * VW, &hyb[g * VW]);
+    }
+    if (wave < 4) {
+        const size_t hb0 = ((size_t)b * 2 + 0) * a.n, hb1 = ((size_t)b * 2 + 1) * a.n;
+        if (livea) { fgfft::store_row<N>(q.hvec + hb0 + (size_t)rowa * N, lane, hxa); fgfft::store_row<N>(q.hvec + hb1 + (size_t)rowa * N, lane, hya); }
+        if (liveb) { fgfft::store_row<N>(q.hvec + hb0 + (size_t)rowb * N, lane, hxb); fgfft::store_row<N>(q.hvec + hb1 + (size_t)rowb * N, lane, hyb); }
+    }
+    __syncthreads();
+    float da[EPL], db[EPL];
+    float part[1] = {0.f};
+    if (wave < 4) {
+        const float* sy_up = (wave == 0) ? reinterpret_cast<const float*>(buf[1][4]) : sy - 2 * N + N;
+        const float* sy_dn = (wave == 3) ? reinterpret_cast<const float*>(buf[1][4]) + N : sy + 2 * N;
+#pragma unroll
+        for (int half = 0; half < 2; ++half) {
+            const int j = half ? rowb : rowa;
+            const bool live = half ? liveb : livea;
+            float (&out)[EPL] = half ? db : da;
+            if (!live) {
+#pragma unroll
+                for (int e = 0; e < EPL; ++e) out[e] = 0.f;
+                continue;
+            }
+            const float hy = a.hy[j];
+            const bool at_lo = j == 0, at_hi = j == a.rows - 1;
+            const float (&hrow)[EPL] = half ? hxb : hxa;
+            const float (&vrow)[EPL] = half ? hyb : hya;
+            const float* vu_ = at_lo ? sy + half * N : (half ? sy : sy_up);
+            const float* vd_ = at_hi ? sy + half * N : (half ? sy_dn : sy + N);
+            float hl[M::NG], hr[M::NG];
+            row_neighbours<N>(hrow, lane, hl, hr);
+#pragma unroll
+            for (int g = 0; g < M::NG; ++g) {
+                const int i0 = g * 64 * VW + lane * VW;
+                float vu[VW], vd[VW], hx[VW], bl[VW], bh[VW];
+                fgfft::ldv<VW>(vu_ + i0, vu);
+                fgfft::ldv<VW>(vd_ + i0, vd);
+                fgfft::ldv<VW>(a.hx + i0, hx);
+                if (at_lo) fgfft::ldv<VW>(a.bvel[2] + ((size_t)b * 2 + 1) * N + i0, bl);
+                if (at_hi) fgfft::ldv<VW>(a.bvel[3] + ((size_t)b * 2 + 1) * N + i0, bh);
+                const bool xlo = (i0 == 0) && a.fixed_x, xhi = (i0 + VW == N) && a.fixed_x;
+#pragma unroll
+                for (int e = 0; e < VW; ++e) {
+                    const int i = g * VW + e;
+                    const float h_l = (e == 0) ? hl[g] : hrow[i > 0 ? i - 1 : 0], h_r = (e == VW - 1) ? hr[g] : hrow[i < EPL - 1 ? i + 1 : EPL - 1];
+                    out[i] = fg_div_cell2d(hrow[i], h_l, h_r, vrow[i], vu[e], vd[e], hy, hx[e], e == 0 && xlo, e == VW - 1 && xhi, at_lo, at_hi,
+                                           a.bvel[0] + ((size_t)b * 2 + 0) * a.rows + j, a.bvel[1] + ((size_t)b * 2 + 0) * a.rows + j, bl[e], bh[e]);
+                }
+            }
+            fg_sumsq_row<EPL>(part[0], out);
+            fgfft::store_row<N>(a.div + (size_t)b * a.n + (size_t)j * N, lane, out);
+        }
+        const float sv = fg_wave_sum(part[0]);
+        if (lane == 0) red[wave] = sv;
+    }
+    __syncthreads();
+    if (wave == 4) return;
+    if (wave == 0) {
+        int last = 0;
+        if (lane == 0) {
+            const float tot = red[0] + red[1] + red[2] + red[3];
+            const uint32_t prev = __hip_atomic_exchange(q.part + (size_t)b * 64 + blockIdx.x, __float_as_uint(tot), __ATOMIC_RELAXED, __HIP_MEMORY_SCOPE_AGENT);
+            asm volatile("" ::"v"(prev) : "memory");
+            last = atomicAdd(q.ticket + b, 1) == (int)gridDim.x - 1;
+        }
+        if (__shfl(last, 0, 64)) {
+            const int nblk = gridDim.x;
+            parts[lane] = lane < nblk ? __uint_as_float(__hip_atomic_load(q.part + (size_t)b * 64 + lane, __ATOMIC_RELAXED, __HIP_MEMORY_SCOPE_AGENT)) : 0.f;
+            fgfft::wave_sync();
+            if (lane < a.ns) {
+                unsigned long long w[4] = {0ull, 0ull, 0ull, 0ull}, poison = 0ull;
+                for (int m = lane; m < nblk; m += a.ns) {
+                    long long k[5];
+                    if (!fg_dacc_split((double)parts[m], k)) { poison += 1ull; continue; }
+#pragma unroll
+                    for (int i = 0; i < 4; ++i) w[i] += (unsigned long long)k[i];
+                }
+                ulonglong2* o = reinterpret_cast<ulonglong2*>(fg_acc_ptr(a.acc, b, 0) + lane);
+                o[0] = make_ulonglong2(w[0], w[1]);
+                o[1] = make_ulonglong2(w[2], w[3]);
+                o[2] = make_ulonglong2(poison, (unsigned long long)__double_as_longlong(0.0));
+            }
+            if (lane == 0) atomicExch(q.ticket + b, 0);
+        }
+    }
+    if (!livea) return;
+    float oa[EPL], ob[EPL];
+    fgfft::forward_rows<N, PERIODIC>(da, db, oa, ob, buf[0][wave], buf[1][wave], twl, a.rot, fgfft::Scales{a.fs0, a.fs}, lane);
+    fgfft::store_row<N>(a.t1 + (size_t)b * a.n + (size_t)rowa * N, lane, oa);
+    if (liveb) fgfft::store_row<N>(a.t1 + (size_t)b * a.n + (size_t)rowb * N, lane, ob);
 }
 
 template <bool PERIODIC>
@@ -425,6 +597,41 @@
     return FG_OK;
 }
 
+template <bool PERIODIC>
+int launch_hdiv(const fg_state* s, int n, const FcgHdivArgs& a, dim3 grid, hipStream_t st) {
+    const int slot = fg_prof_slot(s, FG_PK_DIV, nullptr, s->grid.B, 52.0 * (double)s->grid.n, (32.0 + 5.0 * log2((double)n)) * (double)s->grid.n, st);
+    switch (n) {
+        case 64: FG_LAUNCH_P(s, slot, (k_fcg_hdiv_fwd<64, PERIODIC>), grid, dim3(320), 0, st, a); break;
+        case 128: FG_LAUNCH_P(s, slot, (k_fcg_hdiv_fwd<128, PERIODIC>), grid, dim3(320), 0, st, a); break;
+        case 256: FG_LAUNCH_P(s, slot, (k_fcg_hdiv_fwd<256, PERIODIC>), grid, dim3(320), 0, st, a); break;
+        case 512: FG_LAUNCH_P(s, slot, (k_fcg_hdiv_fwd<512, PERIODIC>), grid, dim3(320), 0, st, a); break;
+        default: fg_set_error("fused CG: unsupported row length"); return FG_ERR_UNSUPPORTED;
+    }
+    return FG_OK;
+}
+
+}
+
+bool fg_fcg_hdiv_ok(const fg_state* s) {
+    return s->hdiv_fused && s->hdiv_part != nullptr && fg_fcg_ok(s) && (s->grid.ny + 7) / 8 <= FG_CG_SLOTS;
+}
+
+int fg_fcg_hdiv_fwd(fg_state* s, const FgBounds& bnd, const fg_real* dt, const fg_real* vel_result, fg_real* hvec, fg_real* div, const FgCgBegin& begin, hipStream_t st) {
+    const FgGrid& G = s->grid;
+    FcgHdivArgs q = {};
+    FcgDivArgs& a = q.d;
+    a.h = hvec; a.div = div; a.r = s->w[0]; a.x = s->p_result; a.t1 = s->w[3];
+    for (int f = 0; f < 4; ++f) a.bvel[f] = bnd.vel[f];
+    a.tw = s->fd_dct_tw; a.rot = s->fd_dct_rot; a.fs0 = s->fd_dct_fwd[0]; a.fs = s->fd_dct_fwd[1];
+    a.dt = dt; a.acc = s->cg_acc; a.ns = begin.ns; a.rows = G.ny; a.n = G.n;
+    a.hx = G.h[0]; a.hy = G.h[1]; a.fixed_x = G.fixed[0];
+    q.rA = s->rA; q.Coff = s->Coff; q.rhs = s->adv_rhs; q.u = vel_result; q.hvec = hvec;
+    q.begin = begin; q.part = s->hdiv_part; q.ticket = s->hdiv_ticket;
+    const dim3 grid((G.ny + 7) / 8, G.B);
+    if (int rc = (s->fd_dct_x == 2 ? launch_hdiv<true>(s, G.nx, q, grid, st) : launch_hdiv<false>(s, G.nx, q, grid, st))) return rc;
+    FG_HIP_CHECK(hipGetLastError());
+    s->hdiv_launches += 1;
+    return FG_OK;
 }
 
 bool fg_fcg_ok(const fg_state* s) {
diff --git a/fluidgym_amd/csrc/fg_hdiv.h b/fluidgym_amd/csrc/fg_hdiv.h
--- /dev/null
+++ b/fluidgym_amd/csrc/fg_hdiv.h
@@ -0,0 +1,37 @@
+#pragma once
+#include "fg_internal.h"
+
+#ifdef __HIPCC__
+__device__ __forceinline__ float fg_fma(float a, float b, float c) { return __builtin_fmaf(a, b, c); }
+__device__ __forceinline__ double fg_fma(double a, double b, double c) { return __builtin_fma(a, b, c); }
+__device__ __forceinline__ fg_real fg_h_faces(fg_real o_xm, fg_real o_xp, fg_real o_ym, fg_real o_yp, fg_real u_xm, fg_real u_xp,
+                                              fg_real u_ym, fg_real u_yp) {
+    return fg_fma(o_yp, u_yp, fg_fma(o_ym, u_ym, fg_fma(o_xm, u_xm, o_xp * u_xp)));
+}
+__device__ __forceinline__ fg_real fg_h_value(fg_real rA, fg_real rhs, fg_real H) { return rA * (rhs - H); }
+
+#if !FG_F64
+__device__ __forceinline__ float fg_div_cell2d(float hc, float h_l, float h_r, float v1, float vu, float vd, float hy, float hx, bool x_lo,
+                                               bool x_hi, bool at_lo, bool at_hi, const float* __restrict__ bx_lo,
+                                               const float* __restrict__ bx_hi, float bl, float bh) {
+    const float mx_hi = x_hi ? *bx_hi : 0.5f * (hc + h_r), mx_lo = x_lo ? *bx_lo : 0.5f * (hc + h_l);
+    const float my_hi = at_hi ? bh : 0.5f * (v1 + vd), my_lo = at_lo ? bl : 0.5f * (v1 + vu);
+    const float fx = fg_fma(mx_hi, hy, -(mx_lo * hy));
+    const float fy = fg_fma(my_hi, hx, -(my_lo * hx));
+    return (0.f + fx) + fy;
+}
+template <int EPL>
+__device__ __forceinline__ void fg_sumsq_row(float& sum, const float (&v)[EPL]) {
+#pragma unroll
+    for (int e = 0; e < EPL; ++e) {
+        if constexpr (EPL == 1) {
+            sum = fg_fma(v[e], v[e], sum);
+        } else {
+            float sq = v[e] * v[e];
+            asm volatile("" : "+v"(sq));
+            sum += sq;
+        }
+    }
+}
+#endif
+#endif
diff --git a/fluidgym_amd/csrc/fg_internal.h b/fluidgym_amd/csrc/fg_internal.h
--- a/fluidgym_amd/csrc/fg_internal.h
+++ b/fluidgym_amd/csrc/fg_internal.h
@@ -656,6 +656,7 @@
     int tridiag_cb;
     int fd_dct_x; float2* fd_dct_tw; float2* fd_dct_rot; float fd_dct_fwd[2]; float fd_dct_inv[2];
     float* fd_lam_x; float* fd_row_inv; float* fd_row_cp; float* fd_row_lower; int fd_rowmean; long fd_row_epoch; mutable long rA_epoch;
+    int hdiv_fused; long hdiv_launches; uint32_t* hdiv_part; int32_t* hdiv_ticket;
     int fd_facfuse;
     float* fd_row_part; long fd_row_part_epoch;
     int32_t* forms_rec;
@@ -758,6 +759,7 @@
 int fg_launch_sgs(const fg_state* s, const FgBounds& bnd, fg_real coefficient, fg_real* out, hipStream_t st);
 int fg_launch_pressure_setup(const fg_state* s, const fg_real* dt, hipStream_t st);
 int fg_launch_h(fg_state* s, const fg_real* dt, const fg_real* vel_result, hipStream_t st);
+int fg_launch_h_div(fg_state* s, const FgBounds& bnd, const fg_real* dt, hipStream_t st, bool cg_from_zero, bool fused_fwd);
 int fg_launch_div(fg_state* s, const FgBounds& bnd, const fg_real* dt, const fg_real* hvec, fg_real* div, hipStream_t st,
                   bool cg_from_zero = false,
                   bool fused_fwd = false);
diff --git a/fluidgym_amd/csrc/fg_piso.hip b/fluidgym_amd/csrc/fg_piso.hip
--- a/fluidgym_amd/csrc/fg_piso.hip
+++ b/fluidgym_amd/csrc/fg_piso.hip
@@ -1,6 +1,7 @@
 #include "fg_internal.h"
 #include "fg_cg.h"
 #include "fg_fftcg.h"
+#include "fg_hdiv.h"
 
 namespace {
 
@@ -228,10 +229,9 @@
         FgVec<VEC> out;
 #pragma unroll
         for (int e = 0; e < VEC; ++e) {
-            fg_real H = off[0].v[e] * u.xm.v[e] + off[1].v[e] * u.xp.v[e] + off[2].v[e] * u.ym.v[e] +
-                      off[3].v[e] * u.yp.v[e];
+            fg_real H = fg_h_faces(off[0].v[e], off[1].v[e], off[2].v[e], off[3].v[e], u.xm.v[e], u.xp.v[e], u.ym.v[e], u.yp.v[e]);
             if constexpr (DIMS == 3) H += off[4].v[e] * u.zm.v[e] + off[5].v[e] * u.zp.v[e];
-            out.v[e] = rA.v[e] * (r.v[e] - H);
+            out.v[e] = fg_h_value(rA.v[e], r.v[e], H);
         }
         fg_store<VEC>(hvec + base + c.idx, out);
     }
@@ -921,6 +921,21 @@
     return FG_OK;
 }
 
+int fg_launch_h_div(fg_state* s, const FgBounds& bnd, const fg_real* dt, hipStream_t st, bool cg_from_zero, bool fused_fwd) {
+#if !FG_F64
+    if (cg_from_zero && fused_fwd && dt != nullptr && fg_fcg_hdiv_ok(s)) {
+        FgCgBegin begin;
+        begin.acc = s->cg_acc; begin.flags = s->flags; begin.info = s->info_dev; begin.mean_sums = s->acc; begin.best = s->cg_best;
+        begin.track_best = s->cg_return_best; begin.ns = fg_cg_slots(s); begin.xsum = s->fcg_xsum;
+        s->prepared.set_cg(begin.ns, begin.track_best, dt);
+        s->prepared.set_cg_start(2);
+        return fg_fcg_hdiv_fwd(s, bnd, dt, s->vel_result, s->hvec, s->div, begin, st);
+    }
+#endif
+    if (int rc = fg_launch_h(s, dt, s->vel_result, st)) return rc;
+    return fg_launch_div(s, bnd, dt, s->hvec, s->div, st, cg_from_zero, fused_fwd);
+}
+
 int fg_launch_div(fg_state* s, const FgBounds& bnd, const fg_real* dt, const fg_real* hvec, fg_real* div,
                   hipStream_t st, bool cg_from_zero, bool fused_fwd) {
     FgCgStart start = {nullptr, nullptr, nullptr, 1};
diff --git a/fluidgym_amd/native.py b/fluidgym_amd/native.py
--- a/fluidgym_amd/native.py
+++ b/fluidgym_amd/native.py
@@ -211,6 +211,14 @@
         L.check(self.lib.fg_read_buffer(self.handle, which, _ptr(out), _stream(self.device)), lib=self.lib)
         return out.view(*shape)
 
+    def write_buffer(self, which: int, t: torch.Tensor):
+        p, n = ctypes.c_void_p(), ctypes.c_int64()
+        L.check(self.lib.fg_get_buffer(self.handle, which, ctypes.byref(p), ctypes.byref(n)), lib=self.lib)
+        src = t.to(device=self.device, dtype=self.dtype).contiguous()
+        assert src.numel() == int(n.value), (src.numel(), int(n.value))
+        L.check(self.lib.fg_write_buffer(self.handle, which, _ptr(src), _stream(self.device)), lib=self.lib)
+        torch.cuda.current_stream(self.device).synchronize()
+
     def _infos(self, n):
         return (L.FgSolveInfo * n)()
 
@@ -260,6 +268,10 @@
 
     def setup_pressure_rhs(self, dt):
         L.check(self.lib.fg_setup_pressure_rhs(self.handle, _ptr(self.dt_tensor(dt)), _stream(self.device)), lib=self.lib)
+
+    def debug_pressure_rhs(self, method=None, pressure_warm_start=False):
+        method = self.default_method if method is None else method
+        L.check(self.lib.fg_debug_pressure_rhs(self.handle, method, int(pressure_warm_start), _stream(self.device)), lib=self.lib)
 
     def solve_pressure(self, tol=1e-5, max_iterations=5000, method=None, use_previous=False):
         method = self.default_method if method is None else method
diff --git a/include/fluidgym_hip.h b/include/fluidgym_hip.h
--- a/include/fluidgym_hip.h
+++ b/include/fluidgym_hip.h
@@ -204,6 +204,8 @@
 int fg_env_reset_solver_state(fg_handle h, const fg_env_sel* sel, int32_t n_sel, void* stream);
 int fg_get_buffer(fg_handle h, int which, fg_real** out_ptr, int64_t* out_count);
 int fg_read_buffer(fg_handle h, int which, fg_real* dst, void* stream);
+int fg_write_buffer(fg_handle h, int which, const fg_real* src, void* stream);
+int fg_debug_pressure_rhs(fg_handle h, int method, int pressure_warm_start, void* stream);
 
 int fg_poisson_apply(fg_handle h, const fg_real* rA, const fg_real* x, fg_real* y, void* stream);
 int fg_poisson_jacobi(fg_handle h, const fg_real* rA, const fg_real* b, fg_real* x, int n_sweeps, fg_real omega,
diff --git a/profiles/gen_switch_table.py b/profiles/gen_switch_table.py
--- a/profiles/gen_switch_table.py
+++ b/profiles/gen_switch_table.py
@@ -16,6 +16,7 @@
     "FG_HELM_ROWFORM": ("bits", "0: Helmholtz factors through k_helm_coeffs + the array-form line kernels (IEEE division instead of v_rcp)"),
     "FG_ADV_LINESWEEP": ("bits", "1: the advection-diffusion systems of the Helmholtz-preconditioned family (wall-refined 2-D grids: RBC) go to line sweeps x <- (D + O_y)^-1 (b - O_x x) first (k_line_sweep_y, fg_linepre.hip), BiCGStab takes what they do not settle; 0 (default): the preconditioned BiCGStab always -- measured on the RBC leg: 16-17 sweeps per velocity solve at the bench state's sub-step, 775 against 793 env-steps/s"),
     "FG_FD_FACFUSE": ("no", "1 (default): the first tridiagonal solve after 1/A changed makes the per-env row-mean factors itself (k_tridiag_y_lds<.., FAC>: same arithmetic, same bits); 0: k_fd_rowmean_factor as a launch of its own (A/B runs)"),
+    "FG_HDIV_FUSED": ("no", "1 (default): on the grids of the fused pressure CG the H operator, the divergence, the start of the solve and its first forward transform are ONE row kernel (k_fcg_hdiv_fwd: the arithmetic of the pair, same bits); 0: k_h and k_fcg_div_fwd as two launches (A/B runs, tests)"),
     "FG_FD_ROWMEAN": ("bits", "1 (default): the fused pressure CG is preconditioned by the row-mean operator (per-env factors, one factorisation per PISO step); 0: the grid's A = 1 factors"),
     "FG_ADV_JACOBI": ("bits", "velocity systems of uniform 2-D grids: 1 Jacobi sweeps first (fg_jacobi.hip), 0 BiCGStab always; unset = what fg_set_advection_jacobi says (the Simulation turns it on: policy advection_jacobi)"),
     "FLUIDGYM_AMD_ADVECTION_JACOBI": ("policy", "policy advection_jacobi (default 1): the Simulation asks for the Jacobi sweeps of fg_jacobi.hip on the grids that qualify"),
```

Result: no change. 9508 env-steps/s (-0.0%).
